# OpenVisualCloud/SVT-HEVC

Hardware: AMD Instinct MI355X
Metric: front-half fps, 4K 8-bit encMode 7 random-access B pictures (BASELINE configs[2]): pictures per second through upload + picture preparation + open-loop motion estimation of 2040 LCUs against 2 list(s) (HME L0 64x32 + L1, full-pel 16x9 85-PU search, sub-pel, bi-prediction) + open-loop intra search +  (higher is better)
Workload: dtype u8; 1 GPU

## Files before the change

include/svt_hevc_amd.h:

```cpp
#ifndef SVT_HEVC_AMD_H
#define SVT_HEVC_AMD_H

#include <stdint.h>
#include <stddef.h>

#ifdef __cplusplus
extern "C" {
#endif

#define SVT_AMD_API __attribute__((visibility("default")))

typedef enum SvtAmdStatus {
    SVT_AMD_OK = 0,
    SVT_AMD_ERR_BAD_PARAM = -1,
    SVT_AMD_ERR_RESOURCES = -2,
    SVT_AMD_ERR_DEVICE = -3
} SvtAmdStatus;


#define SVT_AMD_LCU_SIZE 64
#define SVT_AMD_ME_PU_COUNT 85
#define SVT_AMD_PAD_FULL 68
#define SVT_AMD_PAD_QUARTER 32
#define SVT_AMD_PAD_SIXTEENTH 16
// ... 1239 lines not shown
                                        uint32_t refStride, void *d_dst, uint32_t dstStride,
                                        const SvtAmdMcpBlock *d_blocks, uint32_t nblocks, uint32_t max_block_dim);
SVT_AMD_API int svt_amd_bipred_clip_batch(SvtAmdContext *ctx, int bytes_per_sample, const int16_t *d_l0,
                                          const int16_t *d_l1, void *d_dst, uint32_t dstStride, int32_t offset,
                                          const SvtAmdBiPredBlock *d_blocks, uint32_t nblocks);

#define SVT_AMD_DECL_MCP_UNI(name, T)                                                                          \
    SVT_AMD_API void svt_amd_##name(T *refPic, uint32_t srcStride, T *dst, uint32_t dstStride, uint32_t puWidth, \
                                    uint32_t puHeight, int16_t *firstPassIFDst);
#define SVT_AMD_DECL_MCP_RAW(name, T)                                                                          \
    SVT_AMD_API void svt_amd_##name(T *refPic, uint32_t srcStride, int16_t *dst, uint32_t puWidth,             \
                                    uint32_t puHeight, int16_t *firstPassIFDst);
#define SVT_AMD_DECL_MCP_CUNI(name, T)                                                                         \
    SVT_AMD_API void svt_amd_##name(T *refPic, uint32_t srcStride, T *dst, uint32_t dstStride, uint32_t puWidth, \
                                    uint32_t puHeight, int16_t *firstPassIFDst, uint32_t fracPosx, uint32_t fracPosy);
#define SVT_AMD_DECL_MCP_CRAW(name, T)                                                                         \
    SVT_AMD_API void svt_amd_##name(T *refPic, uint32_t srcStride, int16_t *dst, uint32_t puWidth,             \
                                    uint32_t puHeight, int16_t *firstPassIFDst, uint32_t fracPosx, uint32_t fracPosy);
SVT_AMD_DECL_MCP_UNI(LumaInterpolationFilterPosaNew, uint8_t)
SVT_AMD_DECL_MCP_UNI(LumaInterpolationFilterPosaNew16bit, uint16_t)
SVT_AMD_DECL_MCP_RAW(LumaInterpolationFilterPosaOutRaw, uint8_t)
SVT_AMD_DECL_MCP_RAW(LumaInterpolationFilterPosaOutRaw16bit, uint16_t)
SVT_AMD_DECL_MCP_UNI(LumaInterpolationFilterPosbNew, uint8_t)
SVT_AMD_DECL_MCP_UNI(LumaInterpolationFilterPosbNew16bit, uint16_t)
SVT_AMD_DECL_MCP_RAW(LumaInterpolationFilterPosbOutRaw, uint8_t)
SVT_AMD_DECL_MCP_RAW(LumaInterpolationFilterPosbOutRaw16bit, uint16_t)
SVT_AMD_DECL_MCP_UNI(LumaInterpolationFilterPoscNew, uint8_t)
SVT_AMD_DECL_MCP_UNI(LumaInterpolationFilterPoscNew16bit, uint16_t)
SVT_AMD_DECL_MCP_RAW(LumaInterpolationFilterPoscOutRaw, uint8_t)
SVT_AMD_DECL_MCP_RAW(LumaInterpolationFilterPoscOutRaw16bit, uint16_t)
SVT_AMD_DECL_MCP_UNI(LumaInterpolationFilterPosdNew, uint8_t)
SVT_AMD_DECL_MCP_UNI(LumaInterpolationFilterPosdNew16bit, uint16_t)
SVT_AMD_DECL_MCP_RAW(LumaInterpolationFilterPosdOutRaw, uint8_t)
SVT_AMD_DECL_MCP_RAW(LumaInterpolationFilterPosdOutRaw16bit, uint16_t)
SVT_AMD_DECL_MCP_UNI(LumaInterpolationFilterPoseNew, uint8_t)
SVT_AMD_DECL_MCP_UNI(LumaInterpolationFilterPoseNew16bit, uint16_t)
SVT_AMD_DECL_MCP_RAW(LumaInterpolationFilterPoseOutRaw, uint8_t)
SVT_AMD_DECL_MCP_RAW(LumaInterpolationFilterPoseOutRaw16bit, uint16_t)
SVT_AMD_DECL_MCP_UNI(LumaInterpolationFilterPosfNew, uint8_t)
SVT_AMD_DECL_MCP_UNI(LumaInterpolationFilterPosfNew16bit, uint16_t)
SVT_AMD_DECL_MCP_RAW(LumaInterpolationFilterPosfOutRaw, uint8_t)
SVT_AMD_DECL_MCP_RAW(LumaInterpolationFilterPosfOutRaw16bit, uint16_t)
SVT_AMD_DECL_MCP_UNI(LumaInterpolationFilterPosgNew, uint8_t)
SVT_AMD_DECL_MCP_UNI(LumaInterpolationFilterPosgNew16bit, uint16_t)
SVT_AMD_DECL_MCP_RAW(LumaInterpolationFilterPosgOutRaw, uint8_t)
SVT_AMD_DECL_MCP_RAW(LumaInterpolationFilterPosgOutRaw16bit, uint16_t)
SVT_AMD_DECL_MCP_UNI(LumaInterpolationFilterPoshNew, uint8_t)
SVT_AMD_DECL_MCP_UNI(LumaInterpolationFilterPoshNew16bit, uint16_t)
SVT_AMD_DECL_MCP_RAW(LumaInterpolationFilterPoshOutRaw, uint8_t)
SVT_AMD_DECL_MCP_RAW(LumaInterpolationFilterPoshOutRaw16bit, uint16_t)
SVT_AMD_DECL_MCP_UNI(LumaInterpolationFilterPosiNew, uint8_t)
SVT_AMD_DECL_MCP_UNI(LumaInterpolationFilterPosiNew16bit, uint16_t)
SVT_AMD_DECL_MCP_RAW(LumaInterpolationFilterPosiOutRaw, uint8_t)
SVT_AMD_DECL_MCP_RAW(LumaInterpolationFilterPosiOutRaw16bit, uint16_t)
SVT_AMD_DECL_MCP_UNI(LumaInterpolationFilterPosjNew, uint8_t)
SVT_AMD_DECL_MCP_UNI(LumaInterpolationFilterPosjNew16bit, uint16_t)
SVT_AMD_DECL_MCP_RAW(LumaInterpolationFilterPosjOutRaw, uint8_t)
SVT_AMD_DECL_MCP_RAW(LumaInterpolationFilterPosjOutRaw16bit, uint16_t)
SVT_AMD_DECL_MCP_UNI(LumaInterpolationFilterPoskNew, uint8_t)
SVT_AMD_DECL_MCP_UNI(LumaInterpolationFilterPoskNew16bit, uint16_t)
SVT_AMD_DECL_MCP_RAW(LumaInterpolationFilterPoskOutRaw, uint8_t)
SVT_AMD_DECL_MCP_RAW(LumaInterpolationFilterPoskOutRaw16bit, uint16_t)
SVT_AMD_DECL_MCP_UNI(LumaInterpolationFilterPosnNew, uint8_t)
SVT_AMD_DECL_MCP_UNI(LumaInterpolationFilterPosnNew16bit, uint16_t)
SVT_AMD_DECL_MCP_RAW(LumaInterpolationFilterPosnOutRaw, uint8_t)
SVT_AMD_DECL_MCP_RAW(LumaInterpolationFilterPosnOutRaw16bit, uint16_t)
SVT_AMD_DECL_MCP_UNI(LumaInterpolationFilterPospNew, uint8_t)
SVT_AMD_DECL_MCP_UNI(LumaInterpolationFilterPospNew16bit, uint16_t)
SVT_AMD_DECL_MCP_RAW(LumaInterpolationFilterPospOutRaw, uint8_t)
SVT_AMD_DECL_MCP_RAW(LumaInterpolationFilterPospOutRaw16bit, uint16_t)
SVT_AMD_DECL_MCP_UNI(LumaInterpolationFilterPosqNew, uint8_t)
SVT_AMD_DECL_MCP_UNI(LumaInterpolationFilterPosqNew16bit, uint16_t)
SVT_AMD_DECL_MCP_RAW(LumaInterpolationFilterPosqOutRaw, uint8_t)
SVT_AMD_DECL_MCP_RAW(LumaInterpolationFilterPosqOutRaw16bit, uint16_t)
SVT_AMD_DECL_MCP_UNI(LumaInterpolationFilterPosrNew, uint8_t)
SVT_AMD_DECL_MCP_UNI(LumaInterpolationFilterPosrNew16bit, uint16_t)
SVT_AMD_DECL_MCP_RAW(LumaInterpolationFilterPosrOutRaw, uint8_t)
SVT_AMD_DECL_MCP_RAW(LumaInterpolationFilterPosrOutRaw16bit, uint16_t)
SVT_AMD_DECL_MCP_UNI(LumaInterpolationCopy, uint8_t)
SVT_AMD_DECL_MCP_UNI(LumaInterpolationCopy16bit, uint16_t)
SVT_AMD_DECL_MCP_RAW(LumaInterpolationCopyOutRaw, uint8_t)
SVT_AMD_DECL_MCP_RAW(LumaInterpolationCopyOutRaw16bit, uint16_t)
SVT_AMD_DECL_MCP_CUNI(ChromaInterpolationCopy, uint8_t)
SVT_AMD_DECL_MCP_CUNI(ChromaInterpolationFilterOneD, uint8_t)
SVT_AMD_DECL_MCP_CUNI(ChromaInterpolationFilterTwoD, uint8_t)
SVT_AMD_DECL_MCP_CUNI(ChromaInterpolationCopy16bit, uint16_t)
SVT_AMD_DECL_MCP_CUNI(ChromaInterpolationFilterOneD16bit, uint16_t)
SVT_AMD_DECL_MCP_CUNI(ChromaInterpolationFilterTwoD16bit, uint16_t)
SVT_AMD_DECL_MCP_CRAW(ChromaInterpolationCopyOutRaw, uint8_t)
SVT_AMD_DECL_MCP_CRAW(ChromaInterpolationFilterOneDOutRaw, uint8_t)
SVT_AMD_DECL_MCP_CRAW(ChromaInterpolationFilterTwoDOutRaw, uint8_t)
SVT_AMD_DECL_MCP_CRAW(ChromaInterpolationCopyOutRaw16bit, uint16_t)
SVT_AMD_DECL_MCP_CRAW(ChromaInterpolationFilterOneDOutRaw16bit, uint16_t)
SVT_AMD_DECL_MCP_CRAW(ChromaInterpolationFilterTwoDOutRaw16bit, uint16_t)
SVT_AMD_API void svt_amd_BiPredClipping(uint32_t puWidth, uint32_t puHeight, int16_t *list0Src, int16_t *list1Src,
                                        uint8_t *dst, uint32_t dstStride, int32_t offset);
SVT_AMD_API void svt_amd_BiPredClipping16bit(uint32_t puWidth, uint32_t puHeight, int16_t *list0Src, int16_t *list1Src,
                                             uint16_t *dst, uint32_t dstStride);


typedef struct SvtAmdMdRates {
    uint32_t splitFlagBits[6], skipFlagBits[6], mvpIndexBits[2], intraPartSizeBits[2], interPartSizeBits[8], predModeBits[2];
    uint32_t intraLumaBits[4], intraChromaBits[5], refPicBits[3], mvdBits[12], lumaCbfBits[10], chromaCbfBits[10], rootCbfBits[2];
    uint32_t transSubDivFlagBits[6], mergeFlagBits[2], mergeIndexBits[5], saoMergeFlagBits[2], saoTypeIndexBits[6];
    uint32_t saoOffsetTrunUnaryBits[8], interBiDirBits[8], interUniDirBits[2], pad[17];
} SvtAmdMdRates;
typedef struct SvtAmdMdPicture {
    uint16_t width, height;
    uint8_t slice_type;
    uint8_t temporal_layer, is_reference, enc_mode;
    uint8_t depth_mode;
    uint8_t intra_md_open_loop;
    uint8_t intra_injection_method;
    uint8_t limit_intra;
    uint8_t mpm_search, mpm_search_candidate;
    uint8_t pf_md_level, nfl_level_md, nmm_level_md;
    uint8_t full_loop_escape, single_fast_loop, coeff_cabac_update, spatial_sse_full_loop;
    uint8_t chroma_level;
    uint8_t intra4x4_level;
    uint8_t rdoq_pmcore_method;
    uint8_t skip_ois_8x8, cu8x8_mode, cu16x16_mode, limit_ois_to_dc_mode;
    uint8_t constrained_intra, strong_smoothing;
    uint8_t qp, chroma_qp;
    uint8_t intra8x8_restriction_inter_slice;
    uint8_t pad;
    uint32_t fast_lambda, full_lambda, fast_chroma_lambda, full_chroma_lambda;
    SvtAmdMdRates rates;
} SvtAmdMdPicture;
#define SVT_AMD_MD_LEAVES 85
typedef struct SvtAmdMdLcu {
    uint8_t leaf_count;
    uint8_t leaf_index[SVT_AMD_MD_LEAVES], leaf_split[SVT_AMD_MD_LEAVES];
    uint8_t tile_left, tile_top, tile_right;
    uint8_t is_complete;
    uint8_t complexity_status_2;
    uint8_t contouring_class[4];
    uint8_t chroma_encode_mode;
    uint8_t restrict_intra_global_motion;
    uint8_t lcu_md_mode;
    uint8_t skip_small_cu;
    uint8_t cmplx_noise;
    uint8_t variance_below_200;
    uint8_t edge_block;
    uint8_t no_stop_split;
    uint8_t pad[3];
} SvtAmdMdLcu;
typedef struct SvtAmdTmvpLcu {
    int16_t mv[2][16][2];
    uint64_t ref_poc[2][16];
    uint8_t pred_dir[16], available[16];
} SvtAmdTmvpLcu;
typedef struct SvtAmdMdInter {
    uint64_t picture_number;
    uint64_t ref_poc[2];
    uint64_t colocated_poc;
    uint8_t colocated_pu_ref_list, is_low_delay;
    uint8_t tmvp_enable;
    uint8_t use_subpel;
    uint8_t unrestricted_mv;
    uint8_t generate_amvp_table_md;
    uint8_t extra_injection;
    uint8_t improve_sharpness;
    uint8_t skip_cost_bias;
    uint8_t pad[3];
    uint32_t chroma_weight;
} SvtAmdMdInter;
typedef struct SvtAmdMdLcuOut {
    uint8_t split[SVT_AMD_MD_LEAVES];
    uint8_t tested[SVT_AMD_MD_LEAVES];
    uint8_t pred_mode[SVT_AMD_MD_LEAVES];
    uint8_t intra_luma_mode[SVT_AMD_MD_LEAVES];
    uint8_t ycbf[SVT_AMD_MD_LEAVES];
    uint8_t inter_dir[SVT_AMD_MD_LEAVES];
    uint8_t merge_flag[SVT_AMD_MD_LEAVES], merge_index[SVT_AMD_MD_LEAVES];
    uint8_t pad[8];
    int16_t mv[SVT_AMD_MD_LEAVES][2][2];
    uint64_t cost[SVT_AMD_MD_LEAVES];
    uint64_t merge_cost[SVT_AMD_MD_LEAVES], skip_cost[SVT_AMD_MD_LEAVES];
} SvtAmdMdLcuOut;
SVT_AMD_API int svt_amd_md_picture_supported(const SvtAmdMdPicture *P);
SVT_AMD_API int svt_amd_md_encode_picture(SvtAmdContext *ctx, SvtAmdEncDecPicture *pic, const SvtAmdMdPicture *P, const SvtAmdMdLcu *lcus,
                                          const uint8_t *src_y, uint32_t stride_y, const uint8_t *src_cb, const uint8_t *src_cr,
                                          uint32_t stride_c, const SvtAmdOisLcuResult *ois, int ois_slot, const SvtAmdCabacCost *cost,
                                          SvtAmdMdLcuOut *md_out, SvtAmdLcuWork *works, SvtAmdLcuResult *results);
SVT_AMD_API int svt_amd_md_encode_picture_inter(SvtAmdContext *ctx, SvtAmdEncDecPicture *pic, const SvtAmdMdPicture *P, const SvtAmdMdInter *X,
                                                const SvtAmdMdLcu *lcus, const uint8_t *src_y, uint32_t stride_y, const uint8_t *src_cb,
                                                const uint8_t *src_cr, uint32_t stride_c, const SvtAmdOisLcuResult *ois, int ois_slot,
                                                const SvtAmdMeLcuResult *me, int me_slot, const SvtAmdTmvpLcu *tmvp,
                                                SvtAmdMdLcuOut *md_out, SvtAmdLcuWork *works, SvtAmdLcuResult *results);
SVT_AMD_API int svt_amd_md_encode_picture16(SvtAmdContext *ctx, SvtAmdEncDecPicture *pic, const SvtAmdMdPicture *P, const SvtAmdMdLcu *lcus,
                                            const uint16_t *src_y, uint32_t stride_y, const uint16_t *src_cb, const uint16_t *src_cr,
                                            uint32_t stride_c, const SvtAmdOisLcuResult *ois, int ois_slot, const SvtAmdCabacCost *cost,
                                            SvtAmdMdLcuOut *md_out, SvtAmdLcuWork16 *works, SvtAmdLcuResult16 *results);
SVT_AMD_API int svt_amd_md_encode_picture_inter16(SvtAmdContext *ctx, SvtAmdEncDecPicture *pic, const SvtAmdMdPicture *P, const SvtAmdMdInter *X,
                                                  const SvtAmdMdLcu *lcus, const uint16_t *src_y, uint32_t stride_y, const uint16_t *src_cb,
                                                  const uint16_t *src_cr, uint32_t stride_c, const SvtAmdOisLcuResult *ois, int ois_slot,
                                                  const SvtAmdMeLcuResult *me, int me_slot, const SvtAmdTmvpLcu *tmvp, SvtAmdMdLcuOut *md_out,
                                                  SvtAmdLcuWork16 *works, SvtAmdLcuResult16 *results);
SVT_AMD_API int svt_amd_md_picture_supported_inter(const SvtAmdMdPicture *P, const SvtAmdMdInter *X);
SVT_AMD_API int svt_amd_md_lcus_supported(const SvtAmdMdPicture *P, const SvtAmdMdLcu *lcus, int n);
SVT_AMD_API int svt_amd_md_picture_set_controls(SvtAmdContext *ctx, SvtAmdEncDecPicture *pic, const SvtAmdMdLcu *d_lcus);

#define SVT_AMD_MD_LAUNCH_DECIDE_ONLY 1u
typedef struct SvtAmdMdLaunchJob {
    const SvtAmdMdPicture *P;
    const SvtAmdMdInter *X;
    const SvtAmdCabacCost *cost;
    const SvtAmdMdLcu *d_lcus;
    const void *d_src[3];
    const SvtAmdOisLcuResult *d_ois;
    const SvtAmdMeLcuResult *d_me;
    const SvtAmdTmvpLcu *d_tmvp;
    uint32_t src_pitch_y, src_pitch_c;
    int32_t ois_slot, me_slot;
    uint32_t tiles;
    uint32_t flags;
    uint32_t pad[2];
} SvtAmdMdLaunchJob;
typedef struct SvtAmdMdLaunchStatus {
    SvtAmdMdCtlCheck check;
    uint32_t refused;
    uint32_t pad;
} SvtAmdMdLaunchStatus;
#ifdef __cplusplus
static_assert(sizeof(SvtAmdMdLaunchJob) == 112 && sizeof(SvtAmdMdLaunchStatus) == 96, "launch records");
#else
_Static_assert(sizeof(SvtAmdMdLaunchJob) == 112 && sizeof(SvtAmdMdLaunchStatus) == 96, "launch records");
#endif
SVT_AMD_API int svt_amd_md_encode_picture_launch(SvtAmdContext *ctx, SvtAmdEncDecPicture *pic, const SvtAmdMdLaunchJob *job, SvtAmdMdLaunchStatus *d_status);
SVT_AMD_API int svt_amd_encdec_picture_md_records(SvtAmdEncDecPicture *pic, const SvtAmdMdLcuOut **d_out, const void **d_works, size_t *work_stride,
                                                  const void **d_results, size_t *result_stride);

typedef struct SvtAmdMotionFieldJob {
    const void *d_works;
    size_t      work_stride;
    uint16_t    width, height;
    uint8_t     slice_type;
    uint8_t     pad[3];
    uint64_t    ref_poc[2];
} SvtAmdMotionFieldJob;
typedef struct SvtAmdRefStats {
    uint32_t intra_area_sum;
    uint8_t  intra_coded_area;
    uint8_t  pad[3];
} SvtAmdRefStats;
#define SVT_AMD_MOTION_FIELD 0
#define SVT_AMD_MOTION_FIELD_STATS 1
SVT_AMD_API size_t svt_amd_motion_field_bytes(uint16_t luma_width, uint16_t luma_height, int which);
SVT_AMD_API int svt_amd_motion_field_launch(SvtAmdContext *ctx, const SvtAmdMotionFieldJob *job, SvtAmdTmvpLcu *d_field, SvtAmdRefStats *d_stats);
SVT_AMD_API int svt_amd_encdec_picture_motion_field(SvtAmdContext *ctx, SvtAmdEncDecPicture *pic, int slice_type, const uint64_t ref_poc[2], SvtAmdTmvpLcu *d_field,
                                                    SvtAmdRefStats *d_stats);
SVT_AMD_API int svt_amd_md_picture_set_motion_field(SvtAmdContext *ctx, SvtAmdEncDecPicture *pic, const SvtAmdTmvpLcu *d_field);
SVT_AMD_API int svt_amd_debug_md_profile(SvtAmdContext *ctx, SvtAmdEncDecPicture *pic, unsigned long long *out);
SVT_AMD_API int svt_amd_debug_md_profile_sub(SvtAmdContext *ctx, SvtAmdEncDecPicture *pic, unsigned long long *out);
SVT_AMD_API int svt_amd_debug_md_profile_depth(SvtAmdContext *ctx, SvtAmdEncDecPicture *pic, unsigned long long *out);
SVT_AMD_API int svt_amd_debug_md_force_butterflies(SvtAmdContext *ctx, SvtAmdEncDecPicture *pic, int on);
SVT_AMD_API int svt_amd_debug_md_trace(SvtAmdContext *ctx, SvtAmdEncDecPicture *pic, int lcu, int unit, unsigned long long *out);
SVT_AMD_API int svt_amd_debug_md_kernel_ms(SvtAmdContext *ctx, SvtAmdEncDecPicture *pic, float *ms, int *workgroups);
SVT_AMD_API int svt_amd_debug_md_ep_ms(SvtAmdContext *ctx, SvtAmdEncDecPicture *pic, float *ms);
SVT_AMD_API int svt_amd_debug_md_flights(int *in_flight, int *workgroups_held, int *waiting);
SVT_AMD_API int svt_amd_md_picture_warmup(SvtAmdContext *ctx, SvtAmdEncDecPicture *pic);
SVT_AMD_API int svt_amd_debug_md_kernel_lds_bytes(int inter, int bytes_per_sample);
typedef struct SvtAmdMdListNb {
    int16_t mv[2][2];
    uint8_t dir, avail, pad[2];
} SvtAmdMdListNb;
typedef struct SvtAmdMdListJob {
    uint16_t width, height;
    uint16_t ox, oy;
    uint8_t size;
    uint8_t slice_type;
    uint8_t colocated_pu_ref_list, is_low_delay;
    uint8_t has_field;
    uint8_t total_merge;
    uint8_t tile_left, tile_top, tile_right;
    uint8_t me_dir;
    uint16_t pool[2];
    int16_t me_mv[2][2];
    uint8_t pad[2];
    uint64_t picture_number, ref_poc[2], colocated_poc;
    SvtAmdMdListNb nb[5];
    uint8_t pad2[4];
} SvtAmdMdListJob;
typedef struct SvtAmdMdListOut {
    int16_t amvp[2][2][2];
    uint8_t amvp_count[2];
    uint8_t merge_count;
    uint8_t mvp_idx[2];
    uint8_t merge_dir[5];
    int16_t merge_mv[5][2][2];
    int16_t cand_mv[2][2];
    int16_t mvp[2][2];
    uint8_t pad[14];
} SvtAmdMdListOut;
#ifdef __cplusplus
static_assert(sizeof(SvtAmdMdListNb) == 12 && sizeof(SvtAmdMdListJob) == 128 && sizeof(SvtAmdMdListOut) == 96, "tests mirror these layouts as numpy dtypes");
#else
_Static_assert(sizeof(SvtAmdMdListNb) == 12 && sizeof(SvtAmdMdListJob) == 128 && sizeof(SvtAmdMdListOut) == 96, "tests mirror these layouts as numpy dtypes");
#endif
SVT_AMD_API int svt_amd_debug_md_lists_batch(SvtAmdContext *ctx, const SvtAmdMdListJob *d_jobs, const SvtAmdTmvpLcu *d_pool, SvtAmdMdListOut *d_outs, uint32_t n);
SVT_AMD_API int svt_amd_debug_me_kernel_lds_bytes(const SvtAmdMeParams *params, int phase);
SVT_AMD_API int svt_amd_debug_me_kernel_occupancy(SvtAmdContext *ctx, const SvtAmdMeParams *params, int phase, int *workgroups_per_cu, int *private_bytes);
SVT_AMD_API int svt_amd_debug_launch_markers(SvtAmdContext *ctx, unsigned long long *records, unsigned long long *waits);

#ifdef __cplusplus
}
#endif
#endif
```

svt-hevc_amd/csrc/context.hip:

```cpp
#include <stdarg.h>
#include <stdio.h>
#include <stdlib.h>
#include <string.h>
#include "svt_amd_internal.h"
#include <vector>
#include <mutex>

static thread_local char g_err[512] = "";

void svt_amd_set_error(const char *fmt, ...)
{
    va_list ap;
    va_start(ap, fmt);
    vsnprintf(g_err, sizeof(g_err), fmt, ap);
    va_end(ap);
}

extern "C" const char *svt_amd_last_error(void) { return g_err; }
extern "C" const char *svt_amd_version(void) { return "svt-hevc_amd 0.1 (gfx950)"; }

static int align_up(int v, int a) { return (v + a - 1) / a * a; }

static int plane_create(DevPlane *p, int w, int h, int pad)
{
// ... 422 lines not shown
        HIP_TRY(hipMemcpy(dst, d_src, bytes, hipMemcpyDeviceToHost));
        return SVT_AMD_OK;
    }
    HIP_TRY(hipMemcpyAsync(dst, d_src, bytes, hipMemcpyDeviceToHost, svt_amd_ctx_stream(ctx)));
    HIP_TRY(svt_amd_ctx_sync(ctx));
    return SVT_AMD_OK;
}

extern "C" int svt_amd_device_upload_async(SvtAmdContext *ctx, void *d_dst, const void *src, size_t bytes)
{
    if (!ctx || !d_dst || !src)
        return SVT_AMD_ERR_BAD_PARAM;
    HIP_TRY(hipSetDevice(ctx->device));
    HIP_TRY(hipMemcpyAsync(d_dst, src, bytes, hipMemcpyHostToDevice, svt_amd_ctx_stream(ctx)));
    return SVT_AMD_OK;
}
extern "C" int svt_amd_device_download_async(SvtAmdContext *ctx, void *dst, const void *d_src, size_t bytes)
{
    if (!ctx || !dst || !d_src)
        return SVT_AMD_ERR_BAD_PARAM;
    HIP_TRY(hipSetDevice(ctx->device));
    HIP_TRY(hipMemcpyAsync(dst, d_src, bytes, hipMemcpyDeviceToHost, svt_amd_ctx_stream(ctx)));
    return SVT_AMD_OK;
}
extern "C" int svt_amd_host_alloc(SvtAmdContext *ctx, size_t bytes, void **h_ptr)
{
    if (!ctx || !h_ptr || !bytes)
        return SVT_AMD_ERR_BAD_PARAM;
    HIP_TRY(hipSetDevice(ctx->device));
    HIP_TRY(hipHostMalloc(h_ptr, bytes, hipHostMallocDefault));
    return SVT_AMD_OK;
}
namespace {
struct HostReg { const void *p; size_t bytes; bool ok; };
std::mutex g_reg_mu;
std::vector<HostReg> g_reg;
}
extern "C" int svt_amd_host_register(SvtAmdContext *ctx, const void *h_ptr, size_t bytes)
{
    if (!ctx || !h_ptr || !bytes)
        return SVT_AMD_ERR_BAD_PARAM;
    std::lock_guard<std::mutex> g(g_reg_mu);
    for (HostReg &r : g_reg)
        if (r.p == h_ptr && r.bytes >= bytes)
            return SVT_AMD_OK;
    for (HostReg &r : g_reg)
        if ((const uint8_t *)h_ptr < (const uint8_t *)r.p + r.bytes && (const uint8_t *)r.p < (const uint8_t *)h_ptr + bytes) {
            g_reg.push_back({h_ptr, bytes, false});
            return SVT_AMD_OK;
        }
    (void)hipSetDevice(ctx->device);
    const hipError_t e = hipHostRegister(const_cast<void *>(h_ptr), bytes, hipHostRegisterDefault);
    if (e != hipSuccess)
        (void)hipGetLastError();
    g_reg.push_back({h_ptr, bytes, e == hipSuccess});
    return SVT_AMD_OK;
}
const void *svt_amd_registered_device_ptr(const void *h_ptr, size_t bytes)
{
    std::lock_guard<std::mutex> g(g_reg_mu);
    for (const HostReg &r : g_reg)
        if (r.ok && (const uint8_t *)h_ptr >= (const uint8_t *)r.p && (const uint8_t *)h_ptr + bytes <= (const uint8_t *)r.p + r.bytes) {
            void *d = nullptr;
            if (hipHostGetDevicePointer(&d, const_cast<void *>(r.p), 0) != hipSuccess) {
                (void)hipGetLastError();
                return nullptr;
            }
            return (const uint8_t *)d + ((const uint8_t *)h_ptr - (const uint8_t *)r.p);
        }
    return nullptr;
}
extern "C" int svt_amd_host_unregister_all(SvtAmdContext *ctx)
{
    if (!ctx)
        return SVT_AMD_ERR_BAD_PARAM;
    std::lock_guard<std::mutex> g(g_reg_mu);
    (void)hipSetDevice(ctx->device);
    for (HostReg &r : g_reg)
        if (r.ok && hipHostUnregister(const_cast<void *>(r.p)) != hipSuccess)
            (void)hipGetLastError();
    g_reg.clear();
    return SVT_AMD_OK;
}
extern "C" int svt_amd_host_free(SvtAmdContext *ctx, void *h_ptr)
{
    if (!ctx)
        return SVT_AMD_ERR_BAD_PARAM;
    HIP_TRY(hipSetDevice(ctx->device));
    HIP_TRY(hipHostFree(h_ptr));
    return SVT_AMD_OK;
}


static int check_slot(SvtAmdContext *ctx, int slot)
{
    if (!ctx || slot < 0 || slot >= ctx->num_slots) {
        svt_amd_set_error("bad context/slot %d", slot);
        return SVT_AMD_ERR_BAD_PARAM;
    }
    return SVT_AMD_OK;
}

static int set_geometry(SvtAmdContext *ctx, DevPicture *s, uint16_t width, uint16_t height)
{
    if (width < 64 || height < 64 || (width & 7) || (height & 7) || width > ctx->max_w || height > ctx->max_h) {
        svt_amd_set_error("picture %ux%u not supported by context %ux%u", width, height, ctx->max_w, ctx->max_h);
        return SVT_AMD_ERR_BAD_PARAM;
    }
    s->width = width;
    s->height = height;
    s->full.width = s->hp_b.width = s->hp_h.width = s->hp_j.width = width;
    s->full.height = s->hp_b.height = s->hp_h.height = s->hp_j.height = height;
    s->quarter.width = width >> 1, s->quarter.height = height >> 1;
    s->sixteenth.width = width >> 2, s->sixteenth.height = height >> 2;
    return SVT_AMD_OK;
}

extern "C" int svt_amd_picture_upload_device(SvtAmdContext *ctx, int slot, const void *d_luma,
                                             uint32_t stride, uint16_t width, uint16_t height)
{
    int rc = check_slot(ctx, slot);
    if (rc)
        return rc;
    if (!d_luma || stride < width)
        return SVT_AMD_ERR_BAD_PARAM;
    HIP_TRY(hipSetDevice(ctx->device));
    DevPicture *s = &ctx->slots[slot];
    if ((rc = set_geometry(ctx, s, width, height)) != 0)
        return rc;
    if ((rc = svt_amd_launch_prep(ctx, s, (const uint8_t *)d_luma, stride)) != 0)
        return rc;
    slot_records_forget(&s->rec);
    s->valid = 1;
    return SVT_AMD_OK;
}

extern "C" int svt_amd_picture_upload_device_batch(SvtAmdContext *ctx, int num, const int *slots,
                                                   const void *const *d_luma, uint32_t stride, uint16_t width,
                                                   uint16_t height)
{
    if (!ctx || !slots || !d_luma || num < 1 || num > SVT_AMD_MAX_BATCH || stride < width)
        return SVT_AMD_ERR_BAD_PARAM;
    HIP_TRY(hipSetDevice(ctx->device));
    DevPicture *pics[SVT_AMD_MAX_BATCH];
    for (int i = 0; i < num; i++) {
        int rc = check_slot(ctx, slots[i]);
        if (rc)
            return rc;
        if (!d_luma[i])
            return SVT_AMD_ERR_BAD_PARAM;
        pics[i] = &ctx->slots[slots[i]];
        if ((rc = set_geometry(ctx, pics[i], width, height)) != 0)
            return rc;
    }
    int rc = svt_amd_launch_prep_batch(ctx, pics, (const uint8_t *const *)d_luma, stride, num);
    if (rc)
        return rc;
    for (int i = 0; i < num; i++)
        slot_records_forget(&pics[i]->rec), pics[i]->valid = 1;
    return SVT_AMD_OK;
}

extern "C" int svt_amd_picture_upload(SvtAmdContext *ctx, int slot, const uint8_t *luma,
                                      uint32_t stride, uint16_t width, uint16_t height)
{
    int rc = check_slot(ctx, slot);
    if (rc)
        return rc;
    if (!luma || stride < width)
        return SVT_AMD_ERR_BAD_PARAM;
    HIP_TRY(hipSetDevice(ctx->device));
    DevPicture *s = &ctx->slots[slot];
    if ((size_t)width * height > s->staging_bytes)
        return SVT_AMD_ERR_BAD_PARAM;
    HIP_TRY(hipMemcpy2DAsync(s->d_staging, width, luma, stride, width, height, hipMemcpyHostToDevice, svt_amd_ctx_stream(ctx)));
    HIP_TRY(svt_amd_ctx_sync(ctx));
    return svt_amd_picture_upload_device(ctx, slot, s->d_staging, width, width, height);
}

extern "C" int svt_amd_picture_read_plane(SvtAmdContext *ctx, int slot, int which, uint8_t *dst,
                                          size_t dst_capacity, uint32_t *out_stride,
                                          uint32_t *out_pad, uint32_t *out_rows)
{
    int rc = check_slot(ctx, slot);
    if (rc)
        return rc;
    DevPicture *s = &ctx->slots[slot];
    DevPlane *pl[6] = {&s->full, &s->quarter, &s->sixteenth, &s->hp_b, &s->hp_h, &s->hp_j};
    if (which < 0 || which > 5 || !dst || !out_stride || !out_pad || !out_rows)
        return SVT_AMD_ERR_BAD_PARAM;
    DevPlane *p = pl[which];
    const uint32_t w = (uint32_t)(p->width + 2 * p->pad), rows = (uint32_t)(p->height + 2 * p->pad);
    if (dst_capacity < (size_t)w * rows)
        return SVT_AMD_ERR_BAD_PARAM;
    HIP_TRY(hipSetDevice(ctx->device));
    HIP_TRY(svt_amd_ctx_sync(ctx));
    HIP_TRY(hipMemcpy2D(dst, w, p->origin - (size_t)p->pad * p->pitch - p->pad, (size_t)p->pitch, w, rows,
                        hipMemcpyDeviceToHost));
    *out_stride = w;
    *out_pad = (uint32_t)p->pad;
    *out_rows = rows;
    return SVT_AMD_OK;
}


static int validate_me(SvtAmdContext *ctx, const SvtAmdMeParams *p, int cur_slot, const int ref_slot[2])
{
    if (!ctx || !p || !ref_slot)
        return SVT_AMD_ERR_BAD_PARAM;
    if (p->num_lists < 1 || p->num_lists > 2 || p->num_hme_regions_w > 2 || p->num_hme_regions_h > 2 ||
        p->search_area_width < 1 || p->search_area_height < 1) {
        svt_amd_set_error("svt_amd_me_picture: bad SvtAmdMeParams");
        return SVT_AMD_ERR_BAD_PARAM;
    }
    int rc = check_slot(ctx, cur_slot);
    for (int l = 0; !rc && l < p->num_lists; l++)
        rc = check_slot(ctx, ref_slot[l]);
    if (rc)
        return rc;
    const DevPicture *c = &ctx->slots[cur_slot];
    if (!c->valid || c->width != p->luma_width || c->height != p->luma_height) {
        svt_amd_set_error("svt_amd_me_picture: slot %d does not hold a %ux%u picture", cur_slot, p->luma_width,
                          p->luma_height);
        return SVT_AMD_ERR_BAD_PARAM;
    }
    for (int l = 0; l < p->num_lists; l++) {
        const DevPicture *r = &ctx->slots[ref_slot[l]];
        if (!r->valid || r->width != c->width || r->height != c->height) {
            svt_amd_set_error("svt_amd_me_picture: reference slot %d invalid", ref_slot[l]);
            return SVT_AMD_ERR_BAD_PARAM;
        }
    }
    return SVT_AMD_OK;
}

static int slot_mark_lend(SvtAmdContext *ctx, DevPicture *s, int kind, LaunchMark *mark, uint32_t n, uint32_t begin, uint32_t end)
{
    SlotRecords *r = &s->rec;
    slot_lock(r);
    const hipEvent_t behind = slot_chain_behind(r, kind, ctx, begin == 0 && end >= n);
    hipError_t e = behind ? hipStreamWaitEvent(svt_amd_ctx_stream(ctx), behind, 0) : hipSuccess;
    if (e == hipSuccess && !mark->ev) {
        const hipEvent_t ev = ctx->ev_launch[ctx->launch_next];
        if ((e = hipEventRecord(ev, svt_amd_ctx_stream(ctx))) == hipSuccess) {
            ctx->launch_next = (ctx->launch_next + 1) & 15;
            ctx->mark_records += kind != SLOT_READ;
            *mark = LaunchMark{ev, ctx};
        }
    }
    if (e == hipSuccess) {
        r->mark[kind] = *mark;
        if (kind == SLOT_ME)
            slot_me_cover(r, n, begin, end);
        else if (kind == SLOT_OIS)
            r->ois_lcus = n;
    }
    slot_unlock(r);
    HIP_TRY(e);
    ctx->mark_waits += behind != nullptr;
    return SVT_AMD_OK;
}
int svt_amd_records_wait(SvtAmdContext *ctx, DevPicture *s, int kind, hipEvent_t *seen, int *nseen, int cap)
{
    slot_lock(&s->rec);
    const hipEvent_t ev = slot_wait_for(&s->rec, kind, ctx);
    bool wait = ev != nullptr;
    for (int i = 0; wait && seen && i < *nseen; i++)
        wait = seen[i] != ev;
    const hipError_t e = wait ? hipStreamWaitEvent(svt_amd_ctx_stream(ctx), ev, 0) : hipSuccess;
    if (ev && kind == SLOT_READ && e == hipSuccess)
        s->rec.mark[SLOT_READ] = LaunchMark{nullptr, nullptr};
    slot_unlock(&s->rec);
    HIP_TRY(e);
    if (wait) {
        ctx->mark_waits++;
        if (seen && *nseen < cap)
            seen[(*nseen)++] = ev;
    }
    return SVT_AMD_OK;
}
static int slot_records_before_write(SvtAmdContext *ctx, DevPicture *s) { return svt_amd_records_wait(ctx, s, SLOT_READ, nullptr, nullptr, 0); }
int svt_amd_records_read_mark(SvtAmdContext *ctx, SvtAmdContext *root, int slot)
{
    LaunchMark mark{nullptr, nullptr};
    return slot_mark_lend(ctx, &root->slots[slot], SLOT_READ, &mark, 0, 0, 0);
}
const void *svt_amd_slot_records(SvtAmdContext *root, int slot, int which, int w, int h)
{
    if (slot < 0 || slot >= root->num_slots)
        return nullptr;
    DevPicture *s = &root->slots[slot];
    if (!s->valid || s->width != w || s->height != h || slot_lcus(&s->rec, which) != (uint32_t)svt_amd_lcu_count(w, h))
        return nullptr;
    return which ? (const void *)s->d_ois_out : (const void *)s->d_me_out;
}
extern "C" int svt_amd_debug_launch_markers(SvtAmdContext *ctx, unsigned long long *records, unsigned long long *waits)
{
    if (!ctx || !records || !waits)
        return SVT_AMD_ERR_BAD_PARAM;
    *records = ctx->mark_records, *waits = ctx->mark_waits;
    return SVT_AMD_OK;
}

static int make_job(SvtAmdContext *ctx, const SvtAmdMeParams *params, int cur_slot, const int ref_slot[2],
                    uint32_t lcu_begin, uint32_t lcu_end, MeJobDev *job)
{
    int rc = validate_me(ctx, params, cur_slot, ref_slot);
    if (rc)
        return rc;
    const uint32_t nlcu = svt_amd_lcu_count(params->luma_width, params->luma_height);
    if (lcu_begin >= lcu_end || lcu_end > nlcu) {
        svt_amd_set_error("motion estimation: bad LCU range [%u,%u) of %u", lcu_begin, lcu_end, nlcu);
        return SVT_AMD_ERR_BAD_PARAM;
    }
    DevPicture *c = &ctx->slots[cur_slot];
    const DevPicture *r0 = &ctx->slots[ref_slot[0]];
    const DevPicture *r1 = params->num_lists == 2 ? &ctx->slots[ref_slot[1]] : r0;
    job->P = *params;
    job->cur = make_view(c);
    job->ref0 = make_view(r0);
    job->ref1 = make_view(r1);
    job->out = c->d_me_out;
    job->carry = (struct MeCarry *)c->d_me_carry;
    job->lcu_begin = (int32_t)lcu_begin;
    job->lcu_count = (int32_t)(lcu_end - lcu_begin);
    job->dbg_clock = NULL;
    return SVT_AMD_OK;
}

extern "C" int svt_amd_me_picture_range_launch(SvtAmdContext *ctx, const SvtAmdMeParams *params, int cur_slot,
                                               const int ref_slot[2], uint32_t lcu_begin, uint32_t lcu_end)
{
    MeJobDev job;
    int rc = make_job(ctx, params, cur_slot, ref_slot, lcu_begin, lcu_end, &job);
    if (rc)
        return rc;
    HIP_TRY(hipSetDevice(ctx->device));
    if ((rc = slot_records_before_write(ctx, &ctx->slots[cur_slot])) != 0)
        return rc;
    LaunchMark mark{nullptr, nullptr};
    if ((rc = svt_amd_launch_me_batch(ctx, &job, 1, job.lcu_count)) == SVT_AMD_OK)
        rc = slot_mark_lend(ctx, &ctx->slots[cur_slot], SLOT_ME, &mark, (uint32_t)svt_amd_lcu_count(params->luma_width, params->luma_height), lcu_begin, lcu_end);
    return rc;
}

extern "C" int svt_amd_me_batch_launch(SvtAmdContext *ctx, const SvtAmdMeJob *jobs, int num_jobs)
{
    if (!ctx || !jobs || num_jobs < 1 || num_jobs > SVT_AMD_MAX_BATCH) {
        svt_amd_set_error("svt_amd_me_batch_launch: 1..%d jobs", SVT_AMD_MAX_BATCH);
        return SVT_AMD_ERR_BAD_PARAM;
    }
    MeJobDev *dj = (MeJobDev *)malloc(sizeof(MeJobDev) * (size_t)num_jobs);
    if (!dj)
        return SVT_AMD_ERR_RESOURCES;
    int rc = SVT_AMD_OK, max_lcus = 0;
    for (int i = 0; i < num_jobs && rc == SVT_AMD_OK; i++) {
        const SvtAmdMeParams *p = &jobs[i].params;
        const uint32_t nlcu = svt_amd_lcu_count(p->luma_width, p->luma_height);
        rc = make_job(ctx, p, jobs[i].cur_slot, jobs[i].ref_slot, 0, nlcu, &dj[i]);
        if (rc == SVT_AMD_OK)
            max_lcus = dj[i].lcu_count > max_lcus ? dj[i].lcu_count : max_lcus;
    }
    if (rc == SVT_AMD_OK) {
        hipError_t e = hipSetDevice(ctx->device);
        if (e == hipSuccess && ctx->d_dbg && (size_t)num_jobs * max_lcus <= ctx->dbg_slots)
            for (int i = 0; i < num_jobs; i++)
                dj[i].dbg_clock = ctx->d_dbg;
        for (int i = 0; i < num_jobs && e == hipSuccess && rc == SVT_AMD_OK; i++)
            rc = slot_records_before_write(ctx, &ctx->slots[jobs[i].cur_slot]);
        if (rc == SVT_AMD_OK)
            rc = e == hipSuccess ? svt_amd_launch_me_batch(ctx, dj, num_jobs, max_lcus) : SVT_AMD_ERR_DEVICE;
        LaunchMark mark{nullptr, nullptr};
        for (int i = 0; i < num_jobs && rc == SVT_AMD_OK; i++)
            rc = slot_mark_lend(ctx, &ctx->slots[jobs[i].cur_slot], SLOT_ME, &mark, (uint32_t)dj[i].lcu_count, 0, (uint32_t)dj[i].lcu_count);
    }
    free(dj);
    return rc;
}

extern "C" int svt_amd_debug_me_phase_profile(SvtAmdContext *ctx, size_t workgroups, unsigned long long *out)
{
    if (!ctx)
        return SVT_AMD_ERR_BAD_PARAM;
    HIP_TRY(hipSetDevice(ctx->device));
    if (!out) {
        HIP_TRY(svt_amd_ctx_sync(ctx));
        if (ctx->d_dbg)
            (void)hipFree(ctx->d_dbg);
        ctx->d_dbg = NULL;
        HIP_TRY(hipMalloc((void **)&ctx->d_dbg, workgroups * 16 * sizeof(unsigned long long)));
        HIP_TRY(hipMemset(ctx->d_dbg, 0, workgroups * 16 * sizeof(unsigned long long)));
        ctx->dbg_slots = workgroups;
        return SVT_AMD_OK;
    }
    if (!ctx->d_dbg || workgroups > ctx->dbg_slots)
        return SVT_AMD_ERR_BAD_PARAM;
    HIP_TRY(svt_amd_ctx_sync(ctx));
    HIP_TRY(hipMemcpy(out, ctx->d_dbg, workgroups * 16 * sizeof(unsigned long long), hipMemcpyDeviceToHost));
    (void)hipFree(ctx->d_dbg);
    ctx->d_dbg = NULL;
    ctx->dbg_slots = 0;
    return SVT_AMD_OK;
}

extern "C" int svt_amd_debug_me_kernel_occupancy(SvtAmdContext *ctx, const SvtAmdMeParams *params, int phase, int *workgroups_per_cu, int *private_bytes)
{
    if (!ctx)
        return SVT_AMD_ERR_BAD_PARAM;
    HIP_TRY(hipSetDevice(ctx->device));
    return svt_amd_me_kernel_occupancy(params, phase, workgroups_per_cu, private_bytes);
}

extern "C" int svt_amd_me_picture_launch(SvtAmdContext *ctx, const SvtAmdMeParams *params, int cur_slot,
                                         const int ref_slot[2])
{
    if (!params)
        return SVT_AMD_ERR_BAD_PARAM;
    const uint32_t nlcu = svt_amd_lcu_count(params->luma_width, params->luma_height);
    return svt_amd_me_picture_range_launch(ctx, params, cur_slot, ref_slot, 0, nlcu);
}

static int records_fetch(SvtAmdContext *ctx, int cur_slot, int which, void *out, bool sync)
{
    int rc = check_slot(ctx, cur_slot);
    if (rc)
        return rc;
    if (!out)
        return SVT_AMD_ERR_BAD_PARAM;
    HIP_TRY(hipSetDevice(ctx->device));
    DevPicture *c = &ctx->slots[cur_slot];
    const size_t bytes = (size_t)svt_amd_lcu_count(c->width, c->height) * (which ? sizeof(SvtAmdOisLcuResult) : sizeof(SvtAmdMeLcuResult));
    HIP_TRY(hipMemcpyAsync(out, which ? (const void *)c->d_ois_out : (const void *)c->d_me_out, bytes, hipMemcpyDeviceToHost, svt_amd_ctx_stream(ctx)));
    if (sync)
        HIP_TRY(svt_amd_ctx_sync(ctx));
    return SVT_AMD_OK;
}
extern "C" int svt_amd_me_picture_fetch(SvtAmdContext *ctx, int cur_slot, SvtAmdMeLcuResult *out) { return records_fetch(ctx, cur_slot, 0, out, true); }
extern "C" int svt_amd_me_picture_fetch_async(SvtAmdContext *ctx, int cur_slot, SvtAmdMeLcuResult *out) { return records_fetch(ctx, cur_slot, 0, out, false); }
extern "C" int svt_amd_ois_picture_fetch(SvtAmdContext *ctx, int cur_slot, SvtAmdOisLcuResult *out) { return records_fetch(ctx, cur_slot, 1, out, true); }
extern "C" int svt_amd_ois_picture_fetch_async(SvtAmdContext *ctx, int cur_slot, SvtAmdOisLcuResult *out) { return records_fetch(ctx, cur_slot, 1, out, false); }

extern "C" int svt_amd_lane_event_record(SvtAmdContext *lane, int index)
{
    if (!lane || index < 0 || index >= 8)
        return SVT_AMD_ERR_BAD_PARAM;
    HIP_TRY(hipSetDevice(lane->device));
    if (!lane->ev_user[index])
        HIP_TRY(hipEventCreateWithFlags(&lane->ev_user[index], hipEventDisableTiming));
    HIP_TRY(hipEventRecord(lane->ev_user[index], svt_amd_ctx_stream(lane)));
    return SVT_AMD_OK;
}
extern "C" int svt_amd_lane_event_wait(SvtAmdContext *lane, SvtAmdContext *source, int index)
{
    if (!lane || !source || index < 0 || index >= 8 || lane->device != source->device)
        return SVT_AMD_ERR_BAD_PARAM;
    HIP_TRY(hipSetDevice(lane->device));
    if (source->ev_user[index])
        HIP_TRY(hipStreamWaitEvent(svt_amd_ctx_stream(lane), source->ev_user[index], 0));
    return SVT_AMD_OK;
}

__global__ void __launch_bounds__(256) k_pack_me(const PackSrc *__restrict__ tab, const uint32_t *__restrict__ one, uint32_t *__restrict__ out, int nlcu)
{
    constexpr int IN = sizeof(SvtAmdMeLcuResult) / 4, OUT = SVT_AMD_ME_PU_COUNT * sizeof(SvtAmdMeCuResult) / 4;
    const uint32_t *__restrict__ in = tab ? tab[blockIdx.y].me : one;
    const int i = blockIdx.x * 256 + threadIdx.x, lcu = i / OUT, k = i - lcu * OUT;
    if (lcu < nlcu)
        out[((size_t)blockIdx.y * nlcu + lcu) * OUT + k] = in[(size_t)lcu * IN + k];
}
__global__ void __launch_bounds__(256) k_pack_ois(const PackSrc *__restrict__ tab, const uint32_t *__restrict__ one, uint32_t *__restrict__ out, int nlcu, int nc, int kshift)
{
    constexpr int IN = sizeof(SvtAmdOisLcuResult) / 4, TAIL = 22;
    const int per = SVT_AMD_ME_PU_COUNT * nc + TAIL, lcu = blockIdx.x;
    const uint32_t *__restrict__ src = (tab ? tab[blockIdx.y].ois : one) + (size_t)lcu * IN;
    uint32_t *__restrict__ dst = out + ((size_t)blockIdx.y * nlcu + lcu) * per;
    const int k = threadIdx.x & ((1 << kshift) - 1);
    if (k < nc)
        for (int cu = threadIdx.x >> kshift; cu < SVT_AMD_ME_PU_COUNT; cu += 256 >> kshift)
            dst[cu * nc + k] = src[cu * SVT_AMD_OIS_MAX_CAND + k];
    if (threadIdx.x < TAIL)
        dst[SVT_AMD_ME_PU_COUNT * nc + threadIdx.x] = src[SVT_AMD_ME_PU_COUNT * SVT_AMD_OIS_MAX_CAND + threadIdx.x];
}
static int launch_pack(SvtAmdContext *ctx, const PackSrc *tab, const PackSrc &one, int n, int nlcu, int candidates, void *d_me, void *d_ois)
{
    if (d_me) {
        const int k = nlcu * (int)(SVT_AMD_ME_PU_COUNT * sizeof(SvtAmdMeCuResult) / 4);
        hipLaunchKernelGGL(k_pack_me, dim3((k + 255) / 256, n), dim3(256), 0, svt_amd_ctx_stream(ctx), tab, one.me, (uint32_t *)d_me, nlcu);
    }
    if (d_ois) {
        int kshift = 0;
        while ((1 << kshift) < candidates)
            kshift++;
        hipLaunchKernelGGL(k_pack_ois, dim3(nlcu, n), dim3(256), 0, svt_amd_ctx_stream(ctx), tab, one.ois, (uint32_t *)d_ois, nlcu, candidates, kshift);
    }
    HIP_TRY(hipGetLastError());
    return SVT_AMD_OK;
}
static_assert(sizeof(SvtAmdOisLcuResult) == (SVT_AMD_ME_PU_COUNT * SVT_AMD_OIS_MAX_CAND + 22) * 4, "OIS record layout");
static_assert(sizeof(SvtAmdMeCuResult) == 24 && offsetof(SvtAmdMeLcuResult, pu) == 0, "ME record layout");

extern "C" int svt_amd_ois_compact_candidates(const SvtAmdOisParams *p)
{
    return !p ? SVT_AMD_OIS_MAX_CAND : p->slice_is_intra ? 7 : p->ois_kernel_level ? 18 : 9;
}

static int slot_pack_buffer(SvtAmdContext *ctx, DevPicture *c, size_t bytes, uint8_t **out)
{
    if (bytes > c->pack_bytes) {
        HIP_TRY(svt_amd_ctx_sync(ctx));
        if (c->d_pack)
            (void)hipFree(c->d_pack);
        c->d_pack = nullptr, c->pack_bytes = 0;
        HIP_TRY(hipMalloc((void **)&c->d_pack, bytes));
        c->pack_bytes = bytes;
    }
    *out = c->d_pack;
    return SVT_AMD_OK;
}

static size_t pack_me_bytes(int nlcu) { return ((size_t)nlcu * SVT_AMD_ME_PU_COUNT * sizeof(SvtAmdMeCuResult) + 255) & ~(size_t)255; }

extern "C" int svt_amd_me_picture_fetch_compact_async(SvtAmdContext *ctx, int cur_slot, SvtAmdMeCuResult *out)
{
    int rc = check_slot(ctx, cur_slot);
    if (rc)
        return rc;
    if (!out)
        return SVT_AMD_ERR_BAD_PARAM;
    HIP_TRY(hipSetDevice(ctx->device));
    DevPicture *c = &ctx->slots[cur_slot];
    const int nlcu = svt_amd_lcu_count(c->width, c->height);
    uint8_t *d = nullptr;
    if ((rc = slot_pack_buffer(ctx, c, pack_me_bytes(nlcu) + (size_t)nlcu * sizeof(SvtAmdOisLcuResult), &d)) != 0)
        return rc;
    const int n = nlcu * (int)(SVT_AMD_ME_PU_COUNT * sizeof(SvtAmdMeCuResult) / 4);
    if ((rc = launch_pack(ctx, nullptr, PackSrc{(const uint32_t *)c->d_me_out, nullptr}, 1, nlcu, 1, d, nullptr)) != 0)
        return rc;
    HIP_TRY(hipMemcpyAsync(out, d, (size_t)n * 4, hipMemcpyDeviceToHost, svt_amd_ctx_stream(ctx)));
    return SVT_AMD_OK;
}

extern "C" int svt_amd_ois_picture_fetch_compact_async(SvtAmdContext *ctx, int cur_slot, int candidates, void *out)
{
    int rc = check_slot(ctx, cur_slot);
    if (rc)
        return rc;
    if (!out || candidates < 1 || candidates > SVT_AMD_OIS_MAX_CAND)
        return SVT_AMD_ERR_BAD_PARAM;
    HIP_TRY(hipSetDevice(ctx->device));
    DevPicture *c = &ctx->slots[cur_slot];
    const int nlcu = svt_amd_lcu_count(c->width, c->height);
    uint8_t *d = nullptr;
    if ((rc = slot_pack_buffer(ctx, c, pack_me_bytes(nlcu) + (size_t)nlcu * sizeof(SvtAmdOisLcuResult), &d)) != 0)
        return rc;
    d += pack_me_bytes(nlcu);
    const int n = nlcu * (SVT_AMD_ME_PU_COUNT * candidates + 22);
    if ((rc = launch_pack(ctx, nullptr, PackSrc{nullptr, (const uint32_t *)c->d_ois_out}, 1, nlcu, candidates, nullptr, d)) != 0)
        return rc;
    HIP_TRY(hipMemcpyAsync(out, d, (size_t)n * 4, hipMemcpyDeviceToHost, svt_amd_ctx_stream(ctx)));
    return SVT_AMD_OK;
}

extern "C" int svt_amd_records_pack_batch_async(SvtAmdContext *ctx, const int *slots, int n, int candidates, SvtAmdMeCuResult *d_me, void *d_ois)
{
    if (!ctx || !slots || n < 1 || n > SVT_AMD_MAX_BATCH || (!d_me && !d_ois) || candidates < 1 || candidates > SVT_AMD_OIS_MAX_CAND)
        return SVT_AMD_ERR_BAD_PARAM;
    int rc = check_slot(ctx, slots[0]);
    if (rc)
        return rc;
    HIP_TRY(hipSetDevice(ctx->device));
    const DevPicture *c0 = &ctx->slots[slots[0]];
    const int nlcu = svt_amd_lcu_count(c0->width, c0->height);
    static thread_local PackSrc tab[SVT_AMD_MAX_BATCH];
    for (int i = 0; i < n; i++) {
        if ((rc = check_slot(ctx, slots[i])) != 0)
            return rc;
        const DevPicture *c = &ctx->slots[slots[i]];
        if (c->width != c0->width || c->height != c0->height) {
            svt_amd_set_error("svt_amd_records_pack_batch_async: pictures of different sizes in one batch");
            return SVT_AMD_ERR_BAD_PARAM;
        }
        tab[i].me = (const uint32_t *)c->d_me_out, tab[i].ois = (const uint32_t *)c->d_ois_out;
    }
    if ((rc = svt_amd_upload_descriptors(ctx, ctx->d_pack_src, tab, sizeof(PackSrc) * (size_t)n)) != 0)
        return rc;
    return launch_pack(ctx, (const PackSrc *)ctx->d_pack_src, PackSrc{nullptr, nullptr}, n, nlcu, candidates, d_me, d_ois);
}

extern "C" int svt_amd_me_picture(SvtAmdContext *ctx, const SvtAmdMeParams *params, int cur_slot,
                                  const int ref_slot[2], SvtAmdMeLcuResult *out)
{
    int rc = svt_amd_me_picture_launch(ctx, params, cur_slot, ref_slot);
    if (rc)
        return rc;
    return svt_amd_me_picture_fetch(ctx, cur_slot, out);
}

static int validate_ois(SvtAmdContext *ctx, const SvtAmdOisParams *p, int cur_slot)
{
    int rc = check_slot(ctx, cur_slot);
    if (rc)
        return rc;
    const DevPicture *c = &ctx->slots[cur_slot];
    if (!p || !c->valid || p->luma_width != c->width || p->luma_height != c->height || p->ois_th_set > 2 ||
        p->temporal_layer_index > 5) {
        svt_amd_set_error("svt_amd_ois_picture: bad parameter (slot %d)", cur_slot);
        return SVT_AMD_ERR_BAD_PARAM;
    }
    return SVT_AMD_OK;
}

static void make_ois_job(SvtAmdContext *ctx, const SvtAmdOisParams *params, int cur_slot, const SvtAmdMeLcuResult *d_me,
                         OisJobDev *j)
{
    DevPicture *c = &ctx->slots[cur_slot];
    j->P = *params;
    j->full = c->full.origin;
    j->pitch = c->full.pitch;
    j->lcus_w = (params->luma_width + 63) / 64;
    j->nlcu = j->lcus_w * ((params->luma_height + 63) / 64);
    j->me = d_me;
// ... 284 lines not shown
```

svt-hevc_amd/csrc/me_kernels.hip:

```cpp
#include <mutex>
#include "svt_amd_internal.h"

#define NT 256
#define LCU 64
#ifndef ME_MIN_WAVES_PER_SIMD
#define ME_MIN_WAVES_PER_SIMD 4
#endif
#ifndef ME_HME_WAVES_PER_SIMD
#define ME_HME_WAVES_PER_SIMD 6
#endif
#define COST_PRECISION 8
#define MD_SHIFT 23
#define MD_OFFSET (1u << 22)

typedef uint32_t __attribute__((aligned(1))) u32u;

__device__ __forceinline__ uint32_t ld4(const uint8_t *p) { return *(const u32u *)p; }
__device__ __forceinline__ uint32_t sad4(uint32_t a, uint32_t b, uint32_t acc) { return __builtin_amdgcn_sad_u8(a, b, acc); }
__device__ __forceinline__ uint32_t avg4(uint32_t a, uint32_t b) { return __builtin_amdgcn_lerp(a, b, 0x01010101u); }
__device__ __forceinline__ int imin(int a, int b) { return a < b ? a : b; }
__device__ __forceinline__ int imax(int a, int b) { return a > b ? a : b; }
__device__ __forceinline__ int mvx(uint32_t mv) { return (int)(int16_t)(mv & 0xffff); }
__device__ __forceinline__ int mvy(uint32_t mv) { return (int)(int16_t)(mv >> 16); }
__device__ __forceinline__ uint32_t mvpack(int x, int y) { return ((uint32_t)(uint16_t)y << 16) | (uint16_t)x; }

#define ME_DPP(v, ctrl) ((uint32_t)__builtin_amdgcn_update_dpp(0, (int)(v), ctrl, 0xF, 0xF, true))
template <int GROUP>
__device__ __forceinline__ uint32_t group_sum(uint32_t v)
{
    if (GROUP >= 2)
        v += ME_DPP(v, 0xB1);
    if (GROUP >= 4)
        v += ME_DPP(v, 0x4E);
    if (GROUP >= 8)
        v += ME_DPP(v, 0x141);
    if (GROUP >= 16)
        v += ME_DPP(v, 0x140);
    return v;
}
__device__ __forceinline__ uint32_t group_sum_rt(uint32_t v, int lg)
{
    if (lg >= 1)
        v += ME_DPP(v, 0xB1);
    if (lg >= 2)
        v += ME_DPP(v, 0x4E);
    if (lg >= 3)
        v += ME_DPP(v, 0x141);
    if (lg >= 4)
        v += ME_DPP(v, 0x140);
    if (lg >= 5)
        v += __shfl_xor(v, 16);
    if (lg >= 6)
        v += __shfl_xor(v, 32);
    return v;
}
__device__ __forceinline__ uint32_t wave_sum(uint32_t v)
{
    v = group_sum<16>(v);
    return (uint32_t)__builtin_amdgcn_readlane((int)v, 0) + (uint32_t)__builtin_amdgcn_readlane((int)v, 16) + (uint32_t)__builtin_amdgcn_readlane((int)v, 32) +
           (uint32_t)__builtin_amdgcn_readlane((int)v, 48);
}
__device__ __forceinline__ unsigned long long wave_min64(unsigned long long v)
{
    uint32_t lo = (uint32_t)v, hi = (uint32_t)(v >> 32);
#pragma unroll
    for (int st = 0; st < 4; st++) {
        const int ctrl = st == 0 ? 0xB1 : st == 1 ? 0x4E : st == 2 ? 0x141 : 0x140;
        uint32_t plo, phi;
        if (st == 0)
            plo = ME_DPP(lo, 0xB1), phi = ME_DPP(hi, 0xB1);
        else if (st == 1)
            plo = ME_DPP(lo, 0x4E), phi = ME_DPP(hi, 0x4E);
        else if (st == 2)
            plo = ME_DPP(lo, 0x141), phi = ME_DPP(hi, 0x141);
        else
            plo = ME_DPP(lo, 0x140), phi = ME_DPP(hi, 0x140);
        (void)ctrl;
        const bool less = phi < hi || (phi == hi && plo < lo);
        lo = less ? plo : lo, hi = less ? phi : hi;
    }
    unsigned long long m = ~0ull;
#pragma unroll
    for (int r = 0; r < 64; r += 16) {
        const unsigned long long w = ((unsigned long long)(uint32_t)__builtin_amdgcn_readlane((int)hi, r) << 32) | (uint32_t)__builtin_amdgcn_readlane((int)lo, r);
        m = w < m ? w : m;
    }
    return m;
}

__device__ __forceinline__ uint32_t row_sad(const uint8_t *a, const uint8_t *b, int w)
{
    uint32_t s = 0;
    int x = 0;
    for (; x + 4 <= w; x += 4)
        s = sad4(ld4(a + x), ld4(b + x), s);
    if (x < w) {
        const uint32_t m = (1u << (8 * (w - x))) - 1u;
        s = sad4(ld4(a + x) & m, ld4(b + x) & m, s);
    }
    return s;
}

template <int N>
__device__ __forceinline__ void lds_ld_unaligned(const uint8_t *p, uint32_t (&out)[N])
{
    const uint32_t sh = (uint32_t)(uintptr_t)p & 3u;
    const uint32_t *q = (const uint32_t *)(p - sh);
    uint32_t prev = q[0];
#pragma unroll
    for (int i = 0; i < N; i++) {
        const uint32_t nx = q[i + 1];
        out[i] = __builtin_amdgcn_alignbyte(nx, prev, sh);
        prev = nx;
    }
}

__device__ __forceinline__ uint32_t row_sad_lds(const uint8_t *a, const uint8_t *b, int w)
{
    uint32_t s = 0;
    int x = 0;
    for (; x + 16 <= w; x += 16) {
        uint32_t r[4];
        lds_ld_unaligned<4>(b + x, r);
        const uint4 sv = *(const uint4 *)(a + x);
        s = sad4(sv.x, r[0], s), s = sad4(sv.y, r[1], s), s = sad4(sv.z, r[2], s), s = sad4(sv.w, r[3], s);
    }
    for (; x + 4 <= w; x += 4) {
        uint32_t r[1];
        lds_ld_unaligned<1>(b + x, r);
        s = sad4(*(const uint32_t *)(a + x), r[0], s);
    }
    if (x < w) {
        uint32_t r[1];
        lds_ld_unaligned<1>(b + x, r);
        const uint32_t m = (1u << (8 * (w - x))) - 1u;
        s = sad4(*(const uint32_t *)(a + x) & m, r[0] & m, s);
    }
    return s;
}

__device__ __forceinline__ uint32_t ssd4(uint32_t a, uint32_t b)
{
    uint32_t s = 0;
#pragma unroll
    for (int i = 0; i < 4; i++) {
        const int d = (int)((a >> (8 * i)) & 255) - (int)((b >> (8 * i)) & 255);
        s += (uint32_t)(d * d);
    }
    return s;
}

struct LWin {
    const uint8_t *p;
    int x0, y0, stride;
};
extern __shared__ __attribute__((aligned(16))) uint8_t g_pool[];

__device__ __forceinline__ int win_pitch(int x0, int x1, int odd)
{
    int wa = ((x1 - (x0 & ~15)) + 15) & ~15;
    if (odd && !((wa >> 4) & 1))
        wa += 16;
    return wa;
}
__host__ __device__ __forceinline__ int me_f_pitch(int cols) { return ((cols + 15) & ~15) + 4; }
__host__ __device__ __forceinline__ int me_hp_pitch(int cols) { return (cols + 15) & ~15; }
__device__ __forceinline__ const uint8_t *wat(const LWin &w, int x, int y)
{
    return w.p + (y - w.y0) * w.stride + (x - w.x0);
}
__device__ __forceinline__ int load_window(LWin &w, int off, const uint8_t *plane, int pitch, int x0, int y0, int x1,
                                           int y1, int t, int odd = 0)
{
    const int xa = x0 & ~15, wa = win_pitch(x0, x1, odd), n16 = wa >> 4, rows = y1 - y0;
    uint8_t *dst = g_pool + off;
    w.p = dst, w.x0 = xa, w.y0 = y0, w.stride = wa;
    for (int i = t; i < rows * n16; i += NT) {
        const int r = i / n16, c = i - r * n16;
        *(uint4 *)(dst + r * wa + c * 16) = *(const uint4 *)(plane + (ptrdiff_t)(y0 + r) * pitch + xa + c * 16);
    }
    return off + rows * wa;
}

typedef uint4 __attribute__((aligned(1))) u128u_w;
__device__ __forceinline__ uint32_t umin32(uint32_t a, uint32_t b) { return a < b ? a : b; }
__device__ __forceinline__ uint4 ldu16(const uint8_t *p)
{
    const uint4 v = *(const u128u_w *)p;
    return v;
}

__device__ __forceinline__ int load_window_async(LWin &w, int off, const uint8_t *plane, int pitch, int x0, int y0, int x1,
                                                 int y1, int t, int odd = 0)
{
    const int xa = x0 & ~15, wa = win_pitch(x0, x1, odd), n16 = wa >> 4, rows = y1 - y0, total = rows * n16;
    uint8_t *dst = g_pool + off;
    w.p = dst, w.x0 = xa, w.y0 = y0, w.stride = wa;
    const int lane = t & 63;
    for (int c0 = (t >> 6) * 64; c0 < total; c0 += NT) {
        const int i = c0 + lane;
        if (i < total) {
            const int r = i / n16, c = i - r * n16;
            __builtin_amdgcn_global_load_lds(
                (const __attribute__((address_space(1))) void *)(plane + (ptrdiff_t)(y0 + r) * pitch + xa + c * 16),
                (__attribute__((address_space(3))) void *)(dst + c0 * 16), 16, 0, 0);
        }
    }
    return off + rows * wa;
}

__device__ __forceinline__ int load_windows3_async(LWin &wa_, LWin &wb_, LWin &wc_, int off, const uint8_t *pa, const uint8_t *pb, const uint8_t *pc, int pitch, int x0, int y0,
                                                   int x1, int y1, int t)
{
    const int xa = x0 & ~3, wa = me_hp_pitch(x1 - xa), n16 = wa >> 4, rows = y1 - y0, total = rows * n16, bytes = rows * wa;
    uint8_t *dst = g_pool + off;
    wa_.p = dst, wb_.p = dst + bytes, wc_.p = dst + 2 * bytes;
    wa_.x0 = wb_.x0 = wc_.x0 = xa, wa_.y0 = wb_.y0 = wc_.y0 = y0, wa_.stride = wb_.stride = wc_.stride = wa;
    const int lane = t & 63;
    const uint32_t rc = (1u << 20) / (uint32_t)n16 + 1u;
    for (int c0 = (t >> 6) * 64; c0 < total; c0 += NT) {
        const int i = c0 + lane;
        if (i < total) {
            const int r = (int)(((uint32_t)i * rc) >> 20), c = i - r * n16;
            const ptrdiff_t o = (ptrdiff_t)(y0 + r) * pitch + xa + c * 16;
            __builtin_amdgcn_global_load_lds((const __attribute__((address_space(1))) void *)(pa + o), (__attribute__((address_space(3))) void *)(dst + c0 * 16), 16, 0, 0);
            __builtin_amdgcn_global_load_lds((const __attribute__((address_space(1))) void *)(pb + o), (__attribute__((address_space(3))) void *)(dst + bytes + c0 * 16), 16, 0, 0);
            __builtin_amdgcn_global_load_lds((const __attribute__((address_space(1))) void *)(pc + o), (__attribute__((address_space(3))) void *)(dst + 2 * bytes + c0 * 16), 16, 0, 0);
        }
    }
    return off + 3 * bytes;
}

__constant__ uint8_t c_tab16[16] = {0, 1, 4, 5, 2, 3, 6, 7, 8, 9, 12, 13, 10, 11, 14, 15};
__constant__ uint8_t c_tab8[64] = {0,  1,  4,  5,  16, 17, 20, 21, 2,  3,  6,  7,  18, 19, 22, 23,
                                   8,  9,  12, 13, 24, 25, 28, 29, 10, 11, 14, 15, 26, 27, 30, 31,
                                   32, 33, 36, 37, 48, 49, 52, 53, 34, 35, 38, 39, 50, 51, 54, 55,
                                   40, 41, 44, 45, 56, 57, 60, 61, 42, 43, 46, 47, 58, 59, 62, 63};

struct QSrc { int8_t plane, dx, dy; };
__constant__ QSrc c_qtab[4][8][2] = {
    {{{1, 0, 0}, {0, 0, 0}}, {{0, 0, 0}, {1, 1, 0}}, {{2, 0, 0}, {0, 0, 0}}, {{0, 0, 0}, {2, 0, 1}},
     {{1, 0, 0}, {2, 0, 0}}, {{2, 0, 0}, {1, 1, 0}}, {{2, 0, 1}, {1, 1, 0}}, {{1, 0, 0}, {2, 0, 1}}},
    {{{0, -1, 0}, {1, 0, 0}}, {{1, 0, 0}, {0, 0, 0}}, {{3, 0, 0}, {1, 0, 0}}, {{1, 0, 0}, {3, 0, 1}},
     {{2, -1, 0}, {1, 0, 0}}, {{1, 0, 0}, {2, 0, 0}}, {{1, 0, 0}, {2, 0, 1}}, {{2, -1, 1}, {1, 0, 0}}},
    {{{3, 0, 0}, {2, 0, 0}}, {{2, 0, 0}, {3, 1, 0}}, {{0, 0, -1}, {2, 0, 0}}, {{2, 0, 0}, {0, 0, 0}},
     {{1, 0, -1}, {2, 0, 0}}, {{2, 0, 0}, {1, 1, -1}}, {{2, 0, 0}, {1, 1, 0}}, {{1, 0, 0}, {2, 0, 0}}},
    {{{2, -1, 0}, {3, 0, 0}}, {{3, 0, 0}, {2, 0, 0}}, {{1, 0, -1}, {3, 0, 0}}, {{3, 0, 0}, {1, 0, 0}},
     {{2, -1, 0}, {1, 0, -1}}, {{1, 0, -1}, {2, 0, 0}}, {{1, 0, 0}, {2, 0, 0}}, {{2, -1, 0}, {1, 0, 0}}}};

enum { D_TL = 0, D_T = 1, D_TR = 2, D_R = 3, D_BR = 4, D_B = 5, D_BL = 6, D_L = 7 };

__device__ __forceinline__ void pu_geom_z(int n, int &x, int &y, int &sz)
{
    if (n == 0) {
        x = 0, y = 0, sz = 64;
    } else if (n < 5) {
        const int k = n - 1;
        x = (k & 1) << 5, y = (k >> 1) << 5, sz = 32;
    } else if (n < 21) {
        const int z = n - 5;
        x = ((z & 1) | (((z >> 2) & 1) << 1)) << 4;
        y = (((z >> 1) & 1) | (((z >> 3) & 1) << 1)) << 4;
        sz = 16;
    } else {
        const int z = n - 21;
        x = ((z & 1) | (((z >> 2) & 1) << 1) | (((z >> 4) & 1) << 2)) << 3;
        y = (((z >> 1) & 1) | (((z >> 3) & 1) << 1) | (((z >> 5) & 1) << 2)) << 3;
        sz = 8;
    }
}

__device__ __forceinline__ void clamp_area(int origin, int pad, int pic, int &o, int &size)
{
    if (origin + o < -pad)
        o = -pad - origin;
    if (origin + o > pic - 1)
        o = o - ((origin + o) - (pic - 1));
    if (origin + o + size > pic)
        size = imax(1, size - ((origin + o + size) - pic));
}
__device__ __forceinline__ int clamp_center(int origin, int c, int pad, int pic)
{
    if (origin + c < -pad)
        c = -pad - origin;
    if (origin + c > pic - 1)
        c = c - ((origin + c) - (pic - 1));
    return c;
}

__device__ uint32_t mvd_fraction_bits(int mvdX, int mvdY, const uint32_t *bits)
{
    const uint32_t ax = (uint32_t)abs(mvdX), ay = (uint32_t)abs(mvdY);
    const uint32_t xn = mvdX != 0, yn = mvdY != 0, xg = ax > 1, yg = ay > 1;
    uint32_t n = bits[xn] + bits[yn + (2u << xn)];
    if (xn)
        n += bits[xg + 6];
    if (yn)
        n += bits[yg + 6 + (2u << xg)];
    for (int k = 0; k < 2; k++) {
        const uint32_t a = k ? ay : ax, nz = k ? yn : xn, gt = k ? yg : xg;
        if (!nz)
            continue;
        if (gt) {
            uint32_t symbol = a - 2, count = 1, bn = 0;
            while (symbol >= (1u << count)) {
                bn++;
                symbol -= 1u << count;
                count++;
            }
            n += (bn + 1 + count) * 32768u;
        }
        n += 32768u;
    }
    return n;
}

struct MeShared {
    uint8_t src[LCU * LCU + 16];
    uint8_t qsrc[32 * 16 + 16];
    uint8_t ssrc[16 * 8 + 16];
    unsigned long long hkey[4];
    uint32_t acc[8];
    int16_t hx[3][2][2], hy[3][2][2];
    unsigned long long hs[3][2][2];
    int qp[4][4];
    int cand[6][4];
    uint32_t mvd_bits[12];
};
struct MeSearchShared {
    uint8_t src[LCU * LCU + 16];
};
template <int PHASE> struct MeStatic { typedef MeShared type; };
template <> struct MeStatic<1> { typedef MeSearchShared type; };
struct MeSearch {
    union {
        uint32_t sad32[256][4];
        uint32_t dist[85][8];
    };
    uint32_t key[85];
    unsigned long long key64;
    uint32_t best_sad[2][85], best_mv[2][85];
    uint8_t dir[2][85];
    uint32_t bipred[85];
    int sums[12];
};
struct MeSearchSsd {
    uint32_t dsad[85][8];
    uint32_t best_ssd[2][85];
};
#define ME_SEARCH_BYTES ((int)((sizeof(MeSearch) + 15) & ~(size_t)15))
#define ME_SEARCH_SSD_BYTES ((int)((sizeof(MeSearchSsd) + 15) & ~(size_t)15))
struct MeCarry {
    int16_t hx[3][2][2], hy[3][2][2];
    unsigned long long hs[3][2][2];
    int32_t cx[2], cy[2];
    int32_t hme_init_done, pad;
};
static_assert(sizeof(MeCarry) <= 192, "context.hip reserves 192 bytes of carry per LCU");


typedef uint4 __attribute__((aligned(1))) u128u;
__device__ __forceinline__ void lcu_sads(MeShared &S, const uint8_t *ref, int pitch, int ox, int oy, int lw, int lh, int ncand, int t,
                         int first = 0)
{
    if (t < 8 && t >= first)
        S.acc[t] = 0;
    __syncthreads();
    const int rows = lh >> 1;
    if (lw == LCU) {
        for (int i = first * 128 + t; i < ncand * 128; i += NT) {
            const int c = i >> 7, r = (i >> 2) & 31, qx = (i & 3) << 4;
            uint32_t s = 0;
            if (r < rows) {
                const uint4 a = *(const uint4 *)&S.src[(2 * r) * LCU + qx];
                const uint4 b = *(const u128u *)(ref + (ptrdiff_t)(oy + S.cand[c][3] + 2 * r) * pitch + ox + S.cand[c][2] + qx);
                s = sad4(a.x, b.x, s), s = sad4(a.y, b.y, s), s = sad4(a.z, b.z, s), s = sad4(a.w, b.w, s);
            }
            s = wave_sum(s);
            if ((t & 63) == 0)
                atomicAdd(&S.acc[c], s);
        }
    } else {
        for (int i = first * 32 + t; i < ncand * 32; i += NT) {
            const int c = i >> 5, r = i & 31;
            if (r < rows) {
                const uint32_t s = row_sad(&S.src[(2 * r) * LCU],
                                           ref + (ptrdiff_t)(oy + S.cand[c][3] + 2 * r) * pitch + ox + S.cand[c][2], lw);
                atomicAdd(&S.acc[c], s);
            }
        }
    }
    __syncthreads();
}

__device__ __forceinline__ uint32_t fastdiv_recip(uint32_t d) { return (1u << 24) / d + 1u; }
__device__ __forceinline__ uint32_t fastdiv(uint32_t p, uint32_t r) { return (uint32_t)(((unsigned long long)p * r) >> 24); }

__device__ __forceinline__ void hme_pass(MeShared &S, int level, const uint8_t *refplane, int pitch, int bx0, int by0, int bw,
                         int rows, int nq, int t)
{
    if (t < 4)
        S.hkey[t] = ~0ull;
    {
        int off = 0;
        for (int q = 0; q < nq; q++) {
            const int qx = S.qp[q][0], qy = S.qp[q][1], qw = S.qp[q][2], qh = S.qp[q][3];
            LWin w;
            off = load_window(w, off, refplane, pitch, bx0 + qx, by0 + qy, bx0 + qx + qw + bw,
                              by0 + qy + qh + 2 * (rows - 1) + 1, t);
        }
    }
    __syncthreads();
    const uint8_t *src = level == 0 ? S.ssrc : level == 1 ? S.qsrc : S.src;
    const int sstride = level == 0 ? 16 : level == 1 ? 32 : 2 * LCU;
    const int lg = level == 0 ? 3 : level == 1 ? 4 : 5;
    const int y = t & (rows - 1);
    const uint8_t *srow = src + y * sstride;
    int off = 0;
    for (int q = 0; q < nq; q++) {
        const int qx = S.qp[q][0], qw = S.qp[q][2], qh = S.qp[q][3];
        const int x0 = bx0 + qx, xa = x0 & ~15, wstride = ((x0 + qw + bw - xa) + 15) & ~15;
        const int wrows = qh + 2 * (rows - 1) + 1;
        const uint8_t *wbase = g_pool + off + (x0 - xa) + y * 2 * wstride;
        off += wrows * wstride;
        const int npos = qw * qh, items = npos << lg;
        const uint32_t rc = fastdiv_recip((uint32_t)(qw > 0 ? qw : 1));
        unsigned long long best = ~0ull;
        for (int i0 = 0; i0 < items; i0 += NT) {
            const int p = (i0 + t) >> lg;
            uint32_t sv = 0;
            if (p < npos) {
                const int sy = (int)fastdiv((uint32_t)p, rc), sx = p - sy * qw;
                sv = row_sad_lds(srow, wbase + sy * wstride + sx, bw);
            }
            for (int o = rows >> 1; o > 0; o >>= 1)
                sv += __shfl_xor(sv, o);
            const unsigned long long k = p < npos ? (((unsigned long long)sv << 32) | (uint32_t)p) : ~0ull;
            best = k < best ? k : best;
        }
        best = wave_min64(best);
        if ((t & 63) == 0)
            atomicMin(&S.hkey[q], best);
    }
    __syncthreads();
}

__device__ __forceinline__ unsigned long long qsad(uint32_t ref_lo, uint32_t ref_hi, uint32_t src, unsigned long long acc)
{
    return __builtin_amdgcn_qsad_pk_u16_u8(((unsigned long long)ref_hi << 32) | ref_lo, src, acc);
}

template <int G, int ROWS, int C>
__device__ __forceinline__ void hme_pass_q(MeShared &S, const uint8_t *src, int sstride, const uint8_t *refplane, int pitch, int bx0,
                           int by0, int nq, int t)
{
    if (t < 4)
        S.hkey[t] = ~0ull;
    {
        int off = 0;
        for (int q = 0; q < nq; q++) {
            const int qx = S.qp[q][0], qy = S.qp[q][1], qw = S.qp[q][2], qh = S.qp[q][3];
            LWin w;
            off = load_window_async(w, off, refplane, pitch, bx0 + qx, by0 + qy, bx0 + qx + qw + 4 * G,
                                    by0 + qy + qh + 2 * (ROWS - 1) + 1, t, 1);
        }
    }
    __builtin_amdgcn_s_waitcnt(0);
    __syncthreads();
    const int wave = t >> 6, lane = t & 63;
    const int q = wave % nq, slot = wave / nq, nslots = (4 + nq - 1 - q) / nq;
    int off = 0;
    for (int k = 0; k < q; k++) {
        const int x0k = bx0 + S.qp[k][0];
        off += (S.qp[k][3] + 2 * (ROWS - 1) + 1) * win_pitch(x0k, x0k + S.qp[k][2] + 4 * G, 1);
    }
    const int qw = S.qp[q][2], qh = S.qp[q][3];
    const int x0 = bx0 + S.qp[q][0], xa = x0 & ~15, wstride = win_pitch(x0, x0 + qw + 4 * G, 1);
    const int bo0 = x0 - xa;
    const int m0 = bo0 >> 2, mcount = ((bo0 + qw - 1) >> 2) - m0 + 1;
    const int items = qh * mcount * C;
    const uint32_t rc = fastdiv_recip((uint32_t)(mcount > 0 ? mcount : 1));
    constexpr int RPC = ROWS / C;
    unsigned long long best = ~0ull;
    for (int i0 = slot * 64; i0 < items; i0 += nslots * 64) {
        const int li = i0 + lane, it = li / C, ch = li - it * C;
        const bool live = li < items;
        uint32_t sd[4] = {0, 0, 0, 0};
        int sy = 0, mi = 0;
        if (live) {
            sy = (int)fastdiv((uint32_t)it, rc), mi = it - sy * mcount;
            const uint32_t *wr = (const uint32_t *)(g_pool + off + (sy + 2 * ch * RPC) * wstride) + m0 + mi;
            const uint8_t *sr = src + ch * RPC * sstride;
            unsigned long long acc = 0;
#pragma unroll
            for (int r = 0; r < RPC; r++) {
                uint32_t d0 = wr[0];
#pragma unroll
                for (int g4 = 0; g4 < G; g4 += 4) {
                    const uint32_t d1 = wr[g4 + 1], d2 = wr[g4 + 2], d3 = wr[g4 + 3], d4 = wr[g4 + 4];
                    const uint4 sv = *(const uint4 *)(sr + 4 * g4);
                    acc = qsad(d0, d1, sv.x, acc);
                    acc = qsad(d1, d2, sv.y, acc);
                    acc = qsad(d2, d3, sv.z, acc);
                    acc = qsad(d3, d4, sv.w, acc);
                    d0 = d4;
                }
                wr += (2 * wstride) >> 2;
                sr += sstride;
            }
            sd[0] = (uint32_t)(acc & 0xffff), sd[1] = (uint32_t)(acc >> 16) & 0xffff;
            sd[2] = (uint32_t)(acc >> 32) & 0xffff, sd[3] = (uint32_t)(acc >> 48);
        }
        if (C > 1)
            sd[0] = group_sum<C>(sd[0]), sd[1] = group_sum<C>(sd[1]), sd[2] = group_sum<C>(sd[2]), sd[3] = group_sum<C>(sd[3]);
        if (live && ch == 0) {
#pragma unroll
            for (int k = 0; k < 4; k++) {
                const int sx = 4 * (m0 + mi) + k - bo0;
                if (sx >= 0 && sx < qw) {
                    const unsigned long long key = ((unsigned long long)sd[k] << 32) | (uint32_t)(sy * qw + sx);
                    best = key < best ? key : best;
                }
            }
        }
    }
    best = wave_min64(best);
    if (lane == 0 && best != ~0ull)
        atomicMin(&S.hkey[q], best);
    __syncthreads();
}

__device__ __forceinline__ int hme_l12_width(int w) { return (w < 8) ? 8 : (w & 7) ? w + (w - ((w >> 3) << 3)) : w; }

__device__ __forceinline__ void row_metric(int method, uint32_t a, uint32_t b, uint32_t &d, uint32_t &sad)
{
    const bool ssd = method == SVT_AMD_SSD_SEARCH;
    const uint32_t r = sad4(a, b, ssd ? sad : d);
    const uint32_t q = ssd ? ssd4(a, b) : 0u;
    sad = ssd ? r : sad;
    d = ssd ? d + q : r;
}

#ifndef ME_EXP
#define ME_EXP 0
#endif
#define ME_BI_ITEMS 3
#define ME_F_ITEMS 3
#define LDS_BARRIER() asm volatile("s_waitcnt lgkmcnt(0)\n\ts_barrier" ::: "memory")

#define STAMP(i)                                                                      \
    do {                                                                              \
        if (J.dbg_clock && t == 0)                                                    \
            J.dbg_clock[((size_t)blockIdx.y * J.lcu_count + (lcu - lcu_begin)) * 16 + (i)] = __builtin_readcyclecounter(); \
    } while (0)

__device__ __forceinline__ int tier_first_of(int tier) { return tier == 0 ? 0 : tier == 1 ? 1 : tier == 2 ? 5 : 21; }
__device__ __forceinline__ int tier_cnt_of(int tier) { return 1 << (2 * tier); }
__device__ __forceinline__ int tier_sz_of(int tier) { return 64 >> tier; }
__device__ __forceinline__ int tier_lc_of(int tier) { return tier == 0 ? 5 : tier == 1 ? 3 : tier == 2 ? 1 : 0; }
__device__ __forceinline__ int pick4(int i, int a, int b, int c, int d) { return i == 0 ? a : i == 1 ? b : i == 2 ? c : d; }

template <int PHASE>
__global__ __launch_bounds__(NT, PHASE == 0 ? ME_HME_WAVES_PER_SIMD : ME_MIN_WAVES_PER_SIMD) void k_me(const MeJobDev *__restrict__ jobs, int list)
{
    __shared__ typename MeStatic<PHASE>::type S;
    const MeJobDev &J = jobs[blockIdx.y];
    const int per_xcd = (J.lcu_count + 7) >> 3;
    const int blk = (int)(blockIdx.x & 7) * per_xcd + (int)(blockIdx.x >> 3);
    if ((int)(blockIdx.x >> 3) >= per_xcd || blk >= J.lcu_count)
        return;
    const SvtAmdMeParams &P = J.P;
    if (list >= P.num_lists)
        return;
    const PicView cur = J.cur;
    const PicView &ref0 = J.ref0, &ref1 = J.ref1;
    SvtAmdMeLcuResult *__restrict__ out = J.out;
    const int lcu_begin = J.lcu_begin;
    const int t = threadIdx.x;
    const int W = P.luma_width, H = P.luma_height;
    const int wl = (W + LCU - 1) / LCU;
    const int lcu = lcu_begin + blk;
    const int ox = (lcu % wl) * LCU, oy = (lcu / wl) * LCU;
    const int lw = imin(LCU, W - ox), lh = imin(LCU, H - oy);
    const int pf = cur.pitch_full;
    const int method = P.fractional_search_method;
    MeCarry *__restrict__ carry = &J.carry[lcu];
    SvtAmdMeLcuResult *o = &out[lcu];
    MeSearch &B = *(MeSearch *)g_pool;
    MeSearchSsd &BS = *(MeSearchSsd *)(g_pool + ME_SEARCH_BYTES);
    const PicView &R = list ? ref1 : ref0;
    (void)method;

    STAMP(PHASE == 0 ? 0 : 5);
    int cx = 0, cy = 0;
    const uint32_t mv64_l0 = (PHASE == 0 && list) ? o->best_mv[0][0] : 0u;
    auto tsab_cand = [&](int c, int &ux, int &uy, int &kx, int &ky) {
        ux = c == 1 ? -(int)P.hme_l0_total_w : c == 2 ? (int)P.hme_l0_total_w : c == 5 ? 0 - (mvx(mv64_l0) >> 2) : 0;
        uy = c == 3 ? -(int)P.hme_l0_total_h : c == 4 ? (int)P.hme_l0_total_h : c == 5 ? 0 - (mvy(mv64_l0) >> 2) : 0;
        ux = (int16_t)ux, uy = (int16_t)uy;
        kx = c ? clamp_center(ox, ux, LCU - 1, W) : 0, ky = c ? clamp_center(oy, uy, LCU - 1, H) : 0;
    };
    const bool tsab_early = PHASE == 0 && (P.temporal_layer_index > 0 || list == 0) && P.update_hme_search_center && lw == LCU;
    const int tsab_nc = list == 1 ? 6 : 5;
    uint4 tsab_b[3];
    if constexpr (PHASE == 0) {
        uint32_t sv[4];
#pragma unroll
        for (int k = 0; k < 4; k++) {
            const int i = t + k * NT, y = i >> 4, x = (i & 15) << 2;
            sv[k] = *(const uint32_t *)(cur.full + (ptrdiff_t)(oy + y) * pf + ox + x);
        }
        if (tsab_early) {
#pragma unroll
            for (int k = 0; k < 3; k++) {
                const int i = t + k * NT, c = i >> 7, r = (i >> 2) & 31, qx = (i & 3) << 4;
                tsab_b[k] = make_uint4(0, 0, 0, 0);
                if (c < tsab_nc && r < (lh >> 1)) {
                    int ux, uy, kx, ky;
                    tsab_cand(c, ux, uy, kx, ky);
                    tsab_b[k] = ldu16(R.full + (ptrdiff_t)(oy + ky + 2 * r) * R.pitch_full + ox + kx + qx);
                }
            }
        }
#pragma unroll
        for (int k = 0; k < 4; k++) {
            const int i = t + k * NT, y = i >> 4, x = (i & 15) << 2;
            *(uint32_t *)&S.src[y * LCU + x] = sv[k];
        }
        if (t < 8)
            S.acc[t] = 0;
        if (t < 128) {
            const int y = t >> 3, x = (t & 7) << 2;
            *(uint32_t *)&S.qsrc[y * 32 + x] =
                ld4(cur.quarter + (ptrdiff_t)((oy >> 1) + 2 * y) * cur.pitch_quarter + (ox >> 1) + x);
        } else if (t < 160) {
            const int u = t - 128, y = u >> 2, x = (u & 3) << 2;
            *(uint32_t *)&S.ssrc[y * 16 + x] =
                ld4(cur.sixteenth + (ptrdiff_t)((oy >> 2) + 2 * y) * cur.pitch_sixteenth + (ox >> 2) + x);
        }
        if (t >= 64 && t < 76)
            S.mvd_bits[t - 64] = P.mvd_bits[t - 64];
        if (t < 12) {
            (&S.hx[0][0][0])[t] = list ? (&carry->hx[0][0][0])[t] : (int16_t)0;
            (&S.hy[0][0][0])[t] = list ? (&carry->hy[0][0][0])[t] : (int16_t)0;
            (&S.hs[0][0][0])[t] = list ? (&carry->hs[0][0][0])[t] : 0ull;
        }
        __syncthreads();
    }

    LWin wF, wB, wH, wJ;

    if constexpr (PHASE == 0) {
        int hme_init_done = list ? carry->hme_init_done : 0;
        int zero_sad_valid = 0;
        if (P.temporal_layer_index > 0 || list == 0) {
            STAMP(1);
            if (P.update_hme_search_center) {
                const int nc = tsab_nc;
                if (t < 6) {
                    int ux, uy, kx, ky;
                    tsab_cand(t, ux, uy, kx, ky);
                    S.cand[t][0] = ux, S.cand[t][1] = uy;
                    S.cand[t][2] = kx, S.cand[t][3] = ky;
                }
                if (tsab_early) {
#pragma unroll
                    for (int k = 0; k < 3; k++) {
                        const int i = t + k * NT, c = i >> 7, r = (i >> 2) & 31, qx = (i & 3) << 4;
                        if (i < nc * 128) {
                            uint32_t sd = 0;
                            if (r < (lh >> 1)) {
                                const uint4 a = *(const uint4 *)&S.src[(2 * r) * LCU + qx], b = tsab_b[k];
                                sd = sad4(a.x, b.x, sd), sd = sad4(a.y, b.y, sd), sd = sad4(a.z, b.z, sd), sd = sad4(a.w, b.w, sd);
                            }
                            sd = wave_sum(sd);
                            if ((t & 63) == 0)
                                atomicAdd(&S.acc[c], sd);
                        }
                    }
                    __syncthreads();
                } else {
                    __syncthreads();
                    lcu_sads(S, R.full, R.pitch_full, ox, oy, lw, lh, nc, t);
                }
                zero_sad_valid = 1;
                const uint32_t a0 = S.acc[0], a1 = S.acc[1], a2 = S.acc[2], a3 = S.acc[3], a4 = S.acc[4],
                               a5 = nc == 6 ? S.acc[5] : 0xffffffffu;
                uint32_t best = a0;
                best = a1 < best ? a1 : best, best = a2 < best ? a2 : best, best = a3 < best ? a3 : best;
                best = a4 < best ? a4 : best, best = a5 < best ? a5 : best;
                const int pick = best == a0 ? 0 : best == a1 ? 1 : best == a2 ? 2 : best == a3 ? 3 : best == a5 ? 5 : 4;
                cx = S.cand[pick][0], cy = S.cand[pick][1];
                __syncthreads();
            }

            STAMP(2);
            if (P.enable_hme_flag && lh == LCU) {
                const int nw = P.num_hme_regions_w, nh = P.num_hme_regions_h;
                const int one = (P.one_quadrant_hme && !P.enable_hme_level1 && !P.enable_hme_level2);
                const int nq = nw * nh;
                const int qh_ = t < 4 ? (nw == 2 ? (t >> 1) : t) : 0, qw_ = t < 4 ? (nw == 2 ? (t & 1) : 0) : 0;
                if (!hme_init_done) {
                    if (t < nq) {
                        const int sh0 = P.update_hme_search_center ? 2 : 0, sh1 = P.update_hme_search_center ? 1 : 0;
                        S.hx[0][qw_][qh_] = (int16_t)(cx >> sh0), S.hy[0][qw_][qh_] = (int16_t)(cy >> sh0);
                        S.hx[1][qw_][qh_] = (int16_t)(cx >> sh1), S.hy[1][qw_][qh_] = (int16_t)(cy >> sh1);
                        S.hx[2][qw_][qh_] = (int16_t)cx, S.hy[2][qw_][qh_] = (int16_t)cy;
                    }
                    hme_init_done = 1;
                    __syncthreads();
                }
                const uint32_t mx = P.hme_l0_mult_x, my = P.hme_l0_mult_y;
                if (P.enable_hme_level0) {
                    const int px16 = ox >> 2, py16 = oy >> 2;
                    const int pw16 = W >> 2, ph16 = H >> 2, pad16 = SVT_AMD_PAD_SIXTEENTH - 1;
                    const int nq0 = one ? 1 : nq;
                    if (t < nq0) {
                        int sw, sh, so_x, so_y;
                        if (one) {
                            sw = (int16_t)((P.hme_l0_total_w * mx) / 100), sh = (int16_t)((P.hme_l0_total_h * my) / 100);
                            so_x = -(int)(int16_t)(sw >> 1) + (cx >> 2), so_y = -(int)(int16_t)(sh >> 1) + (cy >> 2);
                            clamp_area(px16, pad16, pw16, so_x, sw);
                            clamp_area(py16, pad16, ph16, so_y, sh);
                            if (sw & 15)
                                sw = (sw >> 4) << 4;
                        } else {
                            sw = (int16_t)(((qw_ ? P.hme_l0_w[1] : P.hme_l0_w[0]) * mx) / 100), sh = (int16_t)(((qh_ ? P.hme_l0_h[1] : P.hme_l0_h[0]) * my) / 100);
                            int dx = cx >> 2, dy = cy >> 2;
                            if (qw_)
                                dx += (int16_t)((P.hme_l0_w[0] * mx) / 100);
                            if (qh_)
                                dy += (int16_t)((P.hme_l0_h[0] * my) / 100);
                            so_x = (int16_t)(-(int)(int16_t)(((P.hme_l0_total_w * mx) / 100) >> 1) + dx);
                            so_y = (int16_t)(-(int)(int16_t)(((P.hme_l0_total_h * my) / 100) >> 1) + dy);
                            clamp_area(px16, pad16, pw16, so_x, sw);
                            clamp_area(py16, pad16, ph16, so_y, sh);
                        }
                        S.qp[t][0] = so_x, S.qp[t][1] = so_y, S.qp[t][2] = sw, S.qp[t][3] = sh;
                    }
                    __syncthreads();
                    if ((lw >> 2) == 16)
                        hme_pass_q<4, 8, 1>(S, S.ssrc, 16, R.sixteenth, R.pitch_sixteenth, px16, py16, nq0, t);
                    else
                        hme_pass(S, 0, R.sixteenth, R.pitch_sixteenth, px16, py16, lw >> 2, 8, nq0, t);
                    if (t < nq0) {
                        const unsigned long long k = S.hkey[t];
                        const int qx = S.qp[t][0], qy = S.qp[t][1], qwv = S.qp[t][2];
                        if (k != ~0ull) {
                            const int p = (int)(uint32_t)k, sy = p / qwv, sx = p - sy * qwv;
                            S.hx[0][qw_][qh_] = (int16_t)((int16_t)(sx + qx) * 4);
                            S.hy[0][qw_][qh_] = (int16_t)((int16_t)(sy + qy) * 4);
                            S.hs[0][qw_][qh_] = (k >> 32) * 2;
                        } else {
                            S.hs[0][qw_][qh_] = 0xffffffull * 2;
                            S.hx[0][qw_][qh_] = (int16_t)((int16_t)(S.hx[0][qw_][qh_] + qx) * 4);
                            S.hy[0][qw_][qh_] = (int16_t)((int16_t)(S.hy[0][qw_][qh_] + qy) * 4);
                        }
                    }
                    if (!P.enable_hme_level1 && !P.enable_hme_level2)
                        __syncthreads();
                }
                for (int lvl = 1; lvl <= 2; lvl++) {
                    if (!(lvl == 1 ? P.enable_hme_level1 : P.enable_hme_level2))
                        continue;
                    const int shf = 2 - lvl;
                    const int bx0 = ox >> shf, by0 = oy >> shf, pwl = W >> shf, phl = H >> shf;
                    const int padl = lvl == 2 ? LCU - 1 : SVT_AMD_PAD_QUARTER - 1;
                    if (t < nq) {
                        int sw = hme_l12_width((int16_t)(lvl == 1 ? (qw_ ? P.hme_l1_w[1] : P.hme_l1_w[0]) : (qw_ ? P.hme_l2_w[1] : P.hme_l2_w[0])));
                        int sh = (int16_t)(lvl == 1 ? (qh_ ? P.hme_l1_h[1] : P.hme_l1_h[0]) : (qh_ ? P.hme_l2_h[1] : P.hme_l2_h[0]));
                        const int pcx = lvl == 1 ? (S.hx[0][qw_][qh_] >> 1) : S.hx[1][qw_][qh_];
                        const int pcy = lvl == 1 ? (S.hy[0][qw_][qh_] >> 1) : S.hy[1][qw_][qh_];
                        int so_x = (int16_t)(-(sw >> 1) + pcx), so_y = (int16_t)(-(sh >> 1) + pcy);
                        clamp_area(bx0, padl, pwl, so_x, sw);
                        clamp_area(by0, padl, phl, so_y, sh);
                        S.qp[t][0] = so_x, S.qp[t][1] = so_y, S.qp[t][2] = sw, S.qp[t][3] = sh;
                    }
                    __syncthreads();
                    if (lw == LCU && lvl == 1)
                        hme_pass_q<8, 16, 4>(S, S.qsrc, 32, R.quarter, R.pitch_quarter, bx0, by0, nq, t);
                    else if (lw == LCU)
                        hme_pass_q<16, 32, 8>(S, S.src, 2 * LCU, R.full, R.pitch_full, bx0, by0, nq, t);
                    else
                        hme_pass(S, lvl, lvl == 1 ? R.quarter : R.full, lvl == 1 ? R.pitch_quarter : R.pitch_full, bx0, by0,
                                 lw >> shf, lvl == 1 ? 16 : 32, nq, t);
                    if (t < nq) {
                        const unsigned long long k = S.hkey[t];
                        const int qx = S.qp[t][0], qy = S.qp[t][1], qwv = S.qp[t][2];
                        const int p = (int)(uint32_t)k, sy = p / qwv, sx = p - sy * qwv;
                        S.hx[lvl][qw_][qh_] = (int16_t)((int16_t)(sx + qx) * (1 << shf));
                        S.hy[lvl][qw_][qh_] = (int16_t)((int16_t)(sy + qy) * (1 << shf));
                        S.hs[lvl][qw_][qh_] = (k >> 32) * 2;
                    }
                    if (lvl == 2 || !P.enable_hme_level2)
                        __syncthreads();
                }
                {
                    int hx = 0, hy = 0;
                    unsigned long long hsv = 0;
                    const int l0only = P.enable_hme_level0 && !P.enable_hme_level1 && !P.enable_hme_level2;
                    const int sel = P.enable_hme_level2 ? 2 : (P.enable_hme_level1 ? 1 : (l0only ? 0 : -1));
                    if (sel >= 0) {
                        hx = S.hx[sel][0][0], hy = S.hy[sel][0][0], hsv = S.hs[sel][0][0];
                        if (!(sel == 0 && P.one_quadrant_hme))
                            for (int h = 0; h < nh; h++)
                                for (int w = (h == 0 ? 1 : 0); w < nw; w++)
                                    if (S.hs[sel][w][h] < hsv)
                                        hx = S.hx[sel][w][h], hy = S.hy[sel][w][h], hsv = S.hs[sel][w][h];
                    }
                    if (sel == 2 && P.ref_pocs_equal && list == 1 && nh * nw > 1) {
                        __syncthreads();
                        if (t == 0) {
                            const int total = nh * nw;
                            for (int q = 0; q < total - 1; q++)
                                for (int r = q + 1; r < total; r++) {
                                    const int qa = q / nw, qb = q % nw, ra = r / nw, rb = r % nw;
                                    if (S.hs[2][qa][qb] > S.hs[2][ra][rb]) {
                                        const int16_t tx = S.hx[2][qa][qb], ty = S.hy[2][qa][qb];
                                        const unsigned long long ts = S.hs[2][qa][qb];
                                        S.hx[2][qa][qb] = S.hx[2][ra][rb], S.hy[2][qa][qb] = S.hy[2][ra][rb], S.hs[2][qa][qb] = S.hs[2][ra][rb];
                                        S.hx[2][ra][rb] = tx, S.hy[2][ra][rb] = ty, S.hs[2][ra][rb] = ts;
                                    }
                                }
                        }
                        __syncthreads();
                        hx = S.hx[2][0][1], hy = S.hy[2][0][1];
                    }
                    cx = hx, cy = hy;
                }
            }
        }
        const int hcx = cx, hcy = cy;

        STAMP(3);
        if (cx != 0 || cy != 0) {
            if (P.update_hme_search_center) {
                cx = clamp_center(ox, cx, LCU - 1, W);
                cy = clamp_center(oy, cy, LCU - 1, H);
            }
            if (t == 0) {
                S.cand[0][2] = 0, S.cand[0][3] = 0;
                S.cand[1][2] = cx, S.cand[1][3] = cy;
            }
            __syncthreads();
            lcu_sads(S, R.full, R.pitch_full, ox, oy, lw, lh, 2, t, zero_sad_valid);
            const uint32_t zeroSad = S.acc[0] << 1, hmeSad = S.acc[1] << 1;
            const unsigned long long zeroCost = (unsigned long long)zeroSad << COST_PRECISION;
            const uint32_t rate = mvd_fraction_bits(abs(cx << 2), abs(cy << 2), S.mvd_bits);
            const unsigned long long hmeCost = (unsigned long long)(uint32_t)(hmeSad << COST_PRECISION) +
                                               ((((unsigned long long)P.lambda * rate) + MD_OFFSET) >> MD_SHIFT);
            if (zeroCost <= hmeCost)
                cx = 0, cy = 0;
            __syncthreads();
        }

        if (t == 0) {
            carry->cx[list] = cx, carry->cy[list] = cy;
            carry->hme_init_done = hme_init_done;
            o->hme_center_x[list] = (int16_t)hcx, o->hme_center_y[list] = (int16_t)hcy;
            if (P.num_lists == 1)
                o->hme_center_x[1] = 0, o->hme_center_y[1] = 0;
        }
        if (t < 12) {
            (&carry->hx[0][0][0])[t] = (&S.hx[0][0][0])[t];
            (&carry->hy[0][0][0])[t] = (&S.hy[0][0][0])[t];
            (&carry->hs[0][0][0])[t] = (&S.hs[0][0][0])[t];
        }
        STAMP(4);
    } else {
        cx = carry->cx[list], cy = carry->cy[list];
        int saw = imin(P.search_area_width, 127), sah = imin(P.search_area_height, 127);
        int sox = cx - (saw >> 1), soy = cy - (sah >> 1);
        clamp_area(ox, LCU - 1, W, sox, saw);
        clamp_area(oy, LCU - 1, H, soy, sah);
        const int wx0 = ox + sox - 2, wy0 = oy + soy - 2, wx1 = ox + sox + saw + 65, wy1 = oy + soy + sah + 65;
        int win_off;
        {
            const uint4 sv = *(const u128u_w *)(cur.full + (ptrdiff_t)(oy + (t >> 2)) * pf + ox + ((t & 3) << 4));
            uint32_t i_sad = 0, i_mv = 0;
            if (list && t < 85)
                i_sad = o->best_sad[0][t], i_mv = o->best_mv[0][t];
            const int wa = me_f_pitch(wx1 - (wx0 - 2));
            const int n16 = wa >> 4, rows = wy1 - wy0, total = rows * n16;
            const uint32_t rc = (1u << 20) / (uint32_t)n16 + 1u;
            const int hp_off = ME_SEARCH_BYTES + (method == SVT_AMD_SSD_SEARCH ? ME_SEARCH_SSD_BYTES : 0);
            uint8_t *dst = g_pool + hp_off + 3 * (wy1 - wy0) * me_hp_pitch(wx1 - (wx0 & ~3));
            wF.p = dst, wF.x0 = wx0 - 2, wF.y0 = wy0, wF.stride = wa;
            uint4 fw[ME_F_ITEMS];
#pragma unroll
            for (int k = 0; k < ME_F_ITEMS; k++) {
                const int i = t + k * NT;
                if (i < total) {
                    const int r = (int)(((uint32_t)i * rc) >> 20), c = i - r * n16;
                    fw[k] = ldu16(R.full + (ptrdiff_t)(wy0 + r) * R.pitch_full + (wx0 - 2) + c * 16);
                }
            }
            *(uint4 *)&S.src[(t >> 2) * LCU + ((t & 3) << 4)] = sv;
            if (t < 85) {
                B.best_sad[list][t] = 0, B.best_mv[list][t] = 0, B.dir[list][t] = 0;
                B.best_sad[1 - list][t] = i_sad, B.best_mv[1 - list][t] = i_mv;
                B.dir[1 - list][t] = 0;
                if (method == SVT_AMD_SSD_SEARCH)
                    BS.best_ssd[list][t] = 0, BS.best_ssd[1 - list][t] = 0;
                B.bipred[t] = 0;
                B.key[t] = 0xffffffffu;
            }
            if (t == 0)
                B.key64 = ~0ull;
#pragma unroll
            for (int k = 0; k < ME_F_ITEMS; k++) {
                const int i = t + k * NT;
                if (i < total) {
                    const int r = (int)(((uint32_t)i * rc) >> 20), c = i - r * n16;
                    uint32_t *d4 = (uint32_t *)(dst + r * wa + c * 16);
                    d4[0] = fw[k].x, d4[1] = fw[k].y, d4[2] = fw[k].z, d4[3] = fw[k].w;
                }
            }
            for (int i = t + ME_F_ITEMS * NT; i < total; i += NT) {
                const int r = (int)(((uint32_t)i * rc) >> 20), c = i - r * n16;
                const uint4 v = ldu16(R.full + (ptrdiff_t)(wy0 + r) * R.pitch_full + (wx0 - 2) + c * 16);
                uint32_t *d4 = (uint32_t *)(dst + r * wa + c * 16);
                d4[0] = v.x, d4[1] = v.y, d4[2] = v.z, d4[3] = v.w;
            }
            win_off = hp_off;
        }
        LDS_BARRIER();

        STAMP(6);
        {
            const int mult8 = saw & ~7;
            const int q = t >> 6, lane = t & 63, grp = lane >> 4, blk = lane & 15;
            const int bx = ((q & 1) << 5) + (((blk & 1) | (((blk >> 2) & 1) << 1)) << 3);
            const int by = ((q >> 1) << 5) + ((((blk >> 1) & 1) | (((blk >> 3) & 1) << 1)) << 3);
            uint32_t s0[4], s1[4];
#pragma unroll
            for (int r = 0; r < 4; r++) {
                s0[r] = *(const uint32_t *)&S.src[(by + 2 * r) * LCU + bx];
                s1[r] = *(const uint32_t *)&S.src[(by + 2 * r) * LCU + bx + 4];
            }
            STAMP(13);
            load_windows3_async(wB, wH, wJ, win_off, R.hp_b, R.hp_h, R.hp_j, R.pitch_full, wx0, wy0, wx1, wy1, t);
#if ME_EXP >= 10
            STAMP(15);
#endif
            const uint32_t *rb4 = (const uint32_t *)wat(wF, ox + bx + sox, oy + by + soy);
            const int fs4 = wF.stride >> 2;
            const int mcount = (saw + 3) >> 2;
            const int rows_per_chunk = imax(1, imin(sah, 256 / saw));
            const uint32_t rcm = fastdiv_recip((uint32_t)mcount), rcs = fastdiv_recip((uint32_t)saw);
            uint32_t best8 = 0xffffffffu, best16 = 0xffffffffu, best32 = 0xffffffffu;
            const int slot = blk & 3;
            const bool fast = (saw & 3) == 0;
            const int sh16 = (slot & 1) ? 0 : 16;
            const int q4 = 4 / mcount, r4 = 4 - q4 * mcount;
            uint32_t b8[4] = {0xffffffffu, 0xffffffffu, 0xffffffffu, 0xffffffffu}, b16 = 0xffffffffu;
            for (int row0 = 0; row0 < sah; row0 += rows_per_chunk) {
                const int nrows = imin(rows_per_chunk, sah - row0), items = nrows * mcount, pbase = row0 * saw;
                if (fast) {
                    int mi = (int)grp, ry = 0;
                    while (mi >= mcount)
                        mi -= mcount, ry++;
                    int ro = (row0 + ry) * fs4 + mi;
                    uint32_t itg = (uint32_t)(row0 * mcount) + (uint32_t)grp;
                    uint32_t cur[12], nxt[12];
#pragma unroll
                    for (int rr = 0; rr < 4; rr++)
                        cur[3 * rr] = rb4[ro + 2 * rr * fs4], cur[3 * rr + 1] = rb4[ro + 2 * rr * fs4 + 1], cur[3 * rr + 2] = rb4[ro + 2 * rr * fs4 + 2];
                    for (int it0 = 0; it0 < items; it0 += 4) {
                        const bool live = it0 + (int)grp < items;
                        {
                            int nmi = mi + r4, nro = ro + q4 * fs4 + r4;
                            if (nmi >= mcount)
                                nmi -= mcount, nro += fs4 - mcount;
                            const bool more = it0 + 4 + (int)grp < items;
                            mi = more ? nmi : mi, ro = more ? nro : ro;
#pragma unroll
                            for (int rr = 0; rr < 4; rr++)
                                nxt[3 * rr] = rb4[ro + 2 * rr * fs4], nxt[3 * rr + 1] = rb4[ro + 2 * rr * fs4 + 1], nxt[3 * rr + 2] = rb4[ro + 2 * rr * fs4 + 2];
                        }
                        unsigned long long acc = 0;
#pragma unroll
                        for (int rr = 0; rr < 4; rr++) {
                            acc = qsad(cur[3 * rr], cur[3 * rr + 1], s0[rr], acc);
                            acc = qsad(cur[3 * rr + 1], cur[3 * rr + 2], s1[rr], acc);
                        }
#pragma unroll
                        for (int k = 0; k < 12; k++)
                            cur[k] = nxt[k];
                        uint32_t lo = live ? (uint32_t)acc : 0xffffffffu, hi = live ? (uint32_t)(acc >> 32) : 0xffffffffu;
                        b8[0] = umin32(b8[0], (lo << 16) | itg), b8[1] = umin32(b8[1], (lo & 0xffff0000u) | itg);
                        b8[2] = umin32(b8[2], (hi << 16) | itg), b8[3] = umin32(b8[3], (hi & 0xffff0000u) | itg);
                        lo += (uint32_t)__builtin_amdgcn_update_dpp(0, (int)lo, 0xB1, 0xF, 0xF, true);
                        hi += (uint32_t)__builtin_amdgcn_update_dpp(0, (int)hi, 0xB1, 0xF, 0xF, true);
                        lo += (uint32_t)__builtin_amdgcn_update_dpp(0, (int)lo, 0x4E, 0xF, 0xF, true);
                        hi += (uint32_t)__builtin_amdgcn_update_dpp(0, (int)hi, 0x4E, 0xF, 0xF, true);
                        const uint32_t sel = slot < 2 ? lo : hi;
                        const uint32_t k16 = live ? (((sel << sh16) & 0xffff0000u) | itg) : 0xffffffffu;
                        b16 = umin32(b16, k16);
                        uint32_t v = (sel >> (16 - sh16)) & 0xffffu;
                        v += (uint32_t)__builtin_amdgcn_update_dpp(0, (int)v, 0x124, 0xF, 0xF, true);
                        v += (uint32_t)__builtin_amdgcn_update_dpp(0, (int)v, 0x128, 0xF, 0xF, true);
                        const uint32_t pk = 4u * itg + (uint32_t)slot;
                        const uint32_t k32 = live ? ((v << 14) | pk) : 0xffffffffu;
                        best32 = umin32(best32, k32);
                        if (live && blk < 4)
                            B.sad32[(int)pk - pbase][q] = v;
                        itg += 4;
                    }
                } else
                for (int it0 = 0; it0 < items; it0 += 4) {
                    const int it = it0 + grp;
                    const bool live = it < items;
                    const int ry = live ? (int)fastdiv((uint32_t)it, rcm) : 0, mi = live ? it - ry * mcount : 0, sy = row0 + ry;
                    const uint32_t *r = rb4 + sy * fs4 + mi;
                    unsigned long long acc = 0;
#pragma unroll
                    for (int rr = 0; rr < 4; rr++) {
                        const uint32_t d0 = r[0], d1 = r[1], d2 = r[2];
                        acc = qsad(d0, d1, s0[rr], acc);
                        acc = qsad(d1, d2, s1[rr], acc);
                        r += 2 * fs4;
                    }
                    const int p0 = sy * saw + 4 * mi;
                    uint32_t lo = (uint32_t)acc, hi = (uint32_t)(acc >> 32);
#pragma unroll
                    for (int k = 0; k < 4; k++) {
                        const uint32_t sv = ((k < 2 ? lo : hi) >> (16 * (k & 1))) & 0xffffu;
                        const uint32_t key = (live && 4 * mi + k < saw) ? ((sv << 14) | (uint32_t)(p0 + k)) : 0xffffffffu;
                        best8 = key < best8 ? key : best8;
                    }
                    lo += (uint32_t)__builtin_amdgcn_update_dpp(0, (int)lo, 0xB1, 0xF, 0xF, true);
                    hi += (uint32_t)__builtin_amdgcn_update_dpp(0, (int)hi, 0xB1, 0xF, 0xF, true);
                    lo += (uint32_t)__builtin_amdgcn_update_dpp(0, (int)lo, 0x4E, 0xF, 0xF, true);
                    hi += (uint32_t)__builtin_amdgcn_update_dpp(0, (int)hi, 0x4E, 0xF, 0xF, true);
                    uint32_t v = ((slot < 2 ? lo : hi) >> (16 * (slot & 1))) & 0xffffu;
                    const bool valid = live && 4 * mi + slot < saw;
                    const uint32_t pk = (uint32_t)(p0 + slot);
                    {
                        const uint32_t key = valid ? ((v << 14) | pk) : 0xffffffffu;
                        best16 = key < best16 ? key : best16;
                    }
                    v += (uint32_t)__builtin_amdgcn_update_dpp(0, (int)v, 0x124, 0xF, 0xF, true);
                    v += (uint32_t)__builtin_amdgcn_update_dpp(0, (int)v, 0x128, 0xF, 0xF, true);
                    {
                        const uint32_t key = valid ? ((v << 14) | pk) : 0xffffffffu;
                        best32 = key < best32 ? key : best32;
                    }
                    if (valid && blk < 4)
                        B.sad32[(int)pk - pbase][q] = v;
                }
#if ME_EXP >= 10
                STAMP(0);
#endif
                LDS_BARRIER();
                {
                    const int p = pbase + t;
                    unsigned long long k64 = ~0ull;
                    if (t < nrows * saw) {
                        const uint4 sq = *(const uint4 *)&B.sad32[t][0];
                        const uint32_t s = sq.x + sq.y + sq.z + sq.w;
                        const int sy = (int)fastdiv((uint32_t)p, rcs), sx = p - sy * saw;
                        const uint32_t code = (sx < mult8) ? (uint32_t)(16383 - p) : (0x4000u | (uint32_t)p);
                        k64 = ((unsigned long long)s << 15) | code;
                    }
                    if (q * 64 < nrows * saw) {
                        k64 = wave_min64(k64);
                        if (lane == 0)
                            atomicMin(&B.key64, k64);
                    }
                }
                LDS_BARRIER();
            }
#if ME_EXP >= 10
            STAMP(1);
#endif
            if (fast) {
#pragma unroll
                for (int k = 0; k < 4; k++)
                    if (b8[k] != 0xffffffffu)
                        best8 = umin32(best8, ((b8[k] >> 16) << 14) | (4u * (b8[k] & 0xffffu) + (uint32_t)k));
                if (b16 != 0xffffffffu)
                    best16 = ((b16 >> 16) << 14) | (4u * (b16 & 0xffffu) + (uint32_t)slot);
            }
            best8 = umin32(best8, (uint32_t)__shfl_xor((int)best8, 16));
            best8 = umin32(best8, (uint32_t)__shfl_xor((int)best8, 32));
#pragma unroll
            for (int o = 1; o <= 2; o <<= 1)
                best16 = umin32(best16, (uint32_t)__shfl_xor((int)best16, o));
            best16 = umin32(best16, (uint32_t)__shfl_xor((int)best16, 16));
            best16 = umin32(best16, (uint32_t)__shfl_xor((int)best16, 32));
#pragma unroll
            for (int o = 1; o <= 32; o <<= 1)
                best32 = umin32(best32, (uint32_t)__shfl_xor((int)best32, o));
            if (grp == 0)
                B.key[21 + ((q << 4) | blk)] = best8;
            if (grp == 0 && (blk & 3) == 0)
                B.key[5 + ((q << 2) | (blk >> 2))] = best16;
            if (lane == 0)
                B.key[1 + q] = best32;
            LDS_BARRIER();
#if ME_EXP >= 10
            STAMP(2);
#endif
            int vx = 0, vy = 0, vs = 0;
            if (t < 85) {
                uint32_t s;
                int p;
                if (t == 0) {
                    const unsigned long long k = B.key64;
                    const uint32_t code = (uint32_t)(k & 0x7fff);
                    s = (uint32_t)(k >> 15);
                    p = (code & 0x4000u) ? (int)(code & 0x3fff) : 16383 - (int)code;
                } else {
                    const uint32_t k = B.key[t];
                    s = k >> 14;
                    p = (int)(k & 0x3fff);
                }
                const int sy = (int)fastdiv((uint32_t)p, rcs), sx = p - sy * saw;
                const uint32_t mv = mvpack((sx + sox) * 4, (sy + soy) * 4);
                B.best_sad[list][t] = 2 * s;
                B.best_mv[list][t] = mv;
                vx = mvx(mv), vy = mvy(mv), vs = (int)(2 * s);
            }
            if (P.fractional_search_model == 1 && t < 128) {
                const bool in8 = t >= 21 && t < 85;
                const int s8x = (int)wave_sum((uint32_t)(in8 ? vx : 0)), s8y = (int)wave_sum((uint32_t)(in8 ? vy : 0)), s8s = (int)wave_sum((uint32_t)(in8 ? vs : 0));
                if (t < 64) {
                    const bool in32 = t >= 1 && t < 5, in16 = t >= 5 && t < 21;
                    const int s32x = (int)wave_sum((uint32_t)(in32 ? vx : 0)), s32y = (int)wave_sum((uint32_t)(in32 ? vy : 0)), s32s = (int)wave_sum((uint32_t)(in32 ? vs : 0));
                    const int s16x = (int)wave_sum((uint32_t)(in16 ? vx : 0)), s16y = (int)wave_sum((uint32_t)(in16 ? vy : 0)), s16s = (int)wave_sum((uint32_t)(in16 ? vs : 0));
                    if (t == 0) {
                        B.sums[0] = s32x, B.sums[1] = s32y, B.sums[2] = s32s;
                        B.sums[3] = s16x, B.sums[4] = s16y, B.sums[5] = s16s;
                        B.sums[6] = s8x, B.sums[7] = s8y, B.sums[8] = s8s;
                    }
                } else if (t == 64) {
                    B.sums[9] = s8x, B.sums[10] = s8y, B.sums[11] = s8s;
                }
            }
            STAMP(14);
            __builtin_amdgcn_s_waitcnt(0);
            __syncthreads();
        }

        STAMP(7);
        int e32 = 0, e16 = 0, e8 = 0, eq = 0;
        if (P.fractional_search_model == 0) {
            e32 = e16 = e8 = eq = 1;
        } else if (P.fractional_search_model == 1) {
            const int sx32 = B.sums[0], sy32 = B.sums[1], ss32 = B.sums[2], ss16 = B.sums[5];
            const int sx8 = B.sums[6] + B.sums[9], sy8 = B.sums[7] + B.sums[10], ss8 = B.sums[8] + B.sums[11];
            const uint32_t ux32 = (uint32_t)(sx32 >> 2), uy32 = (uint32_t)(sy32 >> 2), ux8 = (uint32_t)(sx8 >> 6), uy8 = (uint32_t)(sy8 >> 6);
            const uint32_t mag32 = ux32 * ux32 + uy32 * uy32, mag8 = ux8 * ux8 + uy8 * uy8;
            const uint32_t avg32 = (uint32_t)ss32 >> 2, avg16 = (uint32_t)ss16 >> 4, avg8 = (uint32_t)ss8 >> 6;
            const int tl = P.temporal_layer_index;
            const uint32_t th = tl == 0 ? 48 * 48 : tl == 1 ? 32 * 32 : tl == 2 ? 80 * 80 : 48 * 48;
            const int small32 = mag32 < th, low32 = avg32 < 32 * 32 * 6;
            e32 = (tl == 0 || tl == 2) ? low32 : (tl == 1 ? (small32 ? low32 : 1) : (small32 ? 1 : low32));
            e16 = !(avg16 < 16 * 16 * 2);
            e8 = (tl <= 2) ? !(avg8 < 8 * 8 * 2) : ((mag8 < th) ? !(avg8 < 8 * 8 * 2) : 0);
            eq = 1;
        }
        e16 = e16 && P.cu16x16_mode == 0, e8 = e8 && P.cu8x8_mode != 1;
        const int any_sub = e32 || e16 || e8 || eq || 0;
        const int run_sub = (P.fractional_search_model != 2) && any_sub;
        if (run_sub) {
            const int f64 = P.fractional_search_64x64;
            const int en0 = f64, en1 = e32, en2 = e16, en3 = e8;
#define EN(tier_) pick4(tier_, en0, en1, en2, en3)
            const int rstep = (method == SVT_AMD_SUB_SAD_SEARCH) ? 2 : 1;
            STAMP(8);
            for (int tier = 0; tier < 4; tier++) {
                if (!EN(tier))
                    continue;
                const int sz = tier_sz_of(tier), rows = sz >> (rstep - 1), lc = tier_lc_of(tier), rpc = rows >> lc;
                const int items = tier_cnt_of(tier) * 8 << lc;
                for (int i = t; i < items; i += NT) {
                    const int ch = i & ((1 << lc) - 1), k = (i >> lc) & 7, n = tier_first_of(tier) + (i >> (lc + 3));
                    int px_, py_, psz;
                    pu_geom_z(n, px_, py_, psz);
                    const uint32_t mv = B.best_mv[list][n];
                    const LWin &pl = (k < 2) ? wB : (k < 4 ? wH : wJ);
                    const int ddx = (k == 1 || k == 5 || k == 6) ? 1 : 0, ddy = (k == 3 || k == 6 || k == 7) ? 1 : 0;
                    const int y0 = ch * rpc * rstep;
                    const uint8_t *r = wat(pl, ox + px_ + (mvx(mv) >> 2) + ddx, oy + py_ + (mvy(mv) >> 2) + y0 + ddy);
                    const uint8_t *sp = &S.src[(py_ + y0) * LCU + px_];
                    uint32_t d = 0, sd = 0;
                    const int lgspr = tier == 0 ? 2 : tier == 1 ? 1 : 0, nseg = rpc << lgspr, rs = pl.stride * rstep;
                    for (int s0_ = 0; s0_ < nseg; s0_ += 4) {
                        uint32_t sv[4][4], rv[4][4];
#pragma unroll
                        for (int q_ = 0; q_ < 4; q_++) {
                            const int sg = s0_ + q_, rr = sg >> lgspr, x = (sg & ((1 << lgspr) - 1)) << 4;
                            if (sz >= 16) {
                                const uint4 v4 = *(const uint4 *)(sp + rr * (LCU * rstep) + x);
                                sv[q_][0] = v4.x, sv[q_][1] = v4.y, sv[q_][2] = v4.z, sv[q_][3] = v4.w;
                                lds_ld_unaligned<4>(r + rr * rs + x, rv[q_]);
                            } else {
                                const uint2 v2 = *(const uint2 *)(sp + rr * (LCU * rstep));
                                uint32_t w2[2];
                                lds_ld_unaligned<2>(r + rr * rs, w2);
                                sv[q_][0] = v2.x, sv[q_][1] = v2.y, rv[q_][0] = w2[0], rv[q_][1] = w2[1];
                                sv[q_][2] = sv[q_][3] = rv[q_][2] = rv[q_][3] = 0;
                            }
                        }
#pragma unroll
                        for (int q_ = 0; q_ < 4; q_++) {
                            row_metric(method, sv[q_][0], rv[q_][0], d, sd);
                            row_metric(method, sv[q_][1], rv[q_][1], d, sd);
                            if (sz >= 16) {
                                row_metric(method, sv[q_][2], rv[q_][2], d, sd);
                                row_metric(method, sv[q_][3], rv[q_][3], d, sd);
                            }
                        }
                    }
                    d = group_sum_rt(d, lc);
                    if (method == SVT_AMD_SSD_SEARCH)
                        sd = group_sum_rt(sd, lc);
                    if (ch == 0) {
                        B.dist[n][k] = d;
                        if (method == SVT_AMD_SSD_SEARCH)
                            BS.dsad[n][k] = sd;
                    }
                }
            }
            if (method == SVT_AMD_SSD_SEARCH) {
                for (int tier = 0; tier < 4; tier++) {
                    if (!EN(tier))
                        continue;
                    const int sz = tier_sz_of(tier), items = tier_cnt_of(tier) * sz;
                    for (int i = t; i < items; i += NT) {
                        const int row = i % sz, n = tier_first_of(tier) + i / sz;
                        int px_, py_, psz;
                        pu_geom_z(n, px_, py_, psz);
                        const uint32_t mv = B.best_mv[list][n];
                        const uint8_t *r = wat(wF, ox + px_ + (mvx(mv) >> 2), oy + py_ + (mvy(mv) >> 2) + row);
                        const uint8_t *s = &S.src[(py_ + row) * LCU + px_];
                        uint32_t d = 0;
                        for (int x = 0; x < sz; x += 8) {
                            uint32_t v[2];
                            lds_ld_unaligned<2>(r + x, v);
                            d += ssd4(*(const uint32_t *)(s + x), v[0]) + ssd4(*(const uint32_t *)(s + x + 4), v[1]);
                        }
                        atomicAdd(&BS.best_ssd[list][n], d);
                    }
                }
            }
            __syncthreads();
            if (t < 85) {
                const int tier = t == 0 ? 0 : t < 5 ? 1 : t < 21 ? 2 : 3;
                if (EN(tier)) {
                    const int mdx[8] = {-2, 2, 0, 0, -2, 2, 2, -2}, mdy[8] = {0, 0, -2, 2, -2, -2, 2, 2};
                    const uint32_t mv0 = B.best_mv[list][t];
                    uint32_t bsad = B.best_sad[list][t], bmv = mv0, bssd = method == SVT_AMD_SSD_SEARCH ? BS.best_ssd[list][t] : 0u;
                    uint32_t dmin = 0xffffffffu;
                    for (int k = 0; k < 8; k++) {
                        const uint32_t d = (method == SVT_AMD_SUB_SAD_SEARCH) ? (B.dist[t][k] << 1) : B.dist[t][k];
                        dmin = d < dmin ? d : dmin;
                        if (method == SVT_AMD_SSD_SEARCH) {
                            if (d < bssd)
                                bsad = BS.dsad[t][k], bmv = mvpack(mvx(mv0) + mdx[k], mvy(mv0) + mdy[k]), bssd = d;
                        } else if (d < bsad) {
                            bsad = d, bmv = mvpack(mvx(mv0) + mdx[k], mvy(mv0) + mdy[k]);
                        }
                    }
                    const int chk[8] = {0, 1, 2, 3, 4, 5, 7, 6};
                    const uint8_t code[8] = {D_L, D_R, D_T, D_B, D_TL, D_TR, D_BR, D_BL};
                    uint8_t dirv = 0;
                    for (int i = 7; i >= 0; i--) {
                        const uint32_t d = (method == SVT_AMD_SUB_SAD_SEARCH) ? (B.dist[t][chk[i]] << 1) : B.dist[t][chk[i]];
                        if (d == dmin)
                            dirv = code[chk[i]];
                    }
                    B.best_sad[list][t] = bsad, B.best_mv[list][t] = bmv;
                    if (method == SVT_AMD_SSD_SEARCH)
                        BS.best_ssd[list][t] = bssd;
                    B.dir[list][t] = dirv;
                }
            }
            __syncthreads();

            STAMP(9);
            const int qen0 = f64, qen1 = eq && e32, qen2 = eq && e16, qen3 = eq && e8;
#define QEN(tier_) pick4(tier_, qen0, qen1, qen2, qen3)
            int qcum[5];
            qcum[0] = 0;
#pragma unroll
            for (int tier = 0; tier < 4; tier++)
                qcum[tier + 1] = qcum[tier] + (QEN(tier) ? (((tier_cnt_of(tier) * 3 << (tier == 0 ? 3 : tier_lc_of(tier))) + 63) & ~63) : 0);
            {
                for (int i0 = 0; i0 < qcum[4]; i0 += NT) {
                    const int i = i0 + t;
                    if (i >= qcum[4])
                        continue;
                    const int tier = __builtin_amdgcn_readfirstlane(i < qcum[1] ? 0 : i < qcum[2] ? 1 : i < qcum[3] ? 2 : 3);
                    const int sz = tier == 0 ? 32 : tier_sz_of(tier);
                    const int lc = tier == 0 ? 3 : tier_lc_of(tier), rows = sz >> (rstep - 1), rpc = rows >> lc;
                    const int items = tier_cnt_of(tier) * 3 << lc, ti = i - pick4(tier, qcum[0], qcum[1], qcum[2], qcum[3]);
                    const bool live = ti < items;
                    const int ii = live ? ti : 0;
                    const int ch = ii & ((1 << lc) - 1), pj = ii >> lc, pidx = pj / 3, j = pj - pidx * 3;
                    const int n = tier_first_of(tier) + pidx;
                    int px_, py_, psz;
                    pu_geom_z(n, px_, py_, psz);
                    const uint32_t mv = B.best_mv[list][n];
                    const int xMv = mvx(mv), yMv = mvy(mv);
                    const int qm = (yMv & 2) + ((xMv & 2) >> 1);
                    const int code = (B.dir[list][n] + j - 1 + (qm ? 4 : 0)) & 7;
                    const int k = (int)((0x07361524u >> (4 * code)) & 7u);
                    const int y = ch * rpc * rstep;
                    const int ax = ox + px_ + ((xMv + 2) >> 2), ay = oy + py_ + ((yMv + 2) >> 2) + y;
                    const QSrc q0 = c_qtab[qm][k][0], q1 = c_qtab[qm][k][1];
                    const LWin &w1 = q0.plane == 0 ? wF : q0.plane == 1 ? wB : q0.plane == 2 ? wH : wJ;
                    const LWin &w2 = q1.plane == 0 ? wF : q1.plane == 1 ? wB : q1.plane == 2 ? wH : wJ;
                    const uint8_t *r1 = wat(w1, ax + q0.dx, ay + q0.dy);
                    const uint8_t *r2 = wat(w2, ax + q1.dx, ay + q1.dy);
                    const uint8_t *sp = &S.src[(py_ + y) * LCU + px_];
                    uint32_t d = 0, sdv = 0;
                    if (live) {
                        const int lgspr = sz == 32 ? 1 : 0, nseg = rpc << lgspr, rs1 = w1.stride * rstep, rs2 = w2.stride * rstep;
                        for (int s0_ = 0; s0_ < nseg; s0_ += 4) {
                            uint32_t sv[4][4], v1[4][4], v2[4][4];
#pragma unroll
                            for (int q_ = 0; q_ < 4; q_++) {
                                const int sg = s0_ + q_, rr = sg >> lgspr, x = (sg & ((1 << lgspr) - 1)) << 4;
                                const bool inside_y = (py_ + y + rr * rstep) < lh, in0 = inside_y && (px_ + x) < lw, in1 = inside_y && (px_ + x + 8) < lw;
                                if (sz >= 16) {
                                    const uint4 v4 = *(const uint4 *)(sp + rr * (LCU * rstep) + x);
                                    sv[q_][0] = in0 ? v4.x : 0u, sv[q_][1] = in0 ? v4.y : 0u, sv[q_][2] = in1 ? v4.z : 0u, sv[q_][3] = in1 ? v4.w : 0u;
                                    lds_ld_unaligned<4>(r1 + rr * rs1 + x, v1[q_]);
                                    lds_ld_unaligned<4>(r2 + rr * rs2 + x, v2[q_]);
                                } else {
                                    const uint2 s2 = *(const uint2 *)(sp + rr * (LCU * rstep));
                                    uint32_t a2[2], b2[2];
                                    lds_ld_unaligned<2>(r1 + rr * rs1, a2);
                                    lds_ld_unaligned<2>(r2 + rr * rs2, b2);
                                    sv[q_][0] = in0 ? s2.x : 0u, sv[q_][1] = in0 ? s2.y : 0u, v1[q_][0] = a2[0], v1[q_][1] = a2[1], v2[q_][0] = b2[0], v2[q_][1] = b2[1];
                                    sv[q_][2] = sv[q_][3] = v1[q_][2] = v1[q_][3] = v2[q_][2] = v2[q_][3] = 0;
                                }
                            }
#pragma unroll
                            for (int q_ = 0; q_ < 4; q_++) {
                                row_metric(method, sv[q_][0], avg4(v1[q_][0], v2[q_][0]), d, sdv);
                                row_metric(method, sv[q_][1], avg4(v1[q_][1], v2[q_][1]), d, sdv);
                                if (sz >= 16) {
                                    row_metric(method, sv[q_][2], avg4(v1[q_][2], v2[q_][2]), d, sdv);
                                    row_metric(method, sv[q_][3], avg4(v1[q_][3], v2[q_][3]), d, sdv);
                                }
                            }
                        }
                    }
                    d = group_sum_rt(d, lc);
                    if (method == SVT_AMD_SSD_SEARCH)
                        sdv = group_sum_rt(sdv, lc);
                    if (live && ch == 0) {
                        B.dist[n][k] = d;
                        if (method == SVT_AMD_SSD_SEARCH)
                            BS.dsad[n][k] = sdv;
                    }
                }
            }
            __syncthreads();
            if (t < 85) {
                const int tier = t == 0 ? 0 : t < 5 ? 1 : t < 21 ? 2 : 3;
                if (QEN(tier)) {
                    const int mdx[8] = {-1, 1, 0, 0, -1, 1, 1, -1}, mdy[8] = {0, 0, -1, 1, -1, -1, 1, 1};
                    const int kcode[8] = {D_L, D_R, D_T, D_B, D_TL, D_TR, D_BR, D_BL};
                    const uint32_t mv0 = B.best_mv[list][t];
                    const int qm = (mvy(mv0) & 2) + ((mvx(mv0) & 2) >> 1);
                    const int sd = B.dir[list][t];
                    uint32_t bsad = B.best_sad[list][t], bmv = mv0, bssd = method == SVT_AMD_SSD_SEARCH ? BS.best_ssd[list][t] : 0u;
                    for (int k = 0; k < 8; k++) {
                        const int target = qm ? ((kcode[k] + 4) & 7) : kcode[k];
                        const int diff = (sd - target) & 7;
                        if (!(diff == 0 || diff == 1 || diff == 7))
                            continue;
                        const uint32_t d = (method == SVT_AMD_SUB_SAD_SEARCH) ? (B.dist[t][k] << 1) : B.dist[t][k];
                        if (method == SVT_AMD_SSD_SEARCH) {
                            if (d < bssd)
                                bsad = BS.dsad[t][k], bmv = mvpack(mvx(mv0) + mdx[k], mvy(mv0) + mdy[k]), bssd = d;
                        } else if (d < bsad) {
                            bsad = d, bmv = mvpack(mvx(mv0) + mdx[k], mvy(mv0) + mdy[k]);
                        }
                    }
                    B.best_sad[list][t] = bsad, B.best_mv[list][t] = bmv;
                    if (method == SVT_AMD_SSD_SEARCH)
                        BS.best_ssd[list][t] = bssd;
                }
            }
            __syncthreads();
        }
        if (t < 85) {
            o->best_sad[list][t] = B.best_sad[list][t];
            o->best_mv[list][t] = B.best_mv[list][t];
            if (P.num_lists == 1)
                o->best_sad[1][t] = 0, o->best_mv[1][t] = 0;
        }
        if (t == 0) {
            o->search_origin_x[list] = (int16_t)sox, o->search_origin_y[list] = (int16_t)soy;
            o->search_w[list] = (uint8_t)saw, o->search_h[list] = (uint8_t)sah;
            if (P.num_lists == 1)
                o->search_origin_x[1] = 0, o->search_origin_y[1] = 0, o->search_w[1] = 0, o->search_h[1] = 0;
        }
        if (list != P.num_lists - 1) {
            STAMP(12);
            return;
        }

    STAMP(10);
    if (P.num_lists == 2) {
        const int rstep = (method == SVT_AMD_SUB_SAD_SEARCH) ? 2 : 1;
        const int npu = (P.cu16x16_mode != 0) ? 5 : ((P.cu8x8_mode != 0) ? 21 : 85);
        int cum[5];
        cum[0] = 0;
#pragma unroll
        for (int tier = 0; tier < 4; tier++) {
            const int sz = tier_sz_of(tier), rows = sz >> (rstep - 1), segs = sz >= 16 ? sz >> 4 : 1;
            cum[tier + 1] = cum[tier] + (tier_first_of(tier) < npu ? tier_cnt_of(tier) * rows * segs : 0);
        }
        for (int base = 0; base < cum[4]; base += ME_BI_ITEMS * NT) {
            uint4 va0[ME_BI_ITEMS], vb0[ME_BI_ITEMS], va1[ME_BI_ITEMS], vb1[ME_BI_ITEMS];
            int in_[ME_BI_ITEMS], ij[ME_BI_ITEMS], iG[ME_BI_ITEMS], iw[ME_BI_ITEMS];
            const uint8_t *is[ME_BI_ITEMS];
#pragma unroll
            for (int u = 0; u < ME_BI_ITEMS; u++) {
                const int i = base + u * NT + t;
                iG[u] = 0;
                if (i < cum[4]) {
            const int tier = i < cum[1] ? 0 : i < cum[2] ? 1 : i < cum[3] ? 2 : 3;
                    const int sz = tier_sz_of(tier), rows = sz >> (rstep - 1), lgsegs = tier == 0 ? 2 : tier == 1 ? 1 : 0, wseg = sz >= 16 ? 16 : sz;
                    const int j = i - pick4(tier, cum[0], cum[1], cum[2], cum[3]);
                    const int lgrows = 6 - tier - (rstep == 2 ? 1 : 0);
                    const int seg = j & ((1 << lgsegs) - 1), jr = j >> lgsegs, row = jr & (rows - 1), n = tier_first_of(tier) + (jr >> lgrows);
                    int px_, py_, psz;
                    pu_geom_z(n, px_, py_, psz);
                    const int y = row * rstep, xs = seg << 4;
                    {
                        const uint32_t mv = B.best_mv[0][n];
                        const int xMv = mvx(mv), yMv = mvy(mv);
                        const int ax = ox + px_ + xs + (xMv >> 2), ay = oy + py_ + (yMv >> 2) + y;
                        const uint32_t frac = (uint32_t)((xMv & 3) + ((yMv & 3) << 2));
                        const ptrdiff_t pz = ref0.pitch_full;
                        const uint32_t pa = (0xBAFA5450u >> (2 * frac)) & 3u, pb = (0x54BEBA14u >> (2 * frac)) & 3u;
                        const ptrdiff_t at = (ptrdiff_t)ay * pz + ax;
                        const uint8_t *ba = pa == 0 ? ref0.full : pa == 1 ? ref0.hp_b : pa == 2 ? ref0.hp_h : ref0.hp_j;
                        const uint8_t *bb = pb == 0 ? ref0.full : pb == 1 ? ref0.hp_b : pb == 2 ? ref0.hp_h : ref0.hp_j;
                        const uint8_t *a0p = ba + at + (pa & 1u) + ((pa >> 1) ? pz : 0) + ((0x8000u >> frac) & 1u);
                        const uint8_t *b0p = bb + at + (pb & 1u) + ((pb >> 1) ? pz : 0) + ((0x0888u >> frac) & 1u) + (((0xF000u >> frac) & 1u) ? pz : 0);
                        va0[u] = ldu16(a0p);
                        vb0[u] = va0[u];
                        if (b0p != a0p)
                            vb0[u] = ldu16(b0p);
                    }
                    {
                        const uint32_t mv = B.best_mv[1][n];
                        const int xMv = mvx(mv), yMv = mvy(mv);
                        const int ax = ox + px_ + xs + (xMv >> 2), ay = oy + py_ + (yMv >> 2) + y;
                        const uint32_t frac = (uint32_t)((xMv & 3) + ((yMv & 3) << 2));
                        const uint32_t pa = (0xBAFA5450u >> (2 * frac)) & 3u, pb = (0x54BEBA14u >> (2 * frac)) & 3u;
                        const uint8_t *wpa = pa == 0 ? wF.p : pa == 1 ? wB.p : pa == 2 ? wH.p : wJ.p, *wpb = pb == 0 ? wF.p : pb == 1 ? wB.p : pb == 2 ? wH.p : wJ.p;
                        const int sa = pa == 0 ? wF.stride : wB.stride, sb = pb == 0 ? wF.stride : wB.stride;
                        const int xa0 = pa == 0 ? wF.x0 : wB.x0, xb0 = pb == 0 ? wF.x0 : wB.x0;
                        const uint8_t *a1p = wpa + (ay + (int)(pa >> 1) - wF.y0) * sa + (ax + (int)(pa & 1u) + (int)((0x8000u >> frac) & 1u) - xa0);
                        const uint8_t *b1p = wpb + (ay + (int)(pb >> 1) + (int)((0xF000u >> frac) & 1u) - wF.y0) * sb + (ax + (int)(pb & 1u) + (int)((0x0888u >> frac) & 1u) - xb0);
                        uint32_t w4[4];
                        lds_ld_unaligned<4>(a1p, w4);
                        va1[u] = make_uint4(w4[0], w4[1], w4[2], w4[3]);
                        vb1[u] = va1[u];
                        if (b1p != a1p) {
                            lds_ld_unaligned<4>(b1p, w4);
                            vb1[u] = make_uint4(w4[0], w4[1], w4[2], w4[3]);
                        }
                    }
                    const int per_pu = rows << lgsegs;
                    in_[u] = n, ij[u] = j, iG[u] = per_pu < 64 ? per_pu : 64, iw[u] = wseg;
                    is[u] = &S.src[(py_ + y) * LCU + px_ + xs];
                }
            }
#pragma unroll
            for (int u = 0; u < ME_BI_ITEMS; u++) {
                if (!iG[u])
                    continue;
                const uint4 a0 = va0[u], b0 = vb0[u], a1 = va1[u], b1 = vb1[u];
                uint32_t d = 0;
                if (iw[u] == 16) {
                    const uint4 sv = *(const uint4 *)is[u];
                    d = sad4(sv.x, avg4(avg4(a0.x, b0.x), avg4(a1.x, b1.x)), d);
                    d = sad4(sv.y, avg4(avg4(a0.y, b0.y), avg4(a1.y, b1.y)), d);
                    d = sad4(sv.z, avg4(avg4(a0.z, b0.z), avg4(a1.z, b1.z)), d);
                    d = sad4(sv.w, avg4(avg4(a0.w, b0.w), avg4(a1.w, b1.w)), d);
                } else {
                    const uint2 sv = *(const uint2 *)is[u];
                    d = sad4(sv.x, avg4(avg4(a0.x, b0.x), avg4(a1.x, b1.x)), d);
                    d = sad4(sv.y, avg4(avg4(a0.y, b0.y), avg4(a1.y, b1.y)), d);
                }
                const int G = iG[u];
                d = group_sum_rt(d, 31 - __builtin_clz((unsigned)G));
                if ((ij[u] & (G - 1)) == 0)
                    atomicAdd(&B.bipred[in_[u]], d);
            }
        }
        __syncthreads();
    }

    STAMP(11);
    if (t < 85) {
        const int pu = t;
        const int n = pu == 0 ? 0 : pu < 5 ? pu : pu < 21 ? c_tab16[pu - 5] + 5 : c_tab8[pu - 21] + 21;
        int total = P.num_lists;
        if (P.num_lists == 2 && (P.cu8x8_mode == 0 || pu < 21) && (P.cu16x16_mode == 0 || pu < 5))
            total = 3;
        const uint32_t bi = (method == SVT_AMD_SUB_SAD_SEARCH) ? (B.bipred[n] << 1) : B.bipred[n];
        const uint32_t v[3] = {B.best_sad[0][n], B.best_sad[1][n], bi};
        SvtAmdMeCuResult r;
        r.x_mv_l0 = (int16_t)mvx(B.best_mv[0][n]), r.y_mv_l0 = (int16_t)mvy(B.best_mv[0][n]);
        r.x_mv_l1 = (int16_t)mvx(B.best_mv[1][n]), r.y_mv_l1 = (int16_t)mvy(B.best_mv[1][n]);
        r.total_me_candidate_index = (uint8_t)total;
        for (int k = 0; k < 3; k++)
            r.distortion[k] = 0, r.direction[k] = 0;
        const uint32_t a = v[0], b = v[1], c = v[2];
        if (total == 3) {
            int o0, o1, o2;
            if (a <= b && a <= c) {
                o0 = 0;
                if (b <= c) o1 = 1, o2 = 2; else o1 = 2, o2 = 1;
            } else if (b <= a && b <= c) {
                o0 = 1;
                if (a <= c) o1 = 0, o2 = 2; else o1 = 2, o2 = 0;
            } else if (a <= b) {
                o0 = 2, o1 = 0, o2 = 1;
            } else {
                o0 = 2, o1 = 1, o2 = 0;
            }
            r.distortion[0] = o0 == 0 ? a : o0 == 1 ? b : c, r.direction[0] = (uint8_t)o0;
            r.distortion[1] = o1 == 0 ? a : o1 == 1 ? b : c, r.direction[1] = (uint8_t)o1;
            r.distortion[2] = o2 == 0 ? a : o2 == 1 ? b : c, r.direction[2] = (uint8_t)o2;
        } else if (total == 2) {
            const int f = a <= b ? 0 : 1;
            r.distortion[0] = f ? b : a, r.direction[0] = (uint8_t)f;
            r.distortion[1] = f ? a : b, r.direction[1] = (uint8_t)(1 - f);
        } else {
            r.distortion[0] = a, r.direction[0] = SVT_AMD_UNI_PRED_LIST_0;
        }
        o->pu[pu] = r;
    }
    STAMP(12);
    }
}

static void me_pool_bytes(const SvtAmdMeParams *p, size_t *hme_pool, size_t *search_pool)
{
    auto win = [](int w, int blk, int h, int brows) {
        int pitch = ((w > 1 ? w : 1) + blk + 30) & ~15;
        if (!((pitch >> 4) & 1))
            pitch += 16;
        return (size_t)pitch * (size_t)((h > 1 ? h : 1) + 2 * (brows - 1) + 1);
    };
    size_t need = 0;
    const int nw = p->num_hme_regions_w, nh = p->num_hme_regions_h;
    if (p->enable_hme_flag) {
        for (int lvl = 0; lvl <= 2; lvl++) {
            if (!(lvl == 0 ? p->enable_hme_level0 : lvl == 1 ? p->enable_hme_level1 : p->enable_hme_level2))
                continue;
            const int one = lvl == 0 && p->one_quadrant_hme && !p->enable_hme_level1 && !p->enable_hme_level2;
            const int blk = 16 << lvl, brows = 8 << lvl;
            size_t v = 0, last = 0;
            for (int h = 0; h < (one ? 1 : nh); h++)
                for (int w = 0; w < (one ? 1 : nw); w++) {
                    int sw, sh;
                    if (lvl == 0) {
                        sw = (int)(((one ? p->hme_l0_total_w : p->hme_l0_w[w & 1]) * p->hme_l0_mult_x) / 100);
                        sh = (int)(((one ? p->hme_l0_total_h : p->hme_l0_h[h & 1]) * p->hme_l0_mult_y) / 100);
                    } else {
                        const int rw = lvl == 1 ? p->hme_l1_w[w & 1] : p->hme_l2_w[w & 1];
                        sw = (rw < 8) ? 8 : (rw & 7) ? rw + (rw - ((rw >> 3) << 3)) : rw;
                        sh = lvl == 1 ? p->hme_l1_h[h & 1] : p->hme_l2_h[h & 1];
                    }
                    v += last;
                    last = win(sw, blk, sh, brows);
                }
            v += (last + 1023) & ~(size_t)1023;
            need = v > need ? v : need;
        }
    }
    *hme_pool = (need + 64 + 255) & ~(size_t)255;
    const int saw = p->search_area_width > 127 ? 127 : p->search_area_width;
    const int sah = p->search_area_height > 127 ? 127 : p->search_area_height;
    const size_t rows = (size_t)sah + 67;
    const size_t fwin = ((size_t)me_f_pitch(saw + 69) * rows + 15) & ~(size_t)15, hwin = (size_t)me_hp_pitch(saw + 67 + 3) * rows;
    const size_t ssd = p->fractional_search_method == SVT_AMD_SSD_SEARCH ? (size_t)ME_SEARCH_SSD_BYTES : 0;
    *search_pool = ((size_t)ME_SEARCH_BYTES + ssd + fwin + 3 * hwin + 64 + 255) & ~(size_t)255;
}

static size_t g_me_last_lds[2];
extern "C" int svt_amd_debug_me_kernel_lds_bytes(const SvtAmdMeParams *p, int phase)
{
    if (phase != 0 && phase != 1)
        return SVT_AMD_ERR_BAD_PARAM;
    if (!p)
        return (int)g_me_last_lds[phase];
    size_t pool[2];
    me_pool_bytes(p, &pool[0], &pool[1]);
    return (int)(pool[phase] + (phase ? sizeof(MeSearchShared) : sizeof(MeShared)));
}

int svt_amd_me_kernel_occupancy(const SvtAmdMeParams *p, int phase, int *workgroups_per_cu, int *private_bytes)
{
    if (!p || (phase != 0 && phase != 1) || !workgroups_per_cu || !private_bytes)
        return SVT_AMD_ERR_BAD_PARAM;
    size_t pool[2];
    me_pool_bytes(p, &pool[0], &pool[1]);
    const void *fn = phase ? (const void *)k_me<1> : (const void *)k_me<0>;
    hipFuncAttributes fa;
    HIP_TRY(hipFuncGetAttributes(&fa, fn));
    int n = 0;
    HIP_TRY(hipOccupancyMaxActiveBlocksPerMultiprocessor(&n, fn, NT, pool[phase]));
    *workgroups_per_cu = n, *private_bytes = (int)fa.localSizeBytes;
    return SVT_AMD_OK;
}

int svt_amd_launch_me_batch(SvtAmdContext *ctx, const MeJobDev *host_jobs, int njobs, int max_lcus)
{
    if (njobs < 1 || njobs > SVT_AMD_MAX_BATCH)
        return SVT_AMD_ERR_BAD_PARAM;
    size_t pool0 = 0, pool1 = 0;
    int max_lists = 1;
    for (int i = 0; i < njobs; i++) {
        size_t a, b;
        me_pool_bytes(&host_jobs[i].P, &a, &b);
        pool0 = a > pool0 ? a : pool0;
        pool1 = b > pool1 ? b : pool1;
        max_lists = host_jobs[i].P.num_lists > max_lists ? host_jobs[i].P.num_lists : max_lists;
    }
    if (pool1 + sizeof(MeSearchShared) > 160 * 1024 || pool0 + sizeof(MeShared) > 160 * 1024) {
        svt_amd_set_error("motion estimation: search windows need %zu B of LDS (> 160 KiB)", pool1 + sizeof(MeSearchShared));
        return SVT_AMD_ERR_BAD_PARAM;
    }
    {
        static std::mutex mu;
        static size_t attr0[64], attr1[64], stat0[64], stat1[64];
        std::lock_guard<std::mutex> g(mu);
        const int dv = ctx->device & 63;
        if (!stat1[dv]) {
            hipFuncAttributes fa0, fa1;
            HIP_TRY(hipFuncGetAttributes(&fa0, (const void *)k_me<0>));
            HIP_TRY(hipFuncGetAttributes(&fa1, (const void *)k_me<1>));
            stat0[dv] = fa0.sharedSizeBytes, stat1[dv] = fa1.sharedSizeBytes;
        }
        g_me_last_lds[0] = stat0[dv] + pool0, g_me_last_lds[1] = stat1[dv] + pool1;
        if (pool0 > attr0[dv]) {
            HIP_TRY(hipFuncSetAttribute((const void *)k_me<0>, hipFuncAttributeMaxDynamicSharedMemorySize, (int)pool0));
            attr0[dv] = pool0;
        }
        if (pool1 > attr1[dv]) {
            HIP_TRY(hipFuncSetAttribute((const void *)k_me<1>, hipFuncAttributeMaxDynamicSharedMemorySize, (int)pool1));
            attr1[dv] = pool1;
        }
    }
    {
        const int rcd = svt_amd_upload_descriptors(ctx, ctx->d_jobs, host_jobs, sizeof(MeJobDev) * (size_t)njobs);
        if (rcd)
            return rcd;
    }
    int rc = svt_amd_stamp_begin(ctx, KC_ME_SEARCH);
    if (rc)
        return rc;
    const dim3 grid((unsigned)((max_lcus + 7) & ~7), (unsigned)njobs);
    for (int list = 0; list < max_lists; list++) {
        hipLaunchKernelGGL(k_me<0>, grid, dim3(NT), pool0, svt_amd_ctx_stream(ctx), ctx->d_jobs, list);
        hipLaunchKernelGGL(k_me<1>, grid, dim3(NT), pool1, svt_amd_ctx_stream(ctx), ctx->d_jobs, list);
    }
    HIP_TRY(hipGetLastError());
    return svt_amd_stamp_end(ctx);
}
```

svt-hevc_amd/csrc/svt_amd_internal.h:

```cpp
#ifndef SVT_AMD_INTERNAL_H
#define SVT_AMD_INTERNAL_H

#include <hip/hip_runtime.h>
#include <stdint.h>
#include "../../include/svt_hevc_amd.h"
#include "slot_records.h"

static inline int svt_amd_lcu_count(int w, int h) { return ((w + 63) / 64) * ((h + 63) / 64); }

struct DevPlane {
    uint8_t *origin;
    int32_t  pitch;
    int32_t  width, height, pad;
    uint8_t *alloc;
    size_t   alloc_bytes;
    int32_t  lead_rows;
    int32_t  lead_cols;
};

struct DevPicture {
    DevPlane full, quarter, sixteenth, hp_b, hp_h, hp_j;
    SvtAmdMeLcuResult *d_me_out;
    SvtAmdOisLcuResult *d_ois_out;
    void *d_me_carry;
    uint8_t *d_staging;
    size_t   staging_bytes;
    uint8_t *h_staging;
    uint8_t *d_pack;
    size_t pack_bytes;
    hipEvent_t ev_ready;
    SlotRecords rec;
    uint16_t width, height;
    int      valid;
};

struct PicView {
    const uint8_t *full, *quarter, *sixteenth, *hp_b, *hp_h, *hp_j;
    int32_t pitch_full, pitch_quarter, pitch_sixteenth;
};

enum { KC_PREP = 0, KC_ME_SEARCH = 1, KC_OIS = 2, KC_COUNT = 3 };

#define SVT_AMD_MAX_BATCH 256

struct MeJobDev {
    SvtAmdMeParams P;
    PicView cur, ref0, ref1;
    SvtAmdMeLcuResult *out;
    struct MeCarry *carry;
    int32_t lcu_begin, lcu_count;
    unsigned long long *dbg_clock;
};

struct OisJobDev {
    SvtAmdOisParams P;
    const uint8_t *full;
    int32_t pitch, lcus_w, nlcu;
    const SvtAmdMeLcuResult *me;
    SvtAmdOisLcuResult *out;
};

struct PackSrc {
    const uint32_t *me, *ois;
};

enum SvtAmdBatchEntry { BATCH_SIDE, BATCH_CHROMA, BATCH_DETECT, BATCH_NOISE, BATCH_SBO, BATCH_MDC, BATCH_IRC, BATCH_MDCTL, BATCH_ENTRIES };

struct SvtAmdContext {
    int device;
    SvtAmdContext *parent;
    hipStream_t stream;
    int stream_failed;
    uint16_t max_w, max_h;
    int num_slots;
    DevPicture *slots;
    hipEvent_t ev_begin, ev_end;
    int timer_armed;
    struct Stamp { hipEvent_t a, b; int cls; } *stamps;
    int num_stamps, cap_stamps;
    SvtAmdMeLcuResult *d_me_scratch;
    void *d_prep_jobs;
    OisJobDev *d_ois_jobs;
    MeJobDev *d_jobs;
    unsigned long long *d_dbg;
    size_t dbg_slots;
    void *d_cabac_cost;
    uint8_t *d_leaf_scratch;
    size_t leaf_scratch_bytes;
    SvtAmdMeLcuResult *h_me;
    SvtAmdOisLcuResult *h_ois;
    hipEvent_t ev_done;
    int frontend_busy;
    hipEvent_t ev_user[8];
    uint8_t *h_desc_ring;
    hipEvent_t ev_desc[8];
    int desc_next;
    hipEvent_t ev_launch[16];
    int launch_next;
    unsigned long long mark_records, mark_waits;
    void *d_pack_src;
    void *d_batch[BATCH_ENTRIES];
    void *d_tmvp;
    void *comm;
    int comm_world, comm_rank;
    uint8_t *d_xchg;
    size_t xchg_bytes;
};

int svt_amd_upload_descriptors(SvtAmdContext *ctx, void *d_dst, const void *src, size_t bytes);
int svt_amd_ctx_scratch(SvtAmdContext *ctx, size_t bytes, uint8_t **out);
const void *svt_amd_registered_device_ptr(const void *h_ptr, size_t bytes);

const void *svt_amd_slot_records(SvtAmdContext *root, int slot, int which, int w, int h);
int svt_amd_records_wait(SvtAmdContext *ctx, DevPicture *s, int which, hipEvent_t *seen, int *nseen, int cap);
int svt_amd_records_read_mark(SvtAmdContext *ctx, SvtAmdContext *root, int slot);

void svt_amd_set_error(const char *fmt, ...);

int svt_amd_mdctl_check_async(SvtAmdContext *ctx, const SvtAmdMdLcu *d_lcus, int n, int depth_mode, int inter, SvtAmdMdCtlCheck *h_out);

hipStream_t svt_amd_ctx_stream(SvtAmdContext *ctx);
static inline bool svt_amd_ctx_has_stream(const SvtAmdContext *ctx) { return ctx->stream != nullptr; }
static inline hipError_t svt_amd_ctx_sync(SvtAmdContext *ctx)
{
    return ctx->stream || ctx->stream_failed ? hipStreamSynchronize(ctx->stream) : hipSuccess;
}
#define HIP_TRY(expr)                                                                      \
    do {                                                                                   \
        hipError_t e_ = (expr);                                                            \
        if (e_ != hipSuccess) {                                                            \
            svt_amd_set_error("%s failed: %s (%s:%d)", #expr, hipGetErrorString(e_),       \
                              __FILE__, __LINE__);                                         \
            return SVT_AMD_ERR_DEVICE;                                                     \
        }                                                                                  \
    } while (0)

int svt_amd_stamp_begin(SvtAmdContext *ctx, int cls);
int svt_amd_stamp_end(SvtAmdContext *ctx);

int svt_amd_launch_prep(SvtAmdContext *ctx, DevPicture *pic, const uint8_t *d_luma, uint32_t stride);
int svt_amd_launch_prep_batch(SvtAmdContext *ctx, DevPicture *const *pics, const uint8_t *const *d_luma, uint32_t stride,
                              int n);
int svt_amd_launch_me_batch(SvtAmdContext *ctx, const MeJobDev *host_jobs, int njobs, int max_lcus);
int svt_amd_me_kernel_occupancy(const SvtAmdMeParams *p, int phase, int *workgroups_per_cu, int *private_bytes);
int svt_amd_launch_zz_sad(SvtAmdContext *ctx, const DevPicture *cur, const DevPicture *prev, SvtAmdZzLcu *d_out);
int svt_amd_launch_ois_batch(SvtAmdContext *ctx, const struct OisJobDev *host_jobs, int njobs, int max_lcus);

static inline PicView make_view(const DevPicture *p)
{
    PicView v;
    v.full = p->full.origin;
    v.quarter = p->quarter.origin;
    v.sixteenth = p->sixteenth.origin;
    v.hp_b = p->hp_b.origin;
    v.hp_h = p->hp_h.origin;
    v.hp_j = p->hp_j.origin;
    v.pitch_full = p->full.pitch;
    v.pitch_quarter = p->quarter.pitch;
    v.pitch_sixteenth = p->sixteenth.pitch;
    return v;
}

#endif
```

Before: 4803 fps.

## Pack ME params into control words, raise HME occupancy, uniformize wave indices

```diff
diff --git a/include/svt_hevc_amd.h b/include/svt_hevc_amd.h
--- a/include/svt_hevc_amd.h
+++ b/include/svt_hevc_amd.h
@@ -1565,6 +1565,7 @@
 SVT_AMD_API int svt_amd_debug_me_kernel_lds_bytes(const SvtAmdMeParams *params, int phase);
 SVT_AMD_API int svt_amd_debug_me_kernel_occupancy(SvtAmdContext *ctx, const SvtAmdMeParams *params, int phase, int *workgroups_per_cu, int *private_bytes);
 SVT_AMD_API int svt_amd_debug_launch_markers(SvtAmdContext *ctx, unsigned long long *records, unsigned long long *waits);
+SVT_AMD_API int svt_amd_debug_me_controls_roundtrip(const SvtAmdMeParams *in, SvtAmdMeParams *out, uint32_t *words, int max_words);
 
 #ifdef __cplusplus
 }
diff --git a/svt-hevc_amd/csrc/context.hip b/svt-hevc_amd/csrc/context.hip
--- a/svt-hevc_amd/csrc/context.hip
+++ b/svt-hevc_amd/csrc/context.hip
@@ -748,6 +748,20 @@
     return SVT_AMD_OK;
 }
 
+extern "C" int svt_amd_debug_me_controls_roundtrip(const SvtAmdMeParams *in, SvtAmdMeParams *out, uint32_t *words, int max_words)
+{
+    if (!in || !out || (words && max_words < ME_CTL_WORDS))
+        return SVT_AMD_ERR_BAD_PARAM;
+    uint32_t ctl[ME_CTL_WORDS];
+    me_ctl_pack(in, ctl);
+    memset(out, 0, sizeof(*out));
+    me_ctl_unpack(ctl, out);
+    memcpy(out->mvd_bits, in->mvd_bits, sizeof(out->mvd_bits));
+    for (int i = 0; words && i < ME_CTL_WORDS; i++)
+        words[i] = ctl[i];
+    return ME_CTL_WORDS;
+}
+
 static int make_job(SvtAmdContext *ctx, const SvtAmdMeParams *params, int cur_slot, const int ref_slot[2],
                     uint32_t lcu_begin, uint32_t lcu_end, MeJobDev *job)
 {
@@ -763,6 +777,7 @@
     const DevPicture *r0 = &ctx->slots[ref_slot[0]];
     const DevPicture *r1 = params->num_lists == 2 ? &ctx->slots[ref_slot[1]] : r0;
     job->P = *params;
+    me_ctl_pack(params, job->ctl);
     job->cur = make_view(c);
     job->ref0 = make_view(r0);
     job->ref1 = make_view(r1);
diff --git a/svt-hevc_amd/csrc/me_controls.h b/svt-hevc_amd/csrc/me_controls.h
--- /dev/null
+++ b/svt-hevc_amd/csrc/me_controls.h
@@ -0,0 +1,98 @@
+#ifndef SVT_AMD_ME_CONTROLS_H
+#define SVT_AMD_ME_CONTROLS_H
+#include <stdint.h>
+#include "../../include/svt_hevc_amd.h"
+
+#define ME_CTL_WORDS 16
+
+#define ME_CTL_FIELDS(X)                                                       \
+    X(luma_width,               luma_width,               0,   0,    16,   0)  \
+    X(luma_height,              luma_height,              0,   16,   16,   0)  \
+    X(num_lists,                num_lists,                1,   0,    8,    0)  \
+    X(temporal_layer_index,     temporal_layer_index,     1,   8,    8,    0)  \
+    X(search_area_width,        search_area_width,        1,   16,   8,    0)  \
+    X(search_area_height,       search_area_height,       1,   24,   8,    0)  \
+    X(fractional_search_method, fractional_search_method, 2,   0,    8,    0)  \
+    X(fractional_search_model,  fractional_search_model,  2,   8,    8,    0)  \
+    X(fractional_search_64x64,  fractional_search_64x64,  2,   16,   8,    0)  \
+    X(cu8x8_mode,               cu8x8_mode,               2,   24,   8,    0)  \
+    X(cu16x16_mode,             cu16x16_mode,             3,   0,    8,    0)  \
+    X(update_hme_search_center, update_hme_search_center, 3,   8,    8,    0)  \
+    X(enable_hme_flag,          enable_hme_flag,          3,   16,   8,    0)  \
+    X(ref_pocs_equal,           ref_pocs_equal,           3,   24,   8,    0)  \
+    X(enable_hme_level0,        enable_hme_level0,        4,   0,    8,    0)  \
+    X(enable_hme_level1,        enable_hme_level1,        4,   8,    8,    0)  \
+    X(enable_hme_level2,        enable_hme_level2,        4,   16,   8,    0)  \
+    X(one_quadrant_hme,         one_quadrant_hme,         4,   24,   8,    0)  \
+    X(num_hme_regions_w,        num_hme_regions_w,        5,   0,    8,    0)  \
+    X(num_hme_regions_h,        num_hme_regions_h,        5,   8,    8,    0)  \
+    X(hme_l0_total_w,           hme_l0_total_w,           5,   16,   16,   0)  \
+    X(hme_l0_total_h,           hme_l0_total_h,           6,   0,    16,   0)  \
+    X(hme_l0_mult_x,            hme_l0_mult_x,            6,   16,   16,   0)  \
+    X(hme_l0_mult_y,            hme_l0_mult_y,            7,   0,    16,   0)  \
+    X(hme_l0_w0,                hme_l0_w[0],              7,   16,   16,   0)  \
+    X(hme_l0_w1,                hme_l0_w[1],              8,   0,    16,   0)  \
+    X(hme_l0_h0,                hme_l0_h[0],              8,   16,   16,   0)  \
+    X(hme_l0_h1,                hme_l0_h[1],              9,   0,    16,   0)  \
+    X(hme_l1_w0,                hme_l1_w[0],              9,   16,   16,   0)  \
+    X(hme_l1_w1,                hme_l1_w[1],              10,  0,    16,   0)  \
+    X(hme_l1_h0,                hme_l1_h[0],              10,  16,   16,   0)  \
+    X(hme_l1_h1,                hme_l1_h[1],              11,  0,    16,   0)  \
+    X(hme_l2_w0,                hme_l2_w[0],              11,  16,   16,   0)  \
+    X(hme_l2_w1,                hme_l2_w[1],              12,  0,    16,   0)  \
+    X(hme_l2_h0,                hme_l2_h[0],              12,  16,   16,   0)  \
+    X(hme_l2_h1,                hme_l2_h[1],              13,  0,    16,   0)  \
+    X(lambda,                   lambda,                   14,  0,    32,   0)
+
+#if defined(__HIPCC__) || defined(__CUDACC__)
+#define ME_CTL_FN __host__ __device__ __forceinline__
+#else
+#define ME_CTL_FN static inline
+#endif
+
+ME_CTL_FN uint32_t me_ctl_mask(int width) { return width >= 32 ? 0xffffffffu : (1u << width) - 1u; }
+ME_CTL_FN int32_t me_ctl_field(uint32_t word, int shift, int width, int sgn)
+{
+    const uint32_t v = (word >> shift) & me_ctl_mask(width);
+    return sgn && width < 32 && (v >> (width - 1)) ? (int32_t)(v | ~me_ctl_mask(width)) : (int32_t)v;
+}
+
+#define ME_CTL_GETTER(name, member, word, shift, width, sgn) \
+    ME_CTL_FN int32_t me_ctl_##name(const uint32_t *ctl) { return me_ctl_field(ctl[word], shift, width, sgn); }
+ME_CTL_FIELDS(ME_CTL_GETTER)
+#undef ME_CTL_GETTER
+
+static inline void me_ctl_pack(const SvtAmdMeParams *p, uint32_t ctl[ME_CTL_WORDS])
+{
+    for (int i = 0; i < ME_CTL_WORDS; i++)
+        ctl[i] = 0;
+#define ME_CTL_PACK(name, member, word, shift, width, sgn) ctl[word] |= ((uint32_t)p->member & me_ctl_mask(width)) << shift;
+    ME_CTL_FIELDS(ME_CTL_PACK)
+#undef ME_CTL_PACK
+}
+template <typename T> static inline void me_ctl_store(T &member, int32_t v) { member = (T)v; }
+static inline void me_ctl_unpack(const uint32_t ctl[ME_CTL_WORDS], SvtAmdMeParams *p)
+{
+#define ME_CTL_UNPACK(name, member, word, shift, width, sgn) me_ctl_store(p->member, me_ctl_##name(ctl));
+    ME_CTL_FIELDS(ME_CTL_UNPACK)
+#undef ME_CTL_UNPACK
+}
+
+#ifdef __cplusplus
+constexpr bool me_ctl_table_ok()
+{
+    uint32_t used[ME_CTL_WORDS] = {};
+    bool ok = true;
+#define ME_CTL_CHECK(name, member, word, shift, width, sgn)                                                                  \
+    {                                                                                                                        \
+        const uint32_t m = (width >= 32 ? 0xffffffffu : (1u << width) - 1u) << shift;                                        \
+        ok = ok && word < ME_CTL_WORDS && shift + width <= 32 && width == 8 * (int)sizeof(SvtAmdMeParams::member) && !(used[word] & m); \
+        used[word] |= m;                                                                                                     \
+    }
+    ME_CTL_FIELDS(ME_CTL_CHECK)
+#undef ME_CTL_CHECK
+    return ok;
+}
+static_assert(me_ctl_table_ok(), "ME_CTL_FIELDS: a field leaves its word, differs in width from its member, or overlaps another");
+#endif
+#endif
diff --git a/svt-hevc_amd/csrc/me_kernels.hip b/svt-hevc_amd/csrc/me_kernels.hip
--- a/svt-hevc_amd/csrc/me_kernels.hip
+++ b/svt-hevc_amd/csrc/me_kernels.hip
@@ -7,7 +7,7 @@
 #define ME_MIN_WAVES_PER_SIMD 4
 #endif
 #ifndef ME_HME_WAVES_PER_SIMD
-#define ME_HME_WAVES_PER_SIMD 6
+#define ME_HME_WAVES_PER_SIMD 8
 #endif
 #define COST_PRECISION 8
 #define MD_SHIFT 23
@@ -396,6 +396,8 @@
 __device__ __forceinline__ uint32_t fastdiv_recip(uint32_t d) { return (1u << 24) / d + 1u; }
 __device__ __forceinline__ uint32_t fastdiv(uint32_t p, uint32_t r) { return (uint32_t)(((unsigned long long)p * r) >> 24); }
 
+#define HME_POS(sx, sy) (((uint32_t)(sy) << 16) | (uint32_t)(sx))
+
 __device__ __forceinline__ void hme_pass(MeShared &S, int level, const uint8_t *refplane, int pitch, int bx0, int by0, int bw,
                          int rows, int nq, int t)
 {
@@ -428,14 +430,15 @@
         unsigned long long best = ~0ull;
         for (int i0 = 0; i0 < items; i0 += NT) {
             const int p = (i0 + t) >> lg;
-            uint32_t sv = 0;
+            uint32_t sv = 0, pos = 0;
             if (p < npos) {
                 const int sy = (int)fastdiv((uint32_t)p, rc), sx = p - sy * qw;
                 sv = row_sad_lds(srow, wbase + sy * wstride + sx, bw);
+                pos = HME_POS(sx, sy);
             }
             for (int o = rows >> 1; o > 0; o >>= 1)
                 sv += __shfl_xor(sv, o);
-            const unsigned long long k = p < npos ? (((unsigned long long)sv << 32) | (uint32_t)p) : ~0ull;
+            const unsigned long long k = p < npos ? (((unsigned long long)sv << 32) | pos) : ~0ull;
             best = k < best ? k : best;
         }
         best = wave_min64(best);
@@ -467,15 +470,17 @@
     }
     __builtin_amdgcn_s_waitcnt(0);
     __syncthreads();
-    const int wave = t >> 6, lane = t & 63;
-    const int q = wave % nq, slot = wave / nq, nslots = (4 + nq - 1 - q) / nq;
+    const int wave = __builtin_amdgcn_readfirstlane(t >> 6), lane = t & 63;
+    const int q = nq == 1 ? 0 : nq == 2 ? (wave & 1) : wave;
+    const int slot = nq == 1 ? wave : nq == 2 ? (wave >> 1) : 0;
+    const int nslots = nq == 1 ? 4 : nq == 2 ? 2 : 1;
     int off = 0;
     for (int k = 0; k < q; k++) {
-        const int x0k = bx0 + S.qp[k][0];
-        off += (S.qp[k][3] + 2 * (ROWS - 1) + 1) * win_pitch(x0k, x0k + S.qp[k][2] + 4 * G, 1);
-    }
-    const int qw = S.qp[q][2], qh = S.qp[q][3];
-    const int x0 = bx0 + S.qp[q][0], xa = x0 & ~15, wstride = win_pitch(x0, x0 + qw + 4 * G, 1);
+        const int x0k = bx0 + __builtin_amdgcn_readfirstlane(S.qp[k][0]);
+        off += (__builtin_amdgcn_readfirstlane(S.qp[k][3]) + 2 * (ROWS - 1) + 1) * win_pitch(x0k, x0k + __builtin_amdgcn_readfirstlane(S.qp[k][2]) + 4 * G, 1);
+    }
+    const int qw = __builtin_amdgcn_readfirstlane(S.qp[q][2]), qh = __builtin_amdgcn_readfirstlane(S.qp[q][3]);
+    const int x0 = bx0 + __builtin_amdgcn_readfirstlane(S.qp[q][0]), xa = x0 & ~15, wstride = win_pitch(x0, x0 + qw + 4 * G, 1);
     const int bo0 = x0 - xa;
     const int m0 = bo0 >> 2, mcount = ((bo0 + qw - 1) >> 2) - m0 + 1;
     const int items = qh * mcount * C;
@@ -518,7 +523,7 @@
             for (int k = 0; k < 4; k++) {
                 const int sx = 4 * (m0 + mi) + k - bo0;
                 if (sx >= 0 && sx < qw) {
-                    const unsigned long long key = ((unsigned long long)sd[k] << 32) | (uint32_t)(sy * qw + sx);
+                    const unsigned long long key = ((unsigned long long)sd[k] << 32) | HME_POS(sx, sy);
                     best = key < best ? key : best;
                 }
             }
@@ -569,21 +574,25 @@
     const int blk = (int)(blockIdx.x & 7) * per_xcd + (int)(blockIdx.x >> 3);
     if ((int)(blockIdx.x >> 3) >= per_xcd || blk >= J.lcu_count)
         return;
-    const SvtAmdMeParams &P = J.P;
-    if (list >= P.num_lists)
+    uint32_t ctlw[ME_CTL_WORDS];
+#pragma unroll
+    for (int i = 0; i < ME_CTL_WORDS; i++)
+        ctlw[i] = J.ctl[i];
+#define CTL(f) me_ctl_##f(ctlw)
+    if (list >= CTL(num_lists))
         return;
     const PicView cur = J.cur;
     const PicView &ref0 = J.ref0, &ref1 = J.ref1;
     SvtAmdMeLcuResult *__restrict__ out = J.out;
     const int lcu_begin = J.lcu_begin;
     const int t = threadIdx.x;
-    const int W = P.luma_width, H = P.luma_height;
+    const int W = CTL(luma_width), H = CTL(luma_height);
     const int wl = (W + LCU - 1) / LCU;
     const int lcu = lcu_begin + blk;
     const int ox = (lcu % wl) * LCU, oy = (lcu / wl) * LCU;
     const int lw = imin(LCU, W - ox), lh = imin(LCU, H - oy);
     const int pf = cur.pitch_full;
-    const int method = P.fractional_search_method;
+    const int method = CTL(fractional_search_method);
     MeCarry *__restrict__ carry = &J.carry[lcu];
     SvtAmdMeLcuResult *o = &out[lcu];
     MeSearch &B = *(MeSearch *)g_pool;
@@ -595,12 +604,12 @@
     int cx = 0, cy = 0;
     const uint32_t mv64_l0 = (PHASE == 0 && list) ? o->best_mv[0][0] : 0u;
     auto tsab_cand = [&](int c, int &ux, int &uy, int &kx, int &ky) {
-        ux = c == 1 ? -(int)P.hme_l0_total_w : c == 2 ? (int)P.hme_l0_total_w : c == 5 ? 0 - (mvx(mv64_l0) >> 2) : 0;
-        uy = c == 3 ? -(int)P.hme_l0_total_h : c == 4 ? (int)P.hme_l0_total_h : c == 5 ? 0 - (mvy(mv64_l0) >> 2) : 0;
+        ux = c == 1 ? -(int)CTL(hme_l0_total_w) : c == 2 ? (int)CTL(hme_l0_total_w) : c == 5 ? 0 - (mvx(mv64_l0) >> 2) : 0;
+        uy = c == 3 ? -(int)CTL(hme_l0_total_h) : c == 4 ? (int)CTL(hme_l0_total_h) : c == 5 ? 0 - (mvy(mv64_l0) >> 2) : 0;
         ux = (int16_t)ux, uy = (int16_t)uy;
         kx = c ? clamp_center(ox, ux, LCU - 1, W) : 0, ky = c ? clamp_center(oy, uy, LCU - 1, H) : 0;
     };
-    const bool tsab_early = PHASE == 0 && (P.temporal_layer_index > 0 || list == 0) && P.update_hme_search_center && lw == LCU;
+    const bool tsab_early = PHASE == 0 && (CTL(temporal_layer_index) > 0 || list == 0) && CTL(update_hme_search_center) && lw == LCU;
     const int tsab_nc = list == 1 ? 6 : 5;
     uint4 tsab_b[3];
     if constexpr (PHASE == 0) {
@@ -639,7 +648,7 @@
                 ld4(cur.sixteenth + (ptrdiff_t)((oy >> 2) + 2 * y) * cur.pitch_sixteenth + (ox >> 2) + x);
         }
         if (t >= 64 && t < 76)
-            S.mvd_bits[t - 64] = P.mvd_bits[t - 64];
+            S.mvd_bits[t - 64] = J.P.mvd_bits[t - 64];
         if (t < 12) {
             (&S.hx[0][0][0])[t] = list ? (&carry->hx[0][0][0])[t] : (int16_t)0;
             (&S.hy[0][0][0])[t] = list ? (&carry->hy[0][0][0])[t] : (int16_t)0;
@@ -653,9 +662,9 @@
     if constexpr (PHASE == 0) {
         int hme_init_done = list ? carry->hme_init_done : 0;
         int zero_sad_valid = 0;
-        if (P.temporal_layer_index > 0 || list == 0) {
+        if (CTL(temporal_layer_index) > 0 || list == 0) {
             STAMP(1);
-            if (P.update_hme_search_center) {
+            if (CTL(update_hme_search_center)) {
                 const int nc = tsab_nc;
                 if (t < 6) {
                     int ux, uy, kx, ky;
@@ -695,14 +704,14 @@
             }
 
             STAMP(2);
-            if (P.enable_hme_flag && lh == LCU) {
-                const int nw = P.num_hme_regions_w, nh = P.num_hme_regions_h;
-                const int one = (P.one_quadrant_hme && !P.enable_hme_level1 && !P.enable_hme_level2);
+            if (CTL(enable_hme_flag) && lh == LCU) {
+                const int nw = CTL(num_hme_regions_w), nh = CTL(num_hme_regions_h);
+                const int one = (CTL(one_quadrant_hme) && !CTL(enable_hme_level1) && !CTL(enable_hme_level2));
                 const int nq = nw * nh;
                 const int qh_ = t < 4 ? (nw == 2 ? (t >> 1) : t) : 0, qw_ = t < 4 ? (nw == 2 ? (t & 1) : 0) : 0;
                 if (!hme_init_done) {
                     if (t < nq) {
-                        const int sh0 = P.update_hme_search_center ? 2 : 0, sh1 = P.update_hme_search_center ? 1 : 0;
+                        const int sh0 = CTL(update_hme_search_center) ? 2 : 0, sh1 = CTL(update_hme_search_center) ? 1 : 0;
                         S.hx[0][qw_][qh_] = (int16_t)(cx >> sh0), S.hy[0][qw_][qh_] = (int16_t)(cy >> sh0);
                         S.hx[1][qw_][qh_] = (int16_t)(cx >> sh1), S.hy[1][qw_][qh_] = (int16_t)(cy >> sh1);
                         S.hx[2][qw_][qh_] = (int16_t)cx, S.hy[2][qw_][qh_] = (int16_t)cy;
@@ -710,29 +719,29 @@
                     hme_init_done = 1;
                     __syncthreads();
                 }
-                const uint32_t mx = P.hme_l0_mult_x, my = P.hme_l0_mult_y;
-                if (P.enable_hme_level0) {
+                const uint32_t mx = CTL(hme_l0_mult_x), my = CTL(hme_l0_mult_y);
+                if (CTL(enable_hme_level0)) {
                     const int px16 = ox >> 2, py16 = oy >> 2;
                     const int pw16 = W >> 2, ph16 = H >> 2, pad16 = SVT_AMD_PAD_SIXTEENTH - 1;
                     const int nq0 = one ? 1 : nq;
                     if (t < nq0) {
                         int sw, sh, so_x, so_y;
                         if (one) {
-                            sw = (int16_t)((P.hme_l0_total_w * mx) / 100), sh = (int16_t)((P.hme_l0_total_h * my) / 100);
+                            sw = (int16_t)((CTL(hme_l0_total_w) * mx) / 100), sh = (int16_t)((CTL(hme_l0_total_h) * my) / 100);
                             so_x = -(int)(int16_t)(sw >> 1) + (cx >> 2), so_y = -(int)(int16_t)(sh >> 1) + (cy >> 2);
                             clamp_area(px16, pad16, pw16, so_x, sw);
                             clamp_area(py16, pad16, ph16, so_y, sh);
                             if (sw & 15)
                                 sw = (sw >> 4) << 4;
                         } else {
-                            sw = (int16_t)(((qw_ ? P.hme_l0_w[1] : P.hme_l0_w[0]) * mx) / 100), sh = (int16_t)(((qh_ ? P.hme_l0_h[1] : P.hme_l0_h[0]) * my) / 100);
+                            sw = (int16_t)(((qw_ ? CTL(hme_l0_w1) : CTL(hme_l0_w0)) * mx) / 100), sh = (int16_t)(((qh_ ? CTL(hme_l0_h1) : CTL(hme_l0_h0)) * my) / 100);
                             int dx = cx >> 2, dy = cy >> 2;
                             if (qw_)
-                                dx += (int16_t)((P.hme_l0_w[0] * mx) / 100);
+                                dx += (int16_t)((CTL(hme_l0_w0) * mx) / 100);
                             if (qh_)
-                                dy += (int16_t)((P.hme_l0_h[0] * my) / 100);
-                            so_x = (int16_t)(-(int)(int16_t)(((P.hme_l0_total_w * mx) / 100) >> 1) + dx);
-                            so_y = (int16_t)(-(int)(int16_t)(((P.hme_l0_total_h * my) / 100) >> 1) + dy);
+                                dy += (int16_t)((CTL(hme_l0_h0) * my) / 100);
+                            so_x = (int16_t)(-(int)(int16_t)(((CTL(hme_l0_total_w) * mx) / 100) >> 1) + dx);
+                            so_y = (int16_t)(-(int)(int16_t)(((CTL(hme_l0_total_h) * my) / 100) >> 1) + dy);
                             clamp_area(px16, pad16, pw16, so_x, sw);
                             clamp_area(py16, pad16, ph16, so_y, sh);
                         }
@@ -745,9 +754,9 @@
                         hme_pass(S, 0, R.sixteenth, R.pitch_sixteenth, px16, py16, lw >> 2, 8, nq0, t);
                     if (t < nq0) {
                         const unsigned long long k = S.hkey[t];
-                        const int qx = S.qp[t][0], qy = S.qp[t][1], qwv = S.qp[t][2];
+                        const int qx = S.qp[t][0], qy = S.qp[t][1];
                         if (k != ~0ull) {
-                            const int p = (int)(uint32_t)k, sy = p / qwv, sx = p - sy * qwv;
+                            const int sy = (int)((uint32_t)k >> 16), sx = (int)((uint32_t)k & 0xffffu);
                             S.hx[0][qw_][qh_] = (int16_t)((int16_t)(sx + qx) * 4);
                             S.hy[0][qw_][qh_] = (int16_t)((int16_t)(sy + qy) * 4);
                             S.hs[0][qw_][qh_] = (k >> 32) * 2;
@@ -757,18 +766,18 @@
                             S.hy[0][qw_][qh_] = (int16_t)((int16_t)(S.hy[0][qw_][qh_] + qy) * 4);
                         }
                     }
-                    if (!P.enable_hme_level1 && !P.enable_hme_level2)
+                    if (!CTL(enable_hme_level1) && !CTL(enable_hme_level2))
                         __syncthreads();
                 }
                 for (int lvl = 1; lvl <= 2; lvl++) {
-                    if (!(lvl == 1 ? P.enable_hme_level1 : P.enable_hme_level2))
+                    if (!(lvl == 1 ? CTL(enable_hme_level1) : CTL(enable_hme_level2)))
                         continue;
                     const int shf = 2 - lvl;
                     const int bx0 = ox >> shf, by0 = oy >> shf, pwl = W >> shf, phl = H >> shf;
                     const int padl = lvl == 2 ? LCU - 1 : SVT_AMD_PAD_QUARTER - 1;
                     if (t < nq) {
-                        int sw = hme_l12_width((int16_t)(lvl == 1 ? (qw_ ? P.hme_l1_w[1] : P.hme_l1_w[0]) : (qw_ ? P.hme_l2_w[1] : P.hme_l2_w[0])));
-                        int sh = (int16_t)(lvl == 1 ? (qh_ ? P.hme_l1_h[1] : P.hme_l1_h[0]) : (qh_ ? P.hme_l2_h[1] : P.hme_l2_h[0]));
+                        int sw = hme_l12_width((int16_t)(lvl == 1 ? (qw_ ? CTL(hme_l1_w1) : CTL(hme_l1_w0)) : (qw_ ? CTL(hme_l2_w1) : CTL(hme_l2_w0))));
+                        int sh = (int16_t)(lvl == 1 ? (qh_ ? CTL(hme_l1_h1) : CTL(hme_l1_h0)) : (qh_ ? CTL(hme_l2_h1) : CTL(hme_l2_h0)));
                         const int pcx = lvl == 1 ? (S.hx[0][qw_][qh_] >> 1) : S.hx[1][qw_][qh_];
                         const int pcy = lvl == 1 ? (S.hy[0][qw_][qh_] >> 1) : S.hy[1][qw_][qh_];
                         int so_x = (int16_t)(-(sw >> 1) + pcx), so_y = (int16_t)(-(sh >> 1) + pcy);
@@ -787,28 +796,29 @@
                     if (t < nq) {
                         const unsigned long long k = S.hkey[t];
                         const int qx = S.qp[t][0], qy = S.qp[t][1], qwv = S.qp[t][2];
-                        const int p = (int)(uint32_t)k, sy = p / qwv, sx = p - sy * qwv;
+                        const bool none = k == ~0ull;
+                        const int sy = none ? (qwv == 1 ? -1 : 0) : (int)((uint32_t)k >> 16), sx = none ? -1 - sy * qwv : (int)((uint32_t)k & 0xffffu);
                         S.hx[lvl][qw_][qh_] = (int16_t)((int16_t)(sx + qx) * (1 << shf));
                         S.hy[lvl][qw_][qh_] = (int16_t)((int16_t)(sy + qy) * (1 << shf));
                         S.hs[lvl][qw_][qh_] = (k >> 32) * 2;
                     }
-                    if (lvl == 2 || !P.enable_hme_level2)
+                    if (lvl == 2 || !CTL(enable_hme_level2))
                         __syncthreads();
                 }
                 {
                     int hx = 0, hy = 0;
                     unsigned long long hsv = 0;
-                    const int l0only = P.enable_hme_level0 && !P.enable_hme_level1 && !P.enable_hme_level2;
-                    const int sel = P.enable_hme_level2 ? 2 : (P.enable_hme_level1 ? 1 : (l0only ? 0 : -1));
+                    const int l0only = CTL(enable_hme_level0) && !CTL(enable_hme_level1) && !CTL(enable_hme_level2);
+                    const int sel = CTL(enable_hme_level2) ? 2 : (CTL(enable_hme_level1) ? 1 : (l0only ? 0 : -1));
                     if (sel >= 0) {
                         hx = S.hx[sel][0][0], hy = S.hy[sel][0][0], hsv = S.hs[sel][0][0];
-                        if (!(sel == 0 && P.one_quadrant_hme))
+                        if (!(sel == 0 && CTL(one_quadrant_hme)))
                             for (int h = 0; h < nh; h++)
                                 for (int w = (h == 0 ? 1 : 0); w < nw; w++)
                                     if (S.hs[sel][w][h] < hsv)
                                         hx = S.hx[sel][w][h], hy = S.hy[sel][w][h], hsv = S.hs[sel][w][h];
                     }
-                    if (sel == 2 && P.ref_pocs_equal && list == 1 && nh * nw > 1) {
+                    if (sel == 2 && CTL(ref_pocs_equal) && list == 1 && nh * nw > 1) {
                         __syncthreads();
                         if (t == 0) {
                             const int total = nh * nw;
@@ -834,7 +844,7 @@
 
         STAMP(3);
         if (cx != 0 || cy != 0) {
-            if (P.update_hme_search_center) {
+            if (CTL(update_hme_search_center)) {
                 cx = clamp_center(ox, cx, LCU - 1, W);
                 cy = clamp_center(oy, cy, LCU - 1, H);
             }
@@ -848,7 +858,7 @@
             const unsigned long long zeroCost = (unsigned long long)zeroSad << COST_PRECISION;
             const uint32_t rate = mvd_fraction_bits(abs(cx << 2), abs(cy << 2), S.mvd_bits);
             const unsigned long long hmeCost = (unsigned long long)(uint32_t)(hmeSad << COST_PRECISION) +
-                                               ((((unsigned long long)P.lambda * rate) + MD_OFFSET) >> MD_SHIFT);
+                                               ((((unsigned long long)(uint32_t)CTL(lambda) * rate) + MD_OFFSET) >> MD_SHIFT);
             if (zeroCost <= hmeCost)
                 cx = 0, cy = 0;
             __syncthreads();
@@ -858,7 +868,7 @@
             carry->cx[list] = cx, carry->cy[list] = cy;
             carry->hme_init_done = hme_init_done;
             o->hme_center_x[list] = (int16_t)hcx, o->hme_center_y[list] = (int16_t)hcy;
-            if (P.num_lists == 1)
+            if (CTL(num_lists) == 1)
                 o->hme_center_x[1] = 0, o->hme_center_y[1] = 0;
         }
         if (t < 12) {
@@ -869,7 +879,7 @@
         STAMP(4);
     } else {
         cx = carry->cx[list], cy = carry->cy[list];
-        int saw = imin(P.search_area_width, 127), sah = imin(P.search_area_height, 127);
+        int saw = imin(CTL(search_area_width), 127), sah = imin(CTL(search_area_height), 127);
         int sox = cx - (saw >> 1), soy = cy - (sah >> 1);
         clamp_area(ox, LCU - 1, W, sox, saw);
         clamp_area(oy, LCU - 1, H, soy, sah);
@@ -1122,7 +1132,7 @@
                 B.best_mv[list][t] = mv;
                 vx = mvx(mv), vy = mvy(mv), vs = (int)(2 * s);
             }
-            if (P.fractional_search_model == 1 && t < 128) {
+            if (CTL(fractional_search_model) == 1 && t < 128) {
                 const bool in8 = t >= 21 && t < 85;
                 const int s8x = (int)wave_sum((uint32_t)(in8 ? vx : 0)), s8y = (int)wave_sum((uint32_t)(in8 ? vy : 0)), s8s = (int)wave_sum((uint32_t)(in8 ? vs : 0));
                 if (t < 64) {
@@ -1145,15 +1155,15 @@
 
         STAMP(7);
         int e32 = 0, e16 = 0, e8 = 0, eq = 0;
-        if (P.fractional_search_model == 0) {
+        if (CTL(fractional_search_model) == 0) {
             e32 = e16 = e8 = eq = 1;
-        } else if (P.fractional_search_model == 1) {
+        } else if (CTL(fractional_search_model) == 1) {
             const int sx32 = B.sums[0], sy32 = B.sums[1], ss32 = B.sums[2], ss16 = B.sums[5];
             const int sx8 = B.sums[6] + B.sums[9], sy8 = B.sums[7] + B.sums[10], ss8 = B.sums[8] + B.sums[11];
             const uint32_t ux32 = (uint32_t)(sx32 >> 2), uy32 = (uint32_t)(sy32 >> 2), ux8 = (uint32_t)(sx8 >> 6), uy8 = (uint32_t)(sy8 >> 6);
             const uint32_t mag32 = ux32 * ux32 + uy32 * uy32, mag8 = ux8 * ux8 + uy8 * uy8;
             const uint32_t avg32 = (uint32_t)ss32 >> 2, avg16 = (uint32_t)ss16 >> 4, avg8 = (uint32_t)ss8 >> 6;
-            const int tl = P.temporal_layer_index;
+            const int tl = CTL(temporal_layer_index);
             const uint32_t th = tl == 0 ? 48 * 48 : tl == 1 ? 32 * 32 : tl == 2 ? 80 * 80 : 48 * 48;
             const int small32 = mag32 < th, low32 = avg32 < 32 * 32 * 6;
             e32 = (tl == 0 || tl == 2) ? low32 : (tl == 1 ? (small32 ? low32 : 1) : (small32 ? 1 : low32));
@@ -1161,11 +1171,11 @@
             e8 = (tl <= 2) ? !(avg8 < 8 * 8 * 2) : ((mag8 < th) ? !(avg8 < 8 * 8 * 2) : 0);
             eq = 1;
         }
-        e16 = e16 && P.cu16x16_mode == 0, e8 = e8 && P.cu8x8_mode != 1;
+        e16 = e16 && CTL(cu16x16_mode) == 0, e8 = e8 && CTL(cu8x8_mode) != 1;
         const int any_sub = e32 || e16 || e8 || eq || 0;
-        const int run_sub = (P.fractional_search_model != 2) && any_sub;
+        const int run_sub = (CTL(fractional_search_model) != 2) && any_sub;
         if (run_sub) {
-            const int f64 = P.fractional_search_64x64;
+            const int f64 = CTL(fractional_search_64x64);
             const int en0 = f64, en1 = e32, en2 = e16, en3 = e8;
 #define EN(tier_) pick4(tier_, en0, en1, en2, en3)
             const int rstep = (method == SVT_AMD_SUB_SAD_SEARCH) ? 2 : 1;
@@ -1393,24 +1403,24 @@
         if (t < 85) {
             o->best_sad[list][t] = B.best_sad[list][t];
             o->best_mv[list][t] = B.best_mv[list][t];
-            if (P.num_lists == 1)
+            if (CTL(num_lists) == 1)
                 o->best_sad[1][t] = 0, o->best_mv[1][t] = 0;
         }
         if (t == 0) {
             o->search_origin_x[list] = (int16_t)sox, o->search_origin_y[list] = (int16_t)soy;
             o->search_w[list] = (uint8_t)saw, o->search_h[list] = (uint8_t)sah;
-            if (P.num_lists == 1)
+            if (CTL(num_lists) == 1)
                 o->search_origin_x[1] = 0, o->search_origin_y[1] = 0, o->search_w[1] = 0, o->search_h[1] = 0;
         }
-        if (list != P.num_lists - 1) {
+        if (list != CTL(num_lists) - 1) {
             STAMP(12);
             return;
         }
 
     STAMP(10);
-    if (P.num_lists == 2) {
+    if (CTL(num_lists) == 2) {
         const int rstep = (method == SVT_AMD_SUB_SAD_SEARCH) ? 2 : 1;
-        const int npu = (P.cu16x16_mode != 0) ? 5 : ((P.cu8x8_mode != 0) ? 21 : 85);
+        const int npu = (CTL(cu16x16_mode) != 0) ? 5 : ((CTL(cu8x8_mode) != 0) ? 21 : 85);
         int cum[5];
         cum[0] = 0;
 #pragma unroll
@@ -1507,8 +1517,8 @@
     if (t < 85) {
         const int pu = t;
         const int n = pu == 0 ? 0 : pu < 5 ? pu : pu < 21 ? c_tab16[pu - 5] + 5 : c_tab8[pu - 21] + 21;
-        int total = P.num_lists;
-        if (P.num_lists == 2 && (P.cu8x8_mode == 0 || pu < 21) && (P.cu16x16_mode == 0 || pu < 5))
+        int total = CTL(num_lists);
+        if (CTL(num_lists) == 2 && (CTL(cu8x8_mode) == 0 || pu < 21) && (CTL(cu16x16_mode) == 0 || pu < 5))
             total = 3;
         const uint32_t bi = (method == SVT_AMD_SUB_SAD_SEARCH) ? (B.bipred[n] << 1) : B.bipred[n];
         const uint32_t v[3] = {B.best_sad[0][n], B.best_sad[1][n], bi};
diff --git a/svt-hevc_amd/csrc/svt_amd_internal.h b/svt-hevc_amd/csrc/svt_amd_internal.h
--- a/svt-hevc_amd/csrc/svt_amd_internal.h
+++ b/svt-hevc_amd/csrc/svt_amd_internal.h
@@ -5,6 +5,7 @@
 #include <stdint.h>
 #include "../../include/svt_hevc_amd.h"
 #include "slot_records.h"
+#include "me_controls.h"
 
 static inline int svt_amd_lcu_count(int w, int h) { return ((w + 63) / 64) * ((h + 63) / 64); }
 
@@ -45,6 +46,7 @@
 
 struct MeJobDev {
     SvtAmdMeParams P;
+    uint32_t ctl[ME_CTL_WORDS];
     PicView cur, ref0, ref1;
     SvtAmdMeLcuResult *out;
     struct MeCarry *carry;
```

Result: no change. 4810 fps, median of 2 (+0.1%).
